# lvjiahui/DRT

Measured on AMD Instinct MI355X. Metric: M camera-rays/s (forward+backward) on 50k-tri mesh, 72 views, higher is better.
Workload: dtype f32 traversal + f64 shading/gradients; 1 GPU; horse_vh.ply x4 (1 midpoint subdivision) = 50248 tris / 25126 verts, 72 turntable views, 1024x1024 rays/view, LBVH rebuilt every step, forward+ray_loss+backward+all-reduce+SGD; targets=horse_scan.ply, mode=dropin, hip_graph=False, outputs_recycled=True, ray_binding=True, views_per_gpu=72, views_per_call=72

## Files before the change

drt_amd/_lib.py:

```python
from __future__ import annotations

import ctypes
import os

_HERE = os.path.dirname(os.path.abspath(__file__))
LIB_PATH = os.environ.get("DRT_HIP_LIB") or os.path.join(_HERE, "libdrt_hip.so")

_c = ctypes
_P = _c.c_void_p
_I64 = _c.c_int64
_D = _c.c_double

SIGNATURES = {
    "drt_last_error": (_c.c_char_p, []),
    "drt_version": (_c.c_int, []),
    "drt_deterministic": (_c.c_int, [_c.c_int]),
    "drt_fx_finalize": (_c.c_int, [_P, _I64, _P, _c.c_int, _P]),
    "drt_fx_add": (_c.c_int, [_P, _P, _I64, _P]),
    "drt_fx_to_limbs": (_c.c_int, [_P, _I64, _P, _P]),
    "drt_fx_from_limbs": (_c.c_int, [_P, _I64, _P, _P]),
    "drt_create": (_c.c_int, [_c.c_int, _c.POINTER(_P)]),
    "drt_destroy": (None, [_P]),
    "drt_update_mesh": (_c.c_int, [_P, _P, _I64, _P, _I64, _P]),
    "drt_update_vert": (_c.c_int, [_P, _P, _I64, _P]),
    "drt_update_vert_f64": (_c.c_int, [_P, _P, _I64, _P]),
    "drt_intersect": (_c.c_int, [_P, _P, _I64, _P, _P, _P]),
    "drt_intersect_any": (_c.c_int, [_P, _P, _I64, _P, _P]),
    "drt_intersect_bruteforce": (_c.c_int, [_P, _P, _I64, _P, _P, _P]),
    "drt_bvh_check": (_c.c_int, [_P, _P, _c.POINTER(_I64), _c.POINTER(_c.c_int32), _c.POINTER(_c.c_int32)]),
    "drt_bvh_sorted_faces": (_c.c_int, [_P, _P, _P]),
    "drt_build_params": (_c.c_int, [_P, _c.POINTER(_c.c_float), _P]),
    "drt_bvh_export": (_c.c_int, [_P, _c.c_int, _P, _I64, _P]),
    "drt_tree_mode": (_c.c_int, [_P, _c.c_int, _c.c_int]),
    "drt_render_forward": (_c.c_int, [_P, _P, _P, _P, _I64, _D, _D, _P, _P, _P, _P, _P, _P, _P, _c.c_int, _c.c_int, _c.c_int, _P, _P]),
    "drt_render_backward": (_c.c_int, [_P, _P, _P, _P, _I64, _D, _D, _P, _P, _P, _P, _P, _P, _P, _P]),
    "drt_render_paths_forward": (_c.c_int, [_P, _P, _P, _P, _I64, _D, _D, _c.c_int, _c.c_int, _P, _P, _P, _P, _P, _P, _P, _P]),
    "drt_render_paths_backward": (_c.c_int, [_P, _P, _P, _P, _I64, _D, _D, _c.c_int, _c.c_int, _P, _P, _P, _P, _P, _P, _P, _P]),
    "drt_render_paths_ray_loss_fused": (_c.c_int, [_P, _P, _P, _P, _P, _P, _I64, _D, _D, _c.c_int, _c.c_int, _P, _P, _P, _P]),
    "drt_render_paths_law_forward": (_c.c_int, [_P, _P, _P, _P, _I64, _D, _D, _c.c_int, _c.c_int, _P, _P, _P, _P, _P, _P, _P, _P]),
    "drt_render_paths_law_backward": (_c.c_int, [_P, _P, _P, _P, _I64, _D, _D, _c.c_int, _c.c_int, _P, _P, _P, _P, _P, _P, _P, _P]),
    "drt_render_paths_law_ray_loss_fused": (_c.c_int, [_P, _P, _P, _P, _P, _P, _I64, _D, _D, _c.c_int, _c.c_int, _P, _P, _P, _P]),
    "drt_render_paths_law_ray_loss_ior_fused": (_c.c_int, [_P, _P, _P, _P, _P, _P, _I64, _D, _D, _c.c_int, _c.c_int, _P, _P, _P, _P, _P]),
    "drt_ray_loss": (_c.c_int, [_P, _P, _P, _P, _P, _I64, _P, _P, _P, _P, _P]),
    "drt_ray_loss_listed": (_c.c_int, [_P, _P, _P, _P, _P, _P, _I64, _P, _P, _P, _P]),
    "drt_prefill_zero": (_c.c_int, [_P, _P, _I64, _P]),
    "drt_prefill_wait": (_c.c_int, [_P, _P]),
    "drt_outputs_clean": (_c.c_int, [_P, _P, _P, _P, _I64, _P, _P, _P]),
    "drt_outputs_cancel": (_c.c_int, [_P]),
    "drt_render_seed": (_c.c_int, [_P, _P, _I64]),
    "drt_render_loss_arm": (_c.c_int, [_P, _P, _P, _P, _P, _I64]),
    "drt_render_loss_taken": (_c.c_int, [_P]),
    "drt_ray_loss_listed_grad": (_c.c_int, [_P, _P, _P, _P, _I64, _D, _D, _P, _P, _P, _P, _P, _P, _P, _P, _P]),
    "drt_ray_loss_listed_grad_split": (_c.c_int, [_P, _P, _P, _P, _I64, _D, _D, _P, _P, _P, _P, _P, _P, _P, _P, _P]),
    "drt_scale_rows3": (_c.c_int, [_P, _P, _P, _P, _P]),
    "drt_render_backward_ray_loss": (_c.c_int, [_P, _P, _P, _P, _I64, _D, _D, _P, _P, _P, _P, _P, _P, _P, _P]),
    "drt_render_backward_inputs": (_c.c_int, [_P, _P, _P, _P, _I64, _D, _D, _P, _P, _P, _P, _P, _P, _P, _P, _P, _P, _P]),
    "drt_render_backward_ray_loss_inputs": (_c.c_int, [_P, _P, _P, _P, _I64, _D, _D, _P, _P, _P, _P, _P, _P, _P, _P, _P, _P, _P]),
    "drt_render_ray_loss_fused": (_c.c_int, [_P, _P, _P, _P, _P, _P, _I64, _D, _D, _P, _P, _P, _c.c_int, _c.c_int, _c.c_int, _P, _P]),
    "drt_dihedral_forward": (_c.c_int, [_P, _P, _I64, _P, _P]),
    "drt_dihedral_backward": (_c.c_int, [_P, _P, _I64, _P, _P, _P]),
    "drt_sm_loss_fused": (_c.c_int, [_P, _P, _I64, _P, _P, _P]),
    "drt_silhouette_flags": (_c.c_int, [_P, _P, _I64, _P, _P, _P]),
    "drt_edge_sample_forward": (_c.c_int, [_P, _P, _P, _I64, _P, _P, _P, _P, _P, _c.c_int, _c.c_int, _P, _P]),
    "drt_edge_sample_backward": (_c.c_int, [_P, _P, _I64, _P, _P, _P, _c.c_int, _P, _P]),
    "drt_edge_sample_backward_rows": (_c.c_int, [_P, _P, _I64, _P, _P, _P, _I64, _P, _c.c_int, _P, _P]),
    "drt_vh_term": (_c.c_int, [_P, _P, _I64, _P, _c.c_int, _c.c_int, _P, _P, _P]),
    "drt_edge_sample_backward_term": (_c.c_int, [_P, _P, _I64, _P, _P, _P, _P, _c.c_int, _P, _P]),
    "drt_edge_tables_workspace": (_I64, [_I64]),
    "drt_edge_tables": (_c.c_int, [_P, _I64, _P, _I64, _P, _P, _P, _P, _P, _P, _P]),
    "drt_subdivide_midpoint": (_c.c_int, [_P, _I64, _P, _I64, _P, _I64, _P, _c.c_int, _P, _P, _P]),
    "drt_hull_field": (_c.c_int, [_P, _c.c_int, _c.c_int, _c.c_int, _P, _D, _D, _D, _D, _c.c_int, _c.c_int, _c.c_int, _c.c_int, _P, _P]),
    "drt_hull_mark": (_c.c_int, [_P, _c.c_int, _c.c_int, _c.c_int, _D, _P, _P, _P, _P]),
    "drt_hull_emit": (_c.c_int, [_P, _c.c_int, _c.c_int, _c.c_int, _D, _D, _D, _D, _D, _P, _P, _P, _I64, _I64, _P, _P, _P]),
    "drt_decode_patterns": (_c.c_int, [_P, _P, _I64, _c.c_int, _c.c_int, _c.c_int, _c.c_int, _c.c_int, _c.c_int, _c.c_int, _P, _c.c_int, _P, _P, _P, _P, _P, _P]),
    "drt_render_image": (_c.c_int, [_P, _P, _P, _c.c_int, _c.c_int, _c.c_int, _c.c_int, _c.c_int, _D, _D, _c.c_int, _c.c_int, _c.c_int, _P, _P, _c.c_int, _c.c_int,
                                    _c.c_int, _P, _P, _P, _P, _P, _P]),
    "drt_render_image_loss": (_c.c_int, [_P, _P, _P, _c.c_int, _c.c_int, _c.c_int, _c.c_int, _c.c_int, _D, _D, _c.c_int, _c.c_int, _c.c_int, _P, _P, _c.c_int,
                                         _c.c_int, _c.c_int, _P, _P, _P, _P, _P, _P, _P, _P, _P, _P]),
    "drt_render_image_loss_screen": (_c.c_int, [_P, _P, _P, _c.c_int, _c.c_int, _c.c_int, _c.c_int, _c.c_int, _D, _D, _c.c_int, _c.c_int, _c.c_int, _P, _P, _c.c_int,
                                                _c.c_int, _c.c_int, _P, _P, _P, _P, _P, _P, _P, _P, _P, _P, _P, _P]),
    "drt_render_image_loss_camera": (_c.c_int, [_P, _P, _P, _c.c_int, _c.c_int, _c.c_int, _c.c_int, _c.c_int, _D, _D, _c.c_int, _c.c_int, _c.c_int, _P, _P, _c.c_int,
                                                _c.c_int, _c.c_int, _P, _P, _P, _P, _P, _P, _P, _P, _P, _P, _P, _P, _P]),
    "drt_render_image_absorb": (_c.c_int, [_P, _P, _P, _c.c_int, _c.c_int, _c.c_int, _c.c_int, _c.c_int, _D, _D, _c.c_int, _c.c_int, _c.c_int, _P, _P, _c.c_int,
                                           _c.c_int, _c.c_int, _P, _P, _P, _P, _P, _P, _P, _P]),
    "drt_render_image_loss_absorb": (_c.c_int, [_P, _P, _P, _c.c_int, _c.c_int, _c.c_int, _c.c_int, _c.c_int, _D, _D, _c.c_int, _c.c_int, _c.c_int, _P, _P, _c.c_int,
                                                _c.c_int, _c.c_int, _P, _P, _P, _P, _P, _P, _P, _P, _P, _P, _P, _P]),
    "drt_render_image_env": (_c.c_int, [_P, _P, _P, _c.c_int, _c.c_int, _c.c_int, _c.c_int, _c.c_int, _D, _D, _c.c_int, _c.c_int, _c.c_int, _P, _P, _c.c_int,
                                        _c.c_int, _c.c_int, _P, _P, _P, _P, _P, _P, _c.c_int, _c.c_int, _P, _c.c_int, _P, _P]),
    "drt_render_image_loss_env": (_c.c_int, [_P, _P, _P, _c.c_int, _c.c_int, _c.c_int, _c.c_int, _c.c_int, _D, _D, _c.c_int, _c.c_int, _c.c_int, _P, _P, _c.c_int,
                                             _c.c_int, _c.c_int, _P, _P, _P, _P, _P, _P, _P, _P, _P, _P, _c.c_int, _c.c_int, _P, _c.c_int, _P]),
    "drt_render_image_loss_env_param": (_c.c_int, [_P, _P, _P, _c.c_int, _c.c_int, _c.c_int, _c.c_int, _c.c_int, _D, _D, _c.c_int, _c.c_int, _c.c_int, _P, _P,
                                                   _c.c_int, _c.c_int, _c.c_int, _P, _P, _P, _P, _P, _P, _P, _P, _P, _P, _c.c_int, _c.c_int, _P, _c.c_int, _P, _P, _P]),
    "drt_image_views_check": (_c.c_int, [_c.c_int, _P, _P, _c.c_int, _c.c_int]),
    "drt_image_views_create": (_c.c_int, [_P, _c.c_int, _P, _P, _c.c_int, _c.c_int, _c.POINTER(_P)]),
    "drt_image_views_destroy": (None, [_P]),
    "drt_render_image_loss_views": (_c.c_int, [_P, _P, _P, _P, _c.c_int, _c.c_int, _c.c_int, _c.c_int, _D, _D, _c.c_int, _c.c_int, _c.c_int, _P, _c.c_int,
                                               _c.c_int, _c.c_int, _P, _P, _P, _P, _P, _P, _P, _P, _P]),
    "drt_render_image_loss_views_env": (_c.c_int, [_P, _P, _P, _P, _c.c_int, _c.c_int, _c.c_int, _c.c_int, _D, _D, _c.c_int, _c.c_int, _c.c_int, _P, _c.c_int,
                                                   _c.c_int, _c.c_int, _P, _P, _P, _P, _P, _P, _P, _P, _P, _c.c_int, _c.c_int, _P, _c.c_int, _P]),
    "drt_limit_sgd_step": (_c.c_int, [_P, _P, _P, _I64, _D, _D, _c.c_int, _c.c_int, _D, _P]),
    "drt_limit_sgd_step3": (_c.c_int, [_P, _P, _P, _I64, _D, _D, _c.c_int, _c.c_int, _D, _P, _P, _P, _P, _P]),
    "drt_weight_terms3": (_c.c_int, [_P, _P, _I64, _P, _P]),
    "drt_limit_sgd_step_total": (_c.c_int, [_P, _P, _P, _I64, _D, _D, _c.c_int, _c.c_int, _D, _P, _P, _P, _P]),
    "drt_fx_limbs_limit_sgd_step3": (_c.c_int, [_P, _I64, _P, _P, _P, _D, _D, _c.c_int, _c.c_int, _D, _P, _P, _P, _P]),
    "drt_internal_stream": (_c.c_int, [_P, _c.c_int, _c.POINTER(_P)]),
    "drt_closest_point": (_c.c_int, [_P, _P, _I64, _P, _P, _P, _P]),
    "drt_vh_loss_fused": (_c.c_int, [_P, _P, _P, _P, _I64, _c.c_int, _P, _P, _P, _c.c_int, _c.c_int, _c.c_int, _P, _P, _P]),
    "drt_remesh_isotropic": (_c.c_int, [_P, _I64, _P, _I64, _D, _c.c_int, _D, _c.c_uint, _c.POINTER(_P)]),
    "drt_rm_split_mark": (_c.c_int, [_P, _I64, _P, _D, _P, _P]),
    "drt_rm_split_plan": (_c.c_int, [_P, _I64, _P, _P, _P, _P, _I64, _P, _P, _P]),
    "drt_rm_split_faces": (_c.c_int, [_P, _I64, _P, _P, _P, _P, _P]),
    "drt_rm_vertex_normals": (_c.c_int, [_P, _P, _P, _P, _I64, _P, _P]),
    "drt_rm_vertex_faces": (_c.c_int, [_P, _I64, _I64, _P, _P, _P, _P, _P, _P, _P]),
    "drt_rm_collapse_eval_all": (_c.c_int, [_P, _I64, _P, _P, _P, _P, _D, _D, _c.c_int, _P, _P, _P, _P, _P, _P, _P, _P, _I64, _P, _P]),
    "drt_rm_surface_filter_list": (_c.c_int, [_P, _P, _P, _P, _P, _I64, _D, _P, _P]),
    "drt_rm_surface_filter": (_c.c_int, [_P, _P, _P, _P, _I64, _c.c_int, _D, _P, _P]),
    "drt_rm_closest_near": (_c.c_int, [_P, _P, _I64, _D, _P, _P]),
    "drt_rm_kill_faces": (_c.c_int, [_P, _P, _I64, _P, _P]),
    "drt_rm_collapse_apply": (_c.c_int, [_P, _I64, _P, _P, _P, _P, _P, _P, _I64, _D, _c.c_uint32, _c.c_int, _P, _P, _P, _P, _P, _c.c_int, _P, _P, _P]),
    "drt_rm_round_end": (_c.c_int, [_P, _c.c_int, _P]),
    "drt_rm_flip_eval": (_c.c_int, [_P, _I64, _P, _P, _P, _P, _D, _P, _P, _P, _P, _P]),
    "drt_rm_flip_apply": (_c.c_int, [_I64, _P, _P, _P, _I64, _c.c_int, _P, _P, _c.c_int, _P, _P, _P]),
    "drt_rm_smooth_target": (_c.c_int, [_P, _P, _P, _P, _I64, _P, _P]),
    "drt_rm_face_agreement": (_c.c_int, [_P, _P, _P, _I64, _P, _P]),
    "drt_rm_move_check": (_c.c_int, [_P, _P, _P, _P, _P, _I64, _I64, _P, _P, _P]),
    "drt_mesh_buf_size": (_c.c_int, [_P, _c.POINTER(_I64), _c.POINTER(_I64), _P]),
    "drt_mesh_buf_copy": (_c.c_int, [_P, _P, _P]),
    "drt_mesh_buf_free": (None, [_P]),
    "drt_profile_enable": (_c.c_int, [_P, _c.c_int]),
    "drt_profile_select": (_c.c_int, [_P, _c.c_uint32]),
    "drt_profile_read": (_c.c_int, [_P, _P, _P, _P]),
    "drt_profile_trace_stats": (_c.c_int, [_P, _P]),
    "drt_route_counts": (_c.c_int, [_P, _P]),
    "drt_raster_deal_counts": (_c.c_int, [_P, _P]),
    "drt_check_violations": (_c.c_int, [_P]),
}

_lib = None


class DrtError(RuntimeError):
    pass


def lib():
    global _lib
    if _lib is None:
        if not os.path.exists(LIB_PATH):
            raise DrtError(f"{LIB_PATH} not found: the HIP extension is not built "
                           "(run `python __graft_entry__.py`); there is no CPU fallback")
        h = ctypes.CDLL(LIB_PATH)
        for name, (res, args) in SIGNATURES.items():
            if os.environ.get("DRT_HIP_LIB") and not hasattr(h, name):
                continue
            fn = getattr(h, name)
            fn.restype = res
            fn.argtypes = args
        _lib = h
    return _lib


def check(rc):
    if rc != 0:
        raise DrtError(f"libdrt_hip error {rc}: {lib().drt_last_error().decode(errors='replace')}")


def ptr(t):
    return None if t is None else t.data_ptr()
```

drt_amd/csrc/drt_api.hip:

```cpp
#include "drt_scene.h"

static thread_local char g_err[512] = "";
int fail(int code, const char* fmt, ...) {
    va_list ap;
    va_start(ap, fmt);
    vsnprintf(g_err, sizeof(g_err), fmt, ap);
    va_end(ap);
    return code;
}

int ensure_slow_stack(drt_scene* s, hipStream_t st) {
    if (s->slow_stack) return DRT_OK;
    hipStreamCaptureStatus cap = hipStreamCaptureStatusNone;
    if (hipStreamIsCapturing(st, &cap) == hipSuccess && cap != hipStreamCaptureStatusNone)
        return fail(DRT_E_INVALID, "the first silhouette / closest-point / intersect query of a scene allocates its overflow area and cannot run inside a "
                                   "stream capture: issue one such call eagerly before capturing");
    int blocks = s->grid_trace;
    if (blocks < 4 * s->n_cu) blocks = 4 * s->n_cu;
    if (blocks < kRedoGrid) blocks = kRedoGrid;
    HIP_TRY(hipMalloc(&s->slow_stack, sizeof(int32_t) * (size_t)blocks * kTraceBlock * kStackSlowDev));
    return DRT_OK;
}

static int g_det = -1;
bool det_mode() {
    if (g_det < 0) { const char* ev = getenv("DRT_DETERMINISTIC"); g_det = ev && atoi(ev) != 0 ? 1 : 0; }
    return g_det != 0;
}
__global__ void __launch_bounds__(256) k_fx_finalize(const FxCell* __restrict__ cells, int64_t n, double* __restrict__ out, int accumulate) {
    for (int64_t i = blockIdx.x * 256ll + threadIdx.x; i < n; i += (int64_t)gridDim.x * 256) {
        const FxCell c = cells[i];
        const double v = fx_to_double(Fx128{c.hi, c.lo}, (uint32_t)c.flags);
        out[i] = accumulate ? out[i] + v : v;
    }
}

__global__ void __launch_bounds__(256) k_fx_add(FxCell* __restrict__ dst, const FxCell* __restrict__ src, int64_t n) {
    for (int64_t i = blockIdx.x * 256ll + threadIdx.x; i < n; i += (int64_t)gridDim.x * 256) {
        const FxCell a = dst[i], b = src[i];
        const Fx128 r = fx_add(Fx128{a.hi, a.lo}, Fx128{b.hi, b.lo});
        dst[i] = FxCell{r.hi, r.lo, a.flags | b.flags};
    }
}
constexpr int kLimbBits = kFxLimbBits;
__global__ void __launch_bounds__(256) k_fx_to_limbs(const FxCell* __restrict__ cells, int64_t n, int64_t* __restrict__ limbs) {
    constexpr uint64_t kMask = (1ull << kLimbBits) - 1ull;
    for (int64_t i = blockIdx.x * 256ll + threadIdx.x; i < n; i += (int64_t)gridDim.x * 256) {
        const FxCell c = cells[i];
        const uint64_t hi = (uint64_t)c.hi;
        limbs[4 * i + 0] = (int64_t)(c.lo & kMask);
        limbs[4 * i + 1] = (int64_t)(((c.lo >> kLimbBits) | (hi << (64 - kLimbBits))) & kMask);
        limbs[4 * i + 2] = c.hi >> (2 * kLimbBits - 64);
        limbs[4 * i + 3] = (int64_t)(((c.flags & kFxNaN) ? 1ull : 0ull) | ((c.flags & kFxPosInf) ? 1ull << 20 : 0ull) | ((c.flags & kFxNegInf) ? 1ull << 40 : 0ull));
    }
}
__global__ void __launch_bounds__(256) k_fx_from_limbs(const int64_t* __restrict__ limbs, int64_t n, FxCell* __restrict__ cells) {
    for (int64_t i = blockIdx.x * 256ll + threadIdx.x; i < n; i += (int64_t)gridDim.x * 256) {
        uint32_t flags;
        const Fx128 r = fx_from_limbs(limbs + 4 * i, flags);
        cells[i] = FxCell{r.hi, r.lo, (uint64_t)flags};
    }
}

extern "C" {

const char* drt_last_error(void) { return g_err; }
int drt_version(void) { return 13; }

int drt_deterministic(int on) {
    const int was = det_mode() ? 1 : 0;
    if (on >= 0) g_det = on != 0;
    return was;
}
int drt_fx_add(void* d_dst_cells, const void* d_src_cells, int64_t n, void* stream) {
    if (n < 0) return fail(DRT_E_INVALID, "negative size");
    if (n == 0) return DRT_OK;
    if (!d_dst_cells || !d_src_cells) return fail(DRT_E_INVALID, "null pointer argument");
    k_fx_add<<<grid_for(n, 256, 1024), 256, 0, (hipStream_t)stream>>>(static_cast<FxCell*>(d_dst_cells), static_cast<const FxCell*>(d_src_cells), n);
    HIP_TRY(hipGetLastError());
    return DRT_OK;
}
int drt_fx_to_limbs(const void* d_cells, int64_t n, int64_t* d_limbs, void* stream) {
    if (n < 0) return fail(DRT_E_INVALID, "negative size");
    if (n == 0) return DRT_OK;
    if (!d_cells || !d_limbs) return fail(DRT_E_INVALID, "null pointer argument");
    k_fx_to_limbs<<<grid_for(n, 256, 1024), 256, 0, (hipStream_t)stream>>>(static_cast<const FxCell*>(d_cells), n, d_limbs);
    HIP_TRY(hipGetLastError());
    return DRT_OK;
}
int drt_fx_from_limbs(const int64_t* d_limbs, int64_t n, void* d_cells, void* stream) {
    if (n < 0) return fail(DRT_E_INVALID, "negative size");
    if (n == 0) return DRT_OK;
    if (!d_cells || !d_limbs) return fail(DRT_E_INVALID, "null pointer argument");
    k_fx_from_limbs<<<grid_for(n, 256, 1024), 256, 0, (hipStream_t)stream>>>(d_limbs, n, static_cast<FxCell*>(d_cells));
    HIP_TRY(hipGetLastError());
    return DRT_OK;
}
int drt_fx_finalize(const void* d_cells, int64_t n, double* d_out, int accumulate, void* stream) {
    if (n < 0) return fail(DRT_E_INVALID, "negative size");
    if (n == 0) return DRT_OK;
    if (!d_cells || !d_out) return fail(DRT_E_INVALID, "null pointer argument");
    k_fx_finalize<<<grid_for(n, 256, 1024), 256, 0, (hipStream_t)stream>>>(static_cast<const FxCell*>(d_cells), n, d_out, accumulate);
    HIP_TRY(hipGetLastError());
    return DRT_OK;
}

int drt_create(int device, drt_scene_t** out) {
    if (!out) return fail(DRT_E_INVALID, "out is null");
    int count = 0;
    HIP_TRY(hipGetDeviceCount(&count));
    if (device < 0 || device >= count) return fail(DRT_E_INVALID, "device %d out of range (%d visible)", device, count);
    HIP_TRY(hipSetDevice(device));
    drt_scene* s = new (std::nothrow) drt_scene();
    if (!s) return fail(DRT_E_NOMEM, "host allocation failed");
    s->device = device;
    hipError_t e = hipMalloc(&s->params, sizeof(BuildParams));
    if (e == hipSuccess) e = hipMalloc(&s->scratch, sizeof(unsigned long long) * 8);
    if (e == hipSuccess) e = hipMalloc(&s->bounds_acc, sizeof(uint32_t) * 12);
    if (e == hipSuccess) {
        const uint32_t init[12] = {0xFF800000u, 0xFF800000u, 0xFF800000u, 0x007FFFFFu, 0x007FFFFFu, 0x007FFFFFu,
                                   0xFF800000u, 0xFF800000u, 0xFF800000u, 0x007FFFFFu, 0x007FFFFFu, 0x007FFFFFu};
        e = hipMemcpy(s->bounds_acc, init, sizeof(init), hipMemcpyHostToDevice);
    }
    if (e == hipSuccess) e = hipMalloc(&s->vcount, sizeof(unsigned) * 4);
    if (e == hipSuccess) e = hipMemset(s->vcount, 0, sizeof(unsigned) * 4);
    if (e == hipSuccess) e = hipMalloc(&s->seg_counts, sizeof(unsigned) * drt_scene::kMaxSeg);
    if (e == hipSuccess) e = hipEventCreateWithFlags(&s->fork_ev, hipEventDisableTiming);
    if (e == hipSuccess) e = hipStreamCreateWithFlags(&s->build_stream, hipStreamNonBlocking);
    if (e == hipSuccess) e = hipEventCreateWithFlags(&s->prefill_fork, hipEventDisableTiming);
    if (e == hipSuccess) e = hipEventCreateWithFlags(&s->prefill_done, hipEventDisableTiming);
    if (e == hipSuccess) e = hipEventCreateWithFlags(&s->prefill_done_cap, hipEventDisableTiming);
    if (e == hipSuccess) e = hipEventCreateWithFlags(&s->build_fork, hipEventDisableTiming);
    if (e == hipSuccess) e = hipEventCreateWithFlags(&s->build_done, hipEventDisableTiming);
    if (const char* ev = getenv("DRT_ASYNC_BUILD")) s->async_build = atoi(ev) != 0;
    if (const char* ev = getenv("DRT_CULL_DIRECT")) s->cull_direct = atoi(ev) != 0;
    if (const char* ev = getenv("DRT_CULL_PARK")) s->cull_park = atoi(ev) != 0;
    if (const char* ev = getenv("DRT_CULL_DIRECT_MIN_LOG2")) { const int v = atoi(ev); if (v >= 0 && v <= 40) s->cull_direct_min_rays = (int64_t)1 << v; }
    if (const char* ev = getenv("DRT_TREE")) { const int v = atoi(ev); if (v >= 0 && v <= 2) s->tree_mode = v; }
    if (const char* ev = getenv("DRT_REBUILD_EVERY")) { const int v = atoi(ev); if (v >= 1) s->rebuild_every = v; }
    if (const char* ev = getenv("DRT_STREAMS")) { const int v = atoi(ev); if (v >= 1 && v <= drt_scene::kMaxSub) s->n_sub = v; }
    if (const char* ev = getenv("DRT_RASTER")) s->use_raster = atoi(ev) != 0;
    if (const char* ev = getenv("DRT_RASTER_DEAL")) s->raster_deal = atoi(ev) != 0;
    if (const char* ev = getenv("DRT_RASTER_DEAL_MIN_RUNS")) { const long long v = atoll(ev); if (v >= 0) s->raster_deal_min_runs = v; }
    if (const char* ev = getenv("DRT_RASTER_DEAL_FIXED")) { const int v = atoi(ev); if (v >= 1 && v <= 65536) s->raster_deal_fixed = (uint32_t)v; }
    if (const char* ev = getenv("DRT_HIT_SEED")) s->hit_seed = atoi(ev) != 0;
    if (const char* ev = getenv("DRT_ARM_FINISH_BESIDE")) s->arm_finish_beside = atoi(ev) != 0;
    if (const char* ev = getenv("DRT_SEED_TILED")) s->seed_tiled = atoi(ev) != 0;
    if (const char* ev = getenv("DRT_GRID_CANARY")) s->grid_canary = atoi(ev) != 0;
    if (const char* ev = getenv("DRT_FILL_OVERLAP")) s->fill_overlap = atoi(ev) != 0;
    if (const char* ev = getenv("DRT_FILL_AFTER_SHADE1")) s->fill_after_shade1 = atoi(ev) != 0;
    if (const char* ev = getenv("DRT_SUB_PER_STREAM")) { const int v = atoi(ev); if (v >= 1 && v <= 16) s->sub_per_stream = v; }
    if (const char* ev = getenv("DRT_MIN_SUB_LOG2")) { const int v = atoi(ev); if (v >= 12 && v <= 30) s->min_sub_rays = (int64_t)1 << v; }
    for (int k = 0; k < s->n_sub && e == hipSuccess; ++k) {
        drt_scene::Sub& w = s->sub[k];
        e = hipStreamCreateWithFlags(&w.stream, hipStreamNonBlocking);
        if (e == hipSuccess) e = hipEventCreateWithFlags(&w.done, hipEventDisableTiming);
        if (e == hipSuccess) e = hipEventCreateWithFlags(&w.tail, hipEventDisableTiming);
        if (e == hipSuccess) e = hipEventCreateWithFlags(&w.fill_fork, hipEventDisableTiming);
        if (e == hipSuccess) e = hipEventCreateWithFlags(&w.fill_join, hipEventDisableTiming);
        if (e == hipSuccess) e = hipMalloc(&w.qcount, sizeof(unsigned) * kQCount);
        if (e == hipSuccess) e = hipMalloc(&w.slow_stack, sizeof(int32_t) * (size_t)kRedoGrid * kTraceBlock * kStackSlowDev);
    }
    if (e == hipSuccess) {
        hipDeviceProp_t prop;
        if (hipGetDeviceProperties(&prop, device) == hipSuccess && prop.multiProcessorCount > 0) s->n_cu = prop.multiProcessorCount;
        int per_cu;
        per_cu = query_blocks_per_cu();
        s->grid_trace = s->n_cu * per_cu;
        if (s->grid_trace > kTraceGridMax) s->grid_trace = kTraceGridMax;
        per_cu = pipeline_blocks_per_cu();
        s->grid_path = s->n_cu * per_cu;
        if (s->grid_path * 2 > kTraceGridMax) s->grid_path = kTraceGridMax / 2;
        per_cu = mega_blocks_per_cu();
        s->grid_mega = s->n_cu * per_cu;
        if (const char* e = getenv("DRT_MEGA_BPC")) { const int v = atoi(e); if (v >= 1 && v <= 8) s->grid_mega = v * s->n_cu; }
        if (const char* e = getenv("DRT_MEGA_MAX_LOG2")) { const int v = atoi(e); s->mega_max_rays = v <= 0 ? 0 : (v <= 31 ? (int64_t)1 << v : (int64_t)1 << 31); }
        if (const char* e = getenv("DRT_SHADE_MIN")) { const int v = atoi(e); if (v >= 1 && v <= 64) s->shade_min = v; }
        if (const char* e = getenv("DRT_MEGA_REFILL_MIN")) { const int v = atoi(e); if (v >= 1 && v <= 64) s->mega_refill_min = v; }
        if (const char* e = getenv("DRT_TRACE_BPC")) { const int v = atoi(e); if (v >= 1 && v * s->n_cu * 2 <= kTraceGridMax) s->grid_path = v * s->n_cu; }
        if (const char* e = getenv("DRT_INNER_MIN")) { const int v = atoi(e); if (v >= 1 && v <= 64) s->inner_min = v; }
        if (const char* e = getenv("DRT_REFILL_MIN")) { const int v = atoi(e); if (v >= 1 && v <= 64) s->refill_min = v; }
        if (const char* e = getenv("DRT_CHUNK_LOG2")) { const int v = atoi(e); if (v >= 16 && v <= 30) s->chunk_rays = (int64_t)1 << v; }
    }
    if (e != hipSuccess) {
        drt_destroy(s);
        return fail(DRT_E_HIP, "hipMalloc: %s", hipGetErrorString(e));
    }
    *out = s;
    return DRT_OK;
}

void drt_destroy(drt_scene_t* s) {
    if (!s) return;
    (void)hipSetDevice(s->device);
    if (s->build_stream) (void)hipStreamSynchronize(s->build_stream);
    scene_free_mesh(s);
    if (s->build_fork) (void)hipEventDestroy(s->build_fork);
    if (s->build_done) (void)hipEventDestroy(s->build_done);
    if (s->build_stream) (void)hipStreamDestroy(s->build_stream);
    (void)hipFree(s->params);
    (void)hipFree(s->slow_stack);
    (void)hipFree(s->scratch); (void)hipFree(s->bounds_acc); (void)hipFree(s->seg_counts);
    (void)hipFree(s->b1_list); (void)hipFree(s->b1_redo); (void)hipFree(s->b1_count);
    for (int j = 0; j < drt_scene::kMaxSub; ++j) {
        drt_scene::Sub& w = s->sub[j];
        for (int k = 0; k < 3; ++k) { (void)hipFree(w.q_idx[k]); (void)hipFree(w.q_ray[k]); (void)hipFree(w.q_face[k]); }
        (void)hipFree(w.tmp_face1); (void)hipFree(w.tmp_face2); (void)hipFree(w.qcount); (void)hipFree(w.slow_stack); (void)hipFree(w.redo);
        (void)hipFree(w.zbuf); (void)hipFree(w.zmask); (void)hipFree(w.vmodel); (void)hipFree(w.big); (void)hipFree(w.big_count); (void)hipFree(w.gen_list); (void)hipFree(w.ray64);
        (void)hipFree(w.deal.table);
        if (w.done) (void)hipEventDestroy(w.done);
        if (w.fill_fork) (void)hipEventDestroy(w.fill_fork);
        if (w.fill_join) (void)hipEventDestroy(w.fill_join);
        if (w.tail) (void)hipEventDestroy(w.tail);
        if (w.stream) (void)hipStreamDestroy(w.stream);
    }
    image_views_free(s);
    image_loss_free(s);
    paths_free(s);
    (void)hipFree(s->vcount);
    (void)hipFree(s->vh_list);
    if (s->fork_ev) (void)hipEventDestroy(s->fork_ev);
    if (s->prefill_fork) (void)hipEventDestroy(s->prefill_fork);
    if (s->prefill_done) (void)hipEventDestroy(s->prefill_done);
    if (s->prefill_done_cap) (void)hipEventDestroy(s->prefill_done_cap);
    for (auto& e : s->prof_ev) (void)hipEventDestroy(e);
    (void)hipFree(s->prof_counts);
    delete s;
}

int drt_profile_enable(drt_scene_t* s, int on) {
    CHECK_SCENE(s);
    if (on && s->prof_ev.empty()) {
        s->prof_ev.resize(8192);
        s->prof_stage.resize(4096);
        for (auto& e : s->prof_ev) HIP_TRY(hipEventCreate(&e));
        HIP_TRY(hipMalloc(&s->prof_counts, sizeof(unsigned long long) * (kProfStages + 12)));
        HIP_TRY(hipMemset(s->prof_counts, 0, sizeof(unsigned long long) * (kProfStages + 12)));
    }
    s->prof_on = on != 0;
    s->prof_stats = on == 2;
    s->prof_serial = on == 3;
    return DRT_OK;
}

int drt_profile_select(drt_scene_t* s, uint32_t stage_mask) {
    CHECK_SCENE(s);
    s->prof_mask = stage_mask;
    return DRT_OK;
}

int drt_profile_read(drt_scene_t* s, double* ms_out, int64_t* launches_out, int64_t* items_out) {
    CHECK_SCENE(s);
    if (!ms_out || !launches_out || !items_out) return fail(DRT_E_INVALID, "null pointer argument");
    for (int k = 0; k < kProfStages; ++k) { ms_out[k] = 0.0; launches_out[k] = 0; items_out[k] = 0; }
    if (s->prof_ev.empty()) return DRT_OK;
    HIP_TRY(hipStreamSynchronize(s->prof_stream));
    if (s->build_stream) HIP_TRY(hipStreamSynchronize(s->build_stream));
    if (s->prof_dropped) {
        const size_t lost = s->prof_dropped;
        s->prof_dropped = 0; s->prof_used = 0;
        return fail(DRT_E_INVALID, "%zu stage timings were not recorded (event pool exhausted): read the profile more often", lost);
    }
    for (size_t k = 0; k + 1 < s->prof_used; k += 2) {
        float ms = 0.f;
        HIP_TRY(hipEventElapsedTime(&ms, s->prof_ev[k], s->prof_ev[k + 1]));
        const int stg = s->prof_stage[k / 2];
        ms_out[stg] += ms;
        launches_out[stg] += 1;
    }
    unsigned long long h[kProfStages + 12];
    HIP_TRY(hipMemcpy(h, s->prof_counts, sizeof(h), hipMemcpyDeviceToHost));
    for (int k = 0; k < kProfStages; ++k) items_out[k] = (int64_t)h[k];
    for (int k = 0; k < 12; ++k) s->trace_stats[k] = (int64_t)h[kProfStages + k];
    HIP_TRY(hipMemset(s->prof_counts, 0, sizeof(h)));
    s->prof_used = 0;
    return DRT_OK;
}

int drt_route_counts(drt_scene_t* s, int64_t* out8) {
    CHECK_SCENE(s);
    if (!out8) return fail(DRT_E_INVALID, "null pointer argument");
    for (int k = 0; k < 8; ++k) out8[k] = s->route_counts[k];
    return DRT_OK;
}

int drt_raster_deal_counts(drt_scene_t* s, int64_t* out2) {
    CHECK_SCENE(s);
    if (!out2) return fail(DRT_E_INVALID, "null pointer argument");
    out2[0] = s->raster_deal_counts[0]; out2[1] = s->raster_deal_counts[1];
    return DRT_OK;
}

int drt_internal_stream(drt_scene_t* s, int which, void** out) {
    if (!s || !out) return fail(DRT_E_INVALID, "null pointer argument");
    if (which == 0) { *out = (void*)s->build_stream; return DRT_OK; }
    if (which >= 1 && which <= s->n_sub) { *out = (void*)s->sub[which - 1].stream; return DRT_OK; }
    return fail(DRT_E_INVALID, "no internal stream %d (0 = build, 1..%d = pipelines)", which, s->n_sub);
}

int drt_check_violations(int64_t* out4) {
    if (!out4) return fail(DRT_E_INVALID, "null pointer argument");
#if defined(DRT_CHECK)
    HIP_TRY(hipDeviceSynchronize());
    unsigned long long tot[4] = {0, 0, 0, 0};
    if (check_counters_pipeline(tot) || check_counters_trace(tot)) return fail(DRT_E_HIP, "could not read the check counters");
    for (int k = 0; k < 4; ++k) out4[k] = (int64_t)tot[k];
#else
    for (int k = 0; k < 4; ++k) out4[k] = -1;
#endif
    return DRT_OK;
}

int drt_profile_trace_stats(drt_scene_t* s, int64_t* out12) {
    CHECK_SCENE(s);
    if (!out12) return fail(DRT_E_INVALID, "null pointer argument");
    for (int k = 0; k < 12; ++k) out12[k] = s->trace_stats[k];
    return DRT_OK;
}


}
```

drt_amd/csrc/drt_pipeline.hip:

```cpp
#include "drt_device.h"
#include "drt_trace_kernel.h"
#include "drt_pathsink.h"


struct Ray64 {
    double* o;
    double* d;
};
struct Pipe {
    RayList r0, r1, r2;
    unsigned* count;
    unsigned* valid;
    int32_t* redo;
};




__device__ __forceinline__ void write_dead(int64_t i, double* out_ori, double* out_dir, uint8_t* mask, int32_t* face2) {
    const d3 z{0.0, 0.0, 0.0};
    store_d3(out_ori, i, z);
    store_d3(out_dir, i, z);
    mask[3 * i] = 0; mask[3 * i + 1] = 0; mask[3 * i + 2] = 0;
    face2[i] = -1;
// ... 103 lines not shown
            } else if (!FUSED || valid[i]) {
                const d3 o64 = load_d3(origin, i), d64 = load_d3(dir, i);
                o = to_f32(o64); d = to_f32(d64);
                bool verified = false;
                if (raster) {
                    ViewModel& vm = rz.views[view];
                    verified = vm.ok && view_verify(vm, o64, d64, (double)x, (double)(y - view * (unsigned)rz.img_h));
                    if (!verified && vm.all) __hip_atomic_store(&vm.all, 0, __ATOMIC_RELAXED, __HIP_MEMORY_SCOPE_AGENT);
                }
                if (verified) {
                    cand = key != kRasterEmpty;
                    face = (int32_t)(uint32_t)key;
                } else {
                    cand = n_tris > 0 && (rz.no_tree || hits_top_boxes(nodes, o, d));
                    generic = cand;
                }
            } else if (raster && rz.mode == DRT_GRID_ESTABLISH) {
                ViewModel& vm = rz.views[view];
                if (vm.all && !(vm.ok && view_verify(vm, load_d3(origin, i), load_d3(dir, i), (double)x, (double)(y - view * (unsigned)rz.img_h))))
                    __hip_atomic_store(&vm.all, 0, __ATOMIC_RELAXED, __HIP_MEMORY_SCOPE_AGENT);
            }
        }
        const bool live = i < n;
        if (!dead_writes) {
        } else if (tile_w > 0 && __ballot(cand || !live) == 0ull) {
            write_dead_row<FUSED>(i - (tid & 63), tid & 63, out_ori, out_dir, mask, face1, face2);
        } else if (live && !cand) {
            face1[i] = -1;
            write_dead(i, out_ori, out_dir, mask, face2);
        }
        const int any_cand = __syncthreads_or(cand ? 1 : 0);
        if (clear_bit && (tid & 63) == 0) atomicAnd(&rz.zmask[i >> 11], ~clear_bit);
        if (!any_cand) return;
        int slot;
        if (tile_w > 0) {
            s_flag[vt] = cand ? 1 : 0;
            __syncthreads();
            s_slot[tid] = block_push(s_flag[tid] != 0, &p.count[0], s_tmp);
            __syncthreads();
            slot = s_slot[vt];
            __syncthreads();
        } else {
            slot = block_push(cand, &p.count[0], s_tmp);
        }
        if (slot >= 0) {
            p.r0.idx[slot] = (int32_t)i; store_ray32(p.r0.ray, slot, o, d);
            if (raster) p.r0.face[slot] = generic && rz.pending ? kFacePending : face;
        }
        if (raster && __syncthreads_or(generic ? 1 : 0)) {
            const int g = block_push(generic, &p.count[3], s_tmp);
            if (g >= 0) rz.gen_list[g] = slot;
        }
    }
}

template <bool FUSED>
__global__ void __launch_bounds__(kPathBlock, 8) k_cull(const Node4Q* __restrict__ nodes, int n_tris, const double* __restrict__ origin, const double* __restrict__ dir,
                                                      const uint8_t* __restrict__ valid, int64_t n, double* __restrict__ out_ori,
                                                      double* __restrict__ out_dir, uint8_t* __restrict__ mask,
                                                      int32_t* __restrict__ face1, int32_t* __restrict__ face2, Pipe p, int tile_w, RasterIn rz,
                                                      bool prefilled ) {
    __shared__ CullShared sh;
    cull_patch<FUSED>(blockIdx.x, prefilled, sh, nodes, n_tris, origin, dir, valid, n, out_ori, out_dir, mask, face1, face2, p, tile_w, rz);
}

constexpr int kCullRun = 4;
constexpr int kCullPer = kCullRun;
constexpr int kCullCap = kCullRun * kPathBlock;
constexpr int kCullCursor = 32;
constexpr int kCullFewPerCu = 2;
constexpr int kCullLongRuns = 16;
static_assert(kCullCursor < kQCount, "the cursor word lies inside the counter block");
struct CullBatch {
    int32_t idx[kCullCap];
    int32_t face[kCullCap];
    unsigned n, base, next[2];
    unsigned wtot[kCullPer][kPathWaves];
};
template <bool FUSED>
__global__ void __launch_bounds__(kPathBlock) k_cull_listed(const uint32_t* __restrict__ patches, const unsigned* __restrict__ n_patches,
                                                           const Node4Q* __restrict__ nodes, int n_tris, const double* __restrict__ origin, const double* __restrict__ dir,
                                                           const uint8_t* __restrict__ valid, int64_t n, double* __restrict__ out_ori,
                                                           double* __restrict__ out_dir, uint8_t* __restrict__ mask,
                                                           int32_t* __restrict__ face1, int32_t* __restrict__ face2, Pipe p, int tile_w, RasterIn rz,
                                                           PathCtx c, bool direct, bool prefilled, Ray64 park, unsigned few, unsigned long_list) {
    __shared__ CullShared sh;
    __shared__ CullBatch sb;
    const int tid = threadIdx.x, wave = tid >> 6, lane = tid & 63;
    const unsigned ppr = (unsigned)tile_w / 64u;
    const RayList dst = direct ? p.r1 : p.r0;
    unsigned* const dst_count = direct ? &p.count[1] : &p.count[0];
    unsigned* const cursor = &p.count[kCullCursor];
    unsigned n_hits = 0;
    const unsigned count = *n_patches;
    const unsigned active = count >= long_list ? gridDim.x : min(few, gridDim.x);
    if (blockIdx.x >= active) return;
    unsigned first = blockIdx.x * (unsigned)kCullRun;
    if (tid == 0) {
        sb.n = 0u;
        if (first < count) sb.next[0] = active * (unsigned)kCullRun + atomicAdd(cursor, (unsigned)kCullRun);
    }
    __syncthreads();

    auto close_batch = [&]() {
        const unsigned cnt = sb.n;
        if (cnt == 0u) { __syncthreads(); return; }
        int32_t ei[kCullPer], ef[kCullPer];
        f3 eo[kCullPer], ed[kCullPer];
        bool push[kCullPer];
        unsigned rank[kCullPer];
#pragma unroll
        for (int j = 0; j < kCullPer; ++j) {
            const unsigned k = (unsigned)(j * kPathBlock + tid);
            push[j] = false;
            ei[j] = 0; ef[j] = -1;
            eo[j] = f3{0.f, 0.f, 0.f}; ed[j] = f3{0.f, 0.f, 1.f};
            if (k < cnt) {
                const int64_t i = sb.idx[k];
                const int32_t f1 = sb.face[k];
                ei[j] = (int32_t)i; ef[j] = f1;
                if (direct) {
                    face1[i] = f1;
                    d3 v0, v1, v2;
                    int32_t vid[3];
                    Bounce b;
                    load_tri64(c, f1, v0, v1, v2, vid);
                    bounce_forward(load_d3(origin, i), load_d3(dir, i), v0, v1, v2, c.ior_ext, c.ior_int, b);
                    push[j] = !b.tir;
                    eo[j] = to_f32(b.new_o); ed[j] = to_f32(b.wt);
                    if (push[j] && park.o) { store_d3(park.o, i, b.new_o); store_d3(park.d, i, b.wt); }
                    if (!push[j] && !FUSED) { if (prefilled) face2[i] = -1; else write_dead(i, out_ori, out_dir, mask, face2); }
                    ++n_hits;
                } else {
                    eo[j] = to_f32(load_d3(origin, i)); ed[j] = to_f32(load_d3(dir, i));
                    push[j] = true;
                }
            }
            const unsigned long long bm = __ballot(push[j]);
            if (lane == 0) sb.wtot[j][wave] = (unsigned)__popcll(bm);
            rank[j] = (unsigned)__popcll(bm & ((1ull << lane) - 1ull));
        }
        __syncthreads();
        unsigned tot = 0;
#pragma unroll
        for (int j = 0; j < kCullPer; ++j) {
            unsigned before = tot;
#pragma unroll
            for (int w = 0; w < kPathWaves; ++w) { const unsigned cw = sb.wtot[j][w]; if (w < wave) before += cw; tot += cw; }
            rank[j] += before;
        }
        if (tid == 0) { sb.base = tot ? atomicAdd(dst_count, tot) : 0u; sb.n = 0u; }
        __syncthreads();
        const unsigned base = sb.base;
#pragma unroll
        for (int j = 0; j < kCullPer; ++j) {
            if (!push[j]) continue;
            const unsigned slot = base + rank[j];
            dst.idx[slot] = ei[j];
            float2* e = reinterpret_cast<float2*>(dst.ray + 6 * (int64_t)slot);
            e[0] = float2{eo[j].x, eo[j].y}; e[1] = float2{eo[j].z, ed[j].x}; e[2] = float2{ed[j].y, ed[j].z};
            if (!direct) dst.face[slot] = ef[j];
        }
    };

    for (unsigned it = 0; first < count; ++it) {
        const unsigned cnt = min((unsigned)kCullRun, count - first);
        uint32_t pt[kCullRun];
        bool ok[kCullRun];
        unsigned word[kCullRun];
        unsigned long long key[kCullRun];
        int64_t zs[kCullRun], ri[kCullRun];
#pragma unroll
        for (int j = 0; j < kCullRun; ++j) pt[j] = (unsigned)j < cnt ? patches[first + j] : 0u;
#pragma unroll
        for (int j = 0; j < kCullRun; ++j) {
            const unsigned prow = pt[j] / ppr;
            const unsigned x = 64u * (pt[j] - prow * ppr) + 16u * (unsigned)wave + 4u * ((unsigned)lane >> 4) + ((unsigned)lane & 3u);
            const unsigned y = 4u * prow + (((unsigned)lane >> 2) & 3u);
            const unsigned view = (4u * prow) / (unsigned)rz.img_h;
            ri[j] = (int64_t)y * tile_w + x;
            zs[j] = raster_slot(x, y, (unsigned)tile_w);
            ok[j] = false; word[j] = 0u; key[j] = kRasterEmpty;
            if ((unsigned)j < cnt) {
                ok[j] = rz.views[view].ok && rz.views[view].all;
                word[j] = rz.zmask[ri[j] >> 11];
                key[j] = rz.zbuf[zs[j]];
            }
        }
#pragma unroll
        for (int j = 0; j < kCullRun; ++j) {
            if ((unsigned)j >= cnt) continue;
            if (!ok[j]) {
                cull_patch<FUSED>(pt[j], true, sh, nodes, n_tris, origin, dir, valid, n, out_ori, out_dir, mask, face1, face2, p, tile_w, rz);
                __syncthreads();
                continue;
            }
            const int64_t i = ri[j];
            const bool has = ((word[j] >> ((i >> 6) & 31)) & 1u) != 0u && key[j] != kRasterEmpty;
            if (has) rz.zbuf[zs[j]] = kRasterEmpty;
            const bool take = has && (!FUSED || valid[i]);
            const unsigned long long bm = __ballot(take);
            if (bm != 0ull) {
                unsigned at = 0u;
                if (lane == 0) at = atomicAdd(&sb.n, (unsigned)__popcll(bm));
                at = (unsigned)__shfl((int)at, 0);
                if (take) {
                    const unsigned k = at + (unsigned)__popcll(bm & ((1ull << lane) - 1ull));
                    sb.idx[k] = (int32_t)i;
                    sb.face[k] = (int32_t)(uint32_t)key[j];
                }
            }
        }
        __syncthreads();
        if (tid < 4 * (int)cnt) {
            const unsigned q = patches[first + ((unsigned)tid >> 2)], prow = q / ppr;
            const int64_t i0 = (int64_t)(4u * prow + ((unsigned)tid & 3u)) * tile_w + 64u * (q - prow * ppr);
            const unsigned bit = 1u << ((i0 >> 6) & 31);
            if (rz.zmask[i0 >> 11] & bit) atomicAnd(&rz.zmask[i0 >> 11], ~bit);
        }
        const unsigned nxt = sb.next[it & 1u];
        if (tid == 0 && nxt < count) sb.next[(it + 1u) & 1u] = active * (unsigned)kCullRun + atomicAdd(cursor, (unsigned)kCullRun);
        close_batch();
        first = nxt;
    }
    if (direct) {
        unsigned h = n_hits;
        for (int off = 32; off >= 1; off >>= 1) h += __shfl_xor(h, off);
        if (lane == 0 && h) atomicAdd(&p.count[17], h);
    }
}
constexpr int kCullSgprBlocks = 6;
int cull_blocks_per_cu() {
    int per_cu = 0;
    if (hipOccupancyMaxActiveBlocksPerMultiprocessor(&per_cu, k_cull_listed<false>, kPathBlock, 0) != hipSuccess || per_cu < 1) per_cu = 4;
    int f = 0;
    if (hipOccupancyMaxActiveBlocksPerMultiprocessor(&f, k_cull_listed<true>, kPathBlock, 0) == hipSuccess && f >= 1 && f < per_cu) per_cu = f;
    if (per_cu > 8) per_cu = 8;
    if (per_cu > kCullSgprBlocks) per_cu = kCullSgprBlocks;
    return per_cu;
}

__global__ void __launch_bounds__(kPathBlock) k_patch_list(unsigned n_patches, int tile_w, RasterIn rz, uint32_t* __restrict__ list, unsigned* count) {
    __shared__ unsigned s_tmp[kPathWaves + 1];
    const unsigned patch = blockIdx.x * kPathBlock + threadIdx.x;
    bool take = false;
    if (patch < n_patches) {
        const unsigned ppr = (unsigned)tile_w / 64u, prow = patch / ppr;
        const unsigned view = (4u * prow) / (unsigned)rz.img_h;
        take = true;
        if (rz.views[view].ok && rz.views[view].all) {
            const int64_t row0 = (int64_t)(4u * prow) * tile_w + 64u * (patch - prow * ppr);
            unsigned any = 0;
            for (int r = 0; r < 4; ++r) {
                const int64_t g = (row0 + (int64_t)r * tile_w) >> 6;
                any |= rz.zmask[g >> 5] >> (g & 31);
            }
            take = (any & 1u) != 0;
        }
    }
    const int slot = block_push(take, count, s_tmp);
    if (slot >= 0) list[slot] = patch;
}

template <bool FUSED>
__global__ void __launch_bounds__(kPathBlock) k_shade1(PathCtx c, const double* __restrict__ origin, const double* __restrict__ dir,
                                                        double* __restrict__ out_ori, double* __restrict__ out_dir, uint8_t* __restrict__ mask,
                                                        int32_t* __restrict__ face1, int32_t* __restrict__ face2, Pipe p,
                                                        bool prefilled , Ray64 r64) {
    __shared__ StageMem stage;
    stage_init(stage);
    const unsigned n0 = p.count[0];
    const unsigned per_block = ((n0 + gridDim.x - 1) / gridDim.x + kPathBlock - 1) / kPathBlock * kPathBlock;
    const unsigned first = blockIdx.x * per_block, last = min(n0, first + per_block);
    for (unsigned base = first; base < last; base += kPathBlock) {
        const unsigned k = base + threadIdx.x;
        bool ok = false;
        int64_t i = 0;
        f3 o2{0.f, 0.f, 0.f}, d2{0.f, 0.f, 1.f};
        if (k < n0) {
            i = p.r0.idx[k];
            const int32_t f1 = p.r0.face[k];
            if (f1 != kFacePending) face1[i] = f1;
            if (f1 >= 0) {
                d3 v0, v1, v2;
                int32_t vid[3];
                Bounce b;
                load_tri64(c, f1, v0, v1, v2, vid);
                bounce_forward(load_d3(origin, i), load_d3(dir, i), v0, v1, v2, c.ior_ext, c.ior_int, b);
                ok = !b.tir;
                o2 = to_f32(b.new_o); d2 = to_f32(b.wt);
                if (ok && r64.o) { store_d3(r64.o, i, b.new_o); store_d3(r64.d, i, b.wt); }
            }
            if (!ok && !FUSED && f1 != kFacePending) { if (prefilled) face2[i] = -1; else write_dead(i, out_ori, out_dir, mask, face2); }
        }
        stage_push(stage, ok, (int32_t)i, o2, d2, p.r1, &p.count[1]);
    }
    stage_flush(stage, p.r1, &p.count[1]);
}

template <bool FUSED>
__global__ void __launch_bounds__(kTraceBlock) k_gen_late(PathCtx c, const double* __restrict__ origin, const double* __restrict__ dir,
                                                          double* __restrict__ out_ori, double* __restrict__ out_dir, uint8_t* __restrict__ mask,
                                                          int32_t* __restrict__ face1, int32_t* __restrict__ face2, Pipe p,
                                                          const int32_t* __restrict__ gen_list, bool prefilled, Ray64 r64) {
    __shared__ int32_t lds[kStackFast][kTraceBlock];
    const unsigned n = p.count[3];
    if (n == 0) return;
    Stack st = make_stack(lds, c.tc);
    for (unsigned k = blockIdx.x * kTraceBlock + threadIdx.x; k < n; k += gridDim.x * kTraceBlock) {
        const int32_t slot = gen_list[k];
        if (p.r0.face[slot] != kFacePending) continue;
        const int64_t i = p.r0.idx[slot];
        const float* e = p.r0.ray + 6 * (int64_t)slot;
        const Hit h = traverse<false>(c.tc.nodes, c.tc.tris, c.tc.n_tris, f3{e[0], e[1], e[2]}, f3{e[3], e[4], e[5]}, st);
        p.r0.face[slot] = h.face;
        face1[i] = h.face;
        bool ok = false;
        if (h.face >= 0) {
            d3 v0, v1, v2;
            int32_t vid[3];
            Bounce b;
            load_tri64(c, h.face, v0, v1, v2, vid);
            bounce_forward(load_d3(origin, i), load_d3(dir, i), v0, v1, v2, c.ior_ext, c.ior_int, b);
            ok = !b.tir;
            if (ok) {
                const unsigned s1 = atomicAdd(&p.count[1], 1u);
                p.r1.idx[s1] = (int32_t)i;
                store_ray32(p.r1.ray, (int)s1, to_f32(b.new_o), to_f32(b.wt));
                if (r64.o) { store_d3(r64.o, i, b.new_o); store_d3(r64.d, i, b.wt); }
            }
        }
        if (!ok && !FUSED) { if (prefilled) face2[i] = -1; else write_dead(i, out_ori, out_dir, mask, face2); }
    }
}

template <bool FUSED>
__global__ void __launch_bounds__(kPathBlock) k_shade2(PathCtx c, const double* __restrict__ origin, const double* __restrict__ dir,
                                                        double* __restrict__ out_ori, double* __restrict__ out_dir, uint8_t* __restrict__ mask,
                                                        const int32_t* __restrict__ face1, int32_t* __restrict__ face2, Pipe p,
                                                        bool parked ) {
    __shared__ StageMem stage;
    stage_init(stage);
    const unsigned n1 = p.count[1];
    const unsigned per_block = ((n1 + gridDim.x - 1) / gridDim.x + kPathBlock - 1) / kPathBlock * kPathBlock;
    const unsigned first = blockIdx.x * per_block, last = min(n1, first + per_block);
    for (unsigned base = first; base < last; base += kPathBlock) {
        const unsigned k = base + threadIdx.x;
        bool ok = false;
        int64_t i = 0;
        f3 o3{0.f, 0.f, 0.f}, d3f{0.f, 0.f, 1.f};
        if (k < n1) {
            i = p.r1.idx[k];
            const int32_t f2 = p.r1.face[k];
            if (f2 >= 0) {
                d3 v0, v1, v2;
                int32_t vid[3];
                Bounce b;
                d3 o2, d2;
                if (parked) {
                    o2 = load_d3(out_ori, i); d2 = load_d3(out_dir, i);
                } else {
                    load_tri64(c, face1[i], v0, v1, v2, vid);
                    bounce_forward(load_d3(origin, i), load_d3(dir, i), v0, v1, v2, c.ior_ext, c.ior_int, b);
                    o2 = b.new_o; d2 = b.wt;
                }
                load_tri64(c, f2, v0, v1, v2, vid);
                bounce_forward(o2, d2, v0, v1, v2, c.ior_ext, c.ior_int, b);
                ok = !b.tir;
                if (ok) {
                    o3 = to_f32(b.new_o); d3f = to_f32(b.wt);
                    face2[i] = f2;
                    if (!FUSED) {
                        store_d3(out_ori, i, b.new_o);
                        store_d3(out_dir, i, b.wt);
                        mask[3 * i] = 1; mask[3 * i + 1] = 1; mask[3 * i + 2] = 1;
                    }
                }
            }
            if (!ok) { if (FUSED) face2[i] = -1; else write_dead(i, out_ori, out_dir, mask, face2); }
        }
        stage_push(stage, ok, (int32_t)i, o3, d3f, p.r2, &p.count[2]);
    }
    stage_flush(stage, p.r2, &p.count[2]);
}

__global__ void __launch_bounds__(kPathBlock) k_finish(double* __restrict__ out_ori, double* __restrict__ out_dir, uint8_t* __restrict__ mask,
                                                        int32_t* __restrict__ face2, Pipe p, int64_t chunk_base, int32_t* __restrict__ valid_idx) {
    __shared__ StageMem stage;
    stage_init(stage);
    const RayList out{valid_idx, nullptr, nullptr};
    const unsigned n2 = p.count[2];
    const unsigned per_block = ((n2 + gridDim.x - 1) / gridDim.x + kPathBlock - 1) / kPathBlock * kPathBlock;
    const unsigned first = blockIdx.x * per_block, last = min(n2, first + per_block);
    for (unsigned base = first; base < last; base += kPathBlock) {
        const unsigned k = base + threadIdx.x;
        bool keep = false;
        int64_t i = 0;
        if (k < n2) {
            i = p.r2.idx[k];
            keep = p.r2.face[k] < 0;
            if (!keep) write_dead(i, out_ori, out_dir, mask, face2);
        }
        if (valid_idx) stage_push(stage, keep, (int32_t)(chunk_base + i), f3{0.f, 0.f, 0.f}, f3{0.f, 0.f, 0.f}, out, p.valid);
    }
    if (valid_idx) stage_flush(stage, out, p.valid);
}

enum : int { kLaneIdle = 0, kLaneT1 = 2, kLaneT1D = 3, kLaneT2 = 4, kLaneT2D = 5 };
constexpr int kVBuf = 128;

template <class STACK>
__device__ __forceinline__ bool path_leaf(const TriRec* __restrict__ tris, TravState& s, STACK& st, bool any) {
    if (s.cur == kEmptyChild) return trav_pop(s, st);
    const int32_t ref = ~s.cur;
    const int first = ref >> kLeafBits, count = (ref & (kLeafMax - 1)) + 1;
    for (int j = 0; j < count; ++j) {
        const F4* tp = reinterpret_cast<const F4*>(tris + first + j);
        const F4 p0 = tp[0], p1 = tp[1], p2 = tp[2];
        float t;
        if (tri_hit(s.o, s.d, f3{p0.x, p0.y, p0.z}, f3{p1.x, p1.y, p1.z}, f3{p2.x, p2.y, p2.z}, p1.w, t)) {
            int32_t face;
            memcpy(&face, &p0.w, 4);
            if (any) { s.best_t = t; s.best_face = face; return true; }
            if (t < s.best_t || (t == s.best_t && face < s.best_face)) { s.best_t = t; s.best_face = face; }
        }
    }
    return trav_pop(s, st);
}

template <bool FUSED>
__global__ void __launch_bounds__(kPathBlock, 4) k_path(PathCtx c, Ray64 r64, double* __restrict__ out_ori, double* __restrict__ out_dir, uint8_t* __restrict__ mask,
                                                        int32_t* __restrict__ face2, Pipe p, unsigned* cursor , int64_t chunk_base,
                                                        int32_t* __restrict__ valid_idx, int refill_min, int inner_min, int shade_min,
                                                        unsigned long long* stats, bool count_items) {
    __shared__ int32_t lds[kStackFast + 1 + kGuardRows][kPathBlock];
    __shared__ int32_t s_vbuf[kPathWaves][kVBuf];
    FastStack st;
    st.base = (drt::FastPtr)&lds[0][threadIdx.x]; st.stride = kPathBlock; st.depth = kStackFast - 3; st.reset(); st.overflow = false;
#if defined(DRT_CHECK)
    for (int g = 0; g < kGuardRows; ++g) lds[kStackFast + 1 + g][threadIdx.x] = kGuardPoison;
#endif
    const unsigned n = p.count[1];
    const int lane = threadIdx.x & 63, wv = threadIdx.x >> 6;
    const unsigned long long lower = (1ull << lane) - 1ull;
    constexpr unsigned kXcd = 8;
    const bool split = gridDim.x % kXcd == 0 && n >= 4096u * kXcd;
    const unsigned xcd = split ? blockIdx.x % kXcd : 0u, parts = split ? kXcd : 1u;
    const unsigned wave = (split ? blockIdx.x / kXcd : blockIdx.x) * kPathWaves + (threadIdx.x >> 6);
    const unsigned n_waves = (split ? gridDim.x / kXcd : gridDim.x) * kPathWaves;
    const unsigned part_lo = (unsigned)((unsigned long long)n * xcd / parts), part_hi = (unsigned)((unsigned long long)n * (xcd + 1) / parts);
    const unsigned part_n = part_hi - part_lo;
    unsigned first = (part_n + n_waves - 1) / n_waves;
    first = first > 64u ? 64u : (first < 8u ? 8u : first);
    unsigned my_next = part_lo + wave * first;
    unsigned my_end = my_next + first;
    if (my_end > part_hi) my_end = part_hi;
    if (my_next > part_hi) my_next = part_hi;
    const unsigned dyn_lo = part_lo + n_waves * first;
    bool dry = dyn_lo >= part_hi;
    int32_t* const v_out = FUSED ? p.r2.idx : valid_idx;
    unsigned* const v_count = FUSED ? &p.count[2] : p.valid;
    unsigned vn = 0;
    auto v_flush = [&]() {
        if (vn == 0) return;
        unsigned base = 0;
        if (lane == 0) base = atomicAdd(v_count, vn);
        base = (unsigned)__builtin_amdgcn_readfirstlane((int)base);
        for (unsigned k = lane; k < vn; k += 64u) {
            v_out[base + k] = s_vbuf[wv][k];
            if (FUSED) p.r2.face[base + k] = -1;
        }
        vn = 0;
    };
    int stage = kLaneIdle;
    int32_t rk = 0, ri = 0;
    TravState s;
    s.cur = 0; s.best_face = -1; s.best_t = 0.f;
    unsigned long long wave_steps = 0, lane_steps = 0, leaf_steps = 0;
    unsigned n_t2 = 0;
    for (;;) {
        const unsigned long long idle = __ballot(stage == kLaneIdle);
        if (idle != 0 && (my_next < my_end || !dry) && ((int)__popcll(idle) >= refill_min || idle == ~0ull)) {
            const unsigned want = (unsigned)__popcll(idle);
            unsigned base, got;
            if (my_next < my_end) {
                base = my_next;
                got = my_end - my_next < want ? my_end - my_next : want;
                my_next += got;
            } else {
                unsigned b0 = 0;
                if (lane == 0) b0 = atomicAdd(&cursor[xcd], want);
                b0 = (unsigned)__builtin_amdgcn_readfirstlane((int)b0);
                base = dyn_lo + b0;
                got = base >= part_hi ? 0u : (part_hi - base < want ? part_hi - base : want);
                if (got < want) dry = true;
            }
            const unsigned r = (unsigned)__popcll(idle & lower);
            if (stage == kLaneIdle && r < got) {
                const unsigned k = base + r;
                rk = (int32_t)k;
                ri = p.r1.idx[k];
                const float* e = p.r1.ray + 6 * (int64_t)k;
                trav_init(s, st, f3{e[0], e[1], e[2]}, f3{e[3], e[4], e[5]});
                st.overflow = false;
                stage = kLaneT1;
            }
        }
        if (__ballot(stage != kLaneIdle) == 0) {
            if (my_next < my_end || !dry) continue;
            break;
        }
        {
            const unsigned long long waiting = __ballot(stage & 1), walking = __ballot(stage != kLaneIdle && !(stage & 1));
            if (waiting != 0 && ((int)__popcll(waiting) >= shade_min || walking == 0)) {
                const bool fin = stage == kLaneT2D;
                const bool keep = fin && s.best_face < 0;
                if (fin && !keep) { if (FUSED) face2[ri] = -1; else write_dead(ri, out_ori, out_dir, mask, face2); }
                if (v_out) {
                    const unsigned long long km = __ballot(keep);
                    if (km != 0) {
                        if (keep) s_vbuf[wv][vn + (unsigned)__popcll(km & lower)] = FUSED ? ri : (int32_t)(chunk_base + ri);
                        vn += (unsigned)__popcll(km);
                        __builtin_amdgcn_wave_barrier();
                        if (vn > kVBuf - 64) v_flush();
                    }
                }
                if (fin) stage = kLaneIdle;
                if (stage == kLaneT1D) {
                    const int32_t f2 = s.best_face;
                    bool ok = false;
                    if (f2 >= 0) {
                        d3 v0, v1, v2;
                        int32_t vid[3];
                        Bounce b;
                        const d3 o2 = load_d3(r64.o, ri), d2 = load_d3(r64.d, ri);
                        load_tri64(c, f2, v0, v1, v2, vid);
                        bounce_forward(o2, d2, v0, v1, v2, c.ior_ext, c.ior_int, b);
                        ok = !b.tir;
                        if (ok) {
                            face2[ri] = f2;
                            if (!FUSED) {
                                store_d3(out_ori, ri, b.new_o);
                                store_d3(out_dir, ri, b.wt);
                                mask[3 * (int64_t)ri] = 1; mask[3 * (int64_t)ri + 1] = 1; mask[3 * (int64_t)ri + 2] = 1;
                            }
                            trav_init(s, st, to_f32(b.new_o), to_f32(b.wt));
                            st.overflow = false;
                            stage = kLaneT2;
                            ++n_t2;
                        }
                    }
                    if (!ok) {
                        if (FUSED) face2[ri] = -1; else write_dead(ri, out_ori, out_dir, mask, face2);
                        stage = kLaneIdle;
                    }
                }
            }
        }
        for (;;) {
            const bool walking = stage != kLaneIdle && !(stage & 1);
            const bool at_inner = walking && s.cur >= 0;
            const unsigned long long mi = __ballot(at_inner);
            if (mi == 0) break;
            if ((int)__popcll(mi) < inner_min && __ballot(walking && s.cur < 0) != 0) break;
            ++wave_steps;
            lane_steps += (unsigned long long)__popcll(mi);
            if (at_inner) {
                const bool done = trav_inner<false>(c.tc.nodes, s, st);
                if (st.overflow) {
                    p.redo[atomicAdd(&p.count[5], 1u)] = rk;
                    stage = kLaneIdle;
                } else if (done) {
                    stage |= 1;
                }
            }
        }
        {
            const bool at_leaf = stage != kLaneIdle && !(stage & 1) && s.cur < 0;
            const unsigned long long ml = __ballot(at_leaf);
            if (ml != 0) {
                ++wave_steps; ++leaf_steps;
                lane_steps += (unsigned long long)__popcll(ml);
                if (at_leaf && path_leaf(c.tc.tris, s, st, stage == kLaneT2)) stage |= 1;
            }
        }
    }
    v_flush();
#if defined(DRT_CHECK)
    for (int g = 0; g < kGuardRows; ++g) DRT_DEV_ASSERT(lds[kStackFast + 1 + g][threadIdx.x] == kGuardPoison, drt::kCheckGuardRow);
#endif
    if (count_items) {
        const unsigned t2 = (unsigned)wave_sum((double)n_t2);
        if (lane == 0 && t2) atomicAdd(&p.count[6], t2);
    }
    if (stats && lane == 0 && wave_steps) {
        atomicAdd(stats + 0, wave_steps);
        atomicAdd(stats + 1, lane_steps);
        atomicAdd(stats + 2, leaf_steps);
        atomicMax(stats + 3, wave_steps);
    }
}

template <bool FUSED>
__global__ void __launch_bounds__(kTraceBlock) k_path_redo(PathCtx c, const double* __restrict__ origin, const double* __restrict__ dir, const int32_t* __restrict__ face1,
                                                           double* __restrict__ out_ori, double* __restrict__ out_dir, uint8_t* __restrict__ mask,
                                                           int32_t* __restrict__ face2, Pipe p, int64_t chunk_base, int32_t* __restrict__ valid_idx) {
    __shared__ int32_t lds[kStackFast][kTraceBlock];
    const unsigned n = p.count[5];
    if (n == 0) return;
    Stack st = make_stack(lds, c.tc);
    for (unsigned q = blockIdx.x * kTraceBlock + threadIdx.x; q < n; q += gridDim.x * kTraceBlock) {
        const int32_t rk = p.redo[q];
        const int64_t i = p.r1.idx[rk];
        const float* e = p.r1.ray + 6 * (int64_t)rk;
        const int32_t f2 = traverse<false>(c.tc.nodes, c.tc.tris, c.tc.n_tris, f3{e[0], e[1], e[2]}, f3{e[3], e[4], e[5]}, st).face;
        bool alive = false;
        if (f2 >= 0) {
            d3 v0, v1, v2;
            int32_t vid[3];
            Bounce b;
            load_tri64(c, face1[i], v0, v1, v2, vid);
            bounce_forward(load_d3(origin, i), load_d3(dir, i), v0, v1, v2, c.ior_ext, c.ior_int, b);
            const d3 o2 = b.new_o, d2 = b.wt;
            load_tri64(c, f2, v0, v1, v2, vid);
            bounce_forward(o2, d2, v0, v1, v2, c.ior_ext, c.ior_int, b);
// ... 125 lines not shown
        for (unsigned k = threadIdx.x; k < cnt; k += kPathBlock) list[base + k] = s_buf[k];
        __syncthreads();
        if (threadIdx.x == 0) s_tmp[kPathWaves] = 0u;
        __syncthreads();
    };
    LossAcc<DET> acc;
    const int64_t span = (int64_t)kLossRays * kPathBlock;
    for (int64_t base = blockIdx.x * span; base < n; base += (int64_t)gridDim.x * span) {
        const int64_t i0 = base + kLossRays * (int64_t)threadIdx.x;
        bool on[kLossRays] = {false, false, false, false};
        d3 g[kLossRays] = {d3{0.0, 0.0, 0.0}, d3{0.0, 0.0, 0.0}, d3{0.0, 0.0, 0.0}, d3{0.0, 0.0, 0.0}};
        const bool full = i0 + kLossRays - 1 < n;
        if (full) {
            const uint32_t v4 = *reinterpret_cast<const uint32_t*>(valid + i0);
            const uint32_t* mp = reinterpret_cast<const uint32_t*>(mask + 3 * i0);
            const uint32_t m0 = mp[0], m1 = mp[1], m2 = mp[2];
            on[0] = (v4 & 0xFFu) && (m0 & 0xFFu);
            on[1] = (v4 & 0xFF00u) && (m0 & 0xFF000000u);
            on[2] = (v4 & 0xFF0000u) && (m1 & 0xFF0000u);
            on[3] = (v4 & 0xFF000000u) && (m2 & 0xFF00u);
        } else {
            for (int k = 0; k < kLossRays; ++k) on[k] = i0 + k < n && valid[i0 + k] && mask[3 * (i0 + k)];
        }
        for (int k = 0; k < kLossRays; ++k)
            if (on[k]) acc.add(ray_loss_term(load_d3(out_ori, i0 + k), load_d3(out_dir, i0 + k), load_d3(screen_pixel, i0 + k), g[k]));
        if (g_out_dir) {
            const int64_t w0 = i0 - kLossRays * (int64_t)lane;
            if (w0 + kLossRays * 64 <= n) {
                Dbl2* q = reinterpret_cast<Dbl2*>(g_out_dir + 3 * w0);
                for (int j = 0; j < 6; ++j) q[j * 64 + lane] = Dbl2{0.0, 0.0};
                if (__ballot(on[0] | on[1] | on[2] | on[3]) != 0) {
                    asm volatile("s_waitcnt vmcnt(0)" ::: "memory");
                    for (int k = 0; k < kLossRays; ++k) if (on[k]) store_d3(g_out_dir, i0 + k, g[k]);
                }
            } else {
                for (int k = 0; k < kLossRays; ++k) if (i0 + k < n) store_d3(g_out_dir, i0 + k, g[k]);
            }
        }
        if (list) {
            unsigned long long m[kLossRays];
            unsigned before[kLossRays], tot = 0;
            for (int k = 0; k < kLossRays; ++k) { m[k] = __ballot(on[k]); before[k] = tot; tot += (unsigned)__popcll(m[k]); }
            if (lane == 0) s_tmp[wave] = tot;
            __syncthreads();
            unsigned wbase = s_tmp[kPathWaves], add = 0;
            for (int w = 0; w < kPathWaves; ++w) { const unsigned c = s_tmp[w]; if (w < wave) wbase += c; add += c; }
            if (add) {
                for (int k = 0; k < kLossRays; ++k)
                    if (on[k]) s_buf[wbase + before[k] + (unsigned)__popcll(m[k] & lower)] = (int32_t)(i0 + k);
                __syncthreads();
                if (threadIdx.x == 0) s_tmp[kPathWaves] += add;
                __syncthreads();
                if (s_tmp[kPathWaves] > kLossBuf - kLossRays * kPathBlock) flush();
            } else {
                __syncthreads();
            }
        }
    }
    if (list) flush();
    acc.flush(loss);
}

template <bool DET>
__global__ void __launch_bounds__(256) k_ray_loss_listed(const double* __restrict__ out_ori, const double* __restrict__ out_dir,
                                                         const double* __restrict__ screen_pixel, const uint8_t* __restrict__ valid,
                                                         const int32_t* __restrict__ paths, const int64_t* __restrict__ n_paths, double* loss,
                                                         int32_t* __restrict__ rows, unsigned* n_rows) {
    __shared__ unsigned s_tmp[kPathWaves + 1];
    const int64_t n = *n_paths;
    LossAcc<DET> acc;
    for (int64_t base = blockIdx.x * 256ll; base < n; base += (int64_t)gridDim.x * 256) {
        const int64_t k = base + threadIdx.x;
        bool on = false;
        int32_t i = 0;
        if (k < n) {
            i = paths[k];
            on = valid[i] != 0;
            if (on) { d3 g; acc.add(ray_loss_term(load_d3(out_ori, i), load_d3(out_dir, i), load_d3(screen_pixel, i), g)); }
        }
        if (rows) {
            const int slot = block_push(on, n_rows, s_tmp);
            if (slot >= 0) rows[slot] = i;
        }
    }
    acc.flush(loss);
}

__global__ void __launch_bounds__(256) k_scale_rows3(double* __restrict__ x, const int32_t* __restrict__ list, const unsigned* __restrict__ n_ptr,
                                                     const double* __restrict__ scale) {
    const unsigned n = *n_ptr;
    const double sc = *scale;
    for (unsigned k = blockIdx.x * blockDim.x + threadIdx.x; k < n; k += gridDim.x * blockDim.x) {
        const int64_t i = list[k];
        x[3 * i] *= sc; x[3 * i + 1] *= sc; x[3 * i + 2] *= sc;
    }
}

template <bool DET>
__global__ void __launch_bounds__(256) k_loss_bwd_fused(PathCtx c, const double* __restrict__ origin, const double* __restrict__ dir,
                                                        const double* __restrict__ screen_pixel, const int32_t* __restrict__ face1,
                                                        const int32_t* __restrict__ face2, Pipe p, double* loss, double* grad_verts,
                                                        unsigned long long* n_valid) {
    const unsigned n2 = p.count[2];
    LossAcc<DET> acc;
    unsigned cnt = 0;
    sink_pass<DET, kBwdBatch>(n2, grad_verts, [&](unsigned k, const PathSink<DET>& add) {
        if (p.r2.face[k] >= 0) return;
        const int64_t i = p.r2.idx[k];
        int32_t vid1[3], vid2[3];
        Bounce b1, b2;
        path_recompute(c, load_d3(origin, i), load_d3(dir, i), face1[i], face2[i], b1, b2, vid1, vid2);
        d3 g_dir;
        acc.add(ray_loss_term(b2.new_o, b2.wt, load_d3(screen_pixel, i), g_dir));
        ++cnt;
        path_backward(b1, b2, vid1, vid2, d3{0.0, 0.0, 0.0}, g_dir, add);
    });
    acc.flush(loss);
    if (n_valid && cnt) atomicAdd(n_valid, (unsigned long long)cnt);
}


template <bool DET, bool INPUTS = false>
__global__ void __launch_bounds__(256) k_render_bwd_rows(PathCtx c, const double* __restrict__ origin, const double* __restrict__ dir,
                                                         const double* __restrict__ screen_pixel, const int32_t* __restrict__ face1,
                                                         const int32_t* __restrict__ face2, const int32_t* __restrict__ rows,
                                                         const unsigned* __restrict__ n_rows, const double* __restrict__ scale, double* grad_verts,
                                                         InputGrads in) {
    const unsigned n = *n_rows;
    const double sc = *scale;
    InputAcc<DET> inp;
    sink_pass<DET, kBwdBatch>(n, grad_verts, [&](unsigned k, const PathSink<DET>& add) {
        const int64_t i = rows[k];
        int32_t vid1[3], vid2[3];
        Bounce b1, b2;
        path_recompute(c, load_d3(origin, i), load_d3(dir, i), face1[i], face2[i], b1, b2, vid1, vid2);
        d3 g_dir;
        (void)ray_loss_term(b2.new_o, b2.wt, load_d3(screen_pixel, i), g_dir);
        g_dir = sc * g_dir;
        const d3 z{0.0, 0.0, 0.0};
        if constexpr (INPUTS) {
            d3 g_o0, g_d0;
            double gi, ge;
            path_backward_inputs(c, b1, b2, vid1, vid2, z, g_dir, add, g_o0, g_d0, gi, ge);
            inp.add(in, i, g_o0, g_d0, gi, ge);
        } else {
            path_backward(b1, b2, vid1, vid2, z, g_dir, add);
        }
    });
    if constexpr (INPUTS) inp.flush(in);
}

template <bool DET>
__global__ void __launch_bounds__(256) k_loss_bwd_listed(PathCtx c, const double* __restrict__ origin, const double* __restrict__ dir,
                                                         const double* __restrict__ screen_pixel, const uint8_t* __restrict__ valid,
                                                         const int32_t* __restrict__ face1, const int32_t* __restrict__ face2,
                                                         const int32_t* __restrict__ paths, const int64_t* __restrict__ n_paths,
                                                         const unsigned* __restrict__ first_ptr, const unsigned* __restrict__ n32_ptr,
                                                         double* loss, double* grad_verts) {
    const int64_t first = first_ptr ? (int64_t)*first_ptr : 0;
    paths += first;
    const int64_t n = (n32_ptr ? (int64_t)*n32_ptr : *n_paths) - first;
    LossAcc<DET> acc;
    sink_pass<DET, kBwdBatch>(n, grad_verts, [&](int64_t k, const PathSink<DET>& add) {
        const int64_t i = paths[k];
        if (!valid[i]) return;
        int32_t vid1[3], vid2[3];
        Bounce b1, b2;
        path_recompute(c, load_d3(origin, i), load_d3(dir, i), face1[i], face2[i], b1, b2, vid1, vid2);
        d3 g_dir;
        acc.add(ray_loss_term(b2.new_o, b2.wt, load_d3(screen_pixel, i), g_dir));
        path_backward(b1, b2, vid1, vid2, d3{0.0, 0.0, 0.0}, g_dir, add);
    });
    acc.flush(loss);
}

template <bool DET>
__global__ void __launch_bounds__(256) k_loss_bwd_armed(PathCtx c, const double* __restrict__ origin, const double* __restrict__ dir,
                                                        const double* __restrict__ screen_pixel, const uint8_t* __restrict__ valid,
                                                        const int32_t* __restrict__ face1, const int32_t* __restrict__ face2, Pipe p,
                                                        double* loss, double* grad_verts) {
    const unsigned n2 = p.count[2];
    LossAcc<DET> acc;
    sink_pass<DET, kBwdBatch>(n2, grad_verts, [&](unsigned k, const PathSink<DET>& add) {
        if (p.r2.face[k] >= 0) return;
        const int64_t i = p.r2.idx[k];
        if (!valid[i]) return;
        int32_t vid1[3], vid2[3];
        Bounce b1, b2;
        path_recompute(c, load_d3(origin, i), load_d3(dir, i), face1[i], face2[i], b1, b2, vid1, vid2);
        d3 g_dir;
        acc.add(ray_loss_term(b2.new_o, b2.wt, load_d3(screen_pixel, i), g_dir));
        path_backward(b1, b2, vid1, vid2, d3{0.0, 0.0, 0.0}, g_dir, add);
    });
    acc.flush(loss);
}

__global__ void k_prof_counts(const unsigned* __restrict__ qcount, unsigned long long n_rays, unsigned long long* __restrict__ tot, int fused, int raster, bool mega) {
    if (threadIdx.x != 0 || blockIdx.x != 0) return;
    atomicAdd(&tot[kStageCull], n_rays);
    if (raster) atomicAdd(&tot[kStageRaster], n_rays);
    if (raster && !fused) atomicAdd(&tot[kStageFill], n_rays);
    if (mega) {
        atomicAdd(&tot[kStageTrace1], (unsigned long long)qcount[raster ? 3 : 0]); atomicAdd(&tot[kStageShade1], (unsigned long long)qcount[0] + qcount[17]);
        atomicAdd(&tot[kStagePath], (unsigned long long)qcount[1]);
        atomicAdd(&tot[kStageTrace2], (unsigned long long)qcount[1]); atomicAdd(&tot[kStageShade2], (unsigned long long)qcount[1]);
        atomicAdd(&tot[kStageTrace3], (unsigned long long)qcount[6]);
        atomicAdd(&tot[fused ? kStageLossBwdFused : kStageFinish], (unsigned long long)qcount[6]);
        return;
    }
    atomicAdd(&tot[kStageTrace1], (unsigned long long)qcount[raster ? 3 : 0]); atomicAdd(&tot[kStageShade1], (unsigned long long)qcount[0] + qcount[17]);
    atomicAdd(&tot[kStageTrace2], (unsigned long long)qcount[1]); atomicAdd(&tot[kStageShade2], (unsigned long long)qcount[1]);
    atomicAdd(&tot[kStageTrace3], (unsigned long long)qcount[2]);
    atomicAdd(&tot[fused ? kStageLossBwdFused : kStageFinish], (unsigned long long)qcount[2]);
}
__global__ void k_prof_counts_bwd(const unsigned* __restrict__ vcount, unsigned long long n_rays, unsigned long long* __restrict__ tot) {
    if (threadIdx.x != 0 || blockIdx.x != 0) return;
    tot[kStageCollect] += n_rays;
    tot[kStageBackward] += vcount[0];
}

static int ensure_queues(drt_scene::Sub& w, int64_t n, bool fused, bool mega = false) {
    if (fused && mega && n > w.ray64_cap) {
        (void)hipFree(w.ray64); w.ray64 = nullptr; w.ray64_cap = 0;
        HIP_TRY(hipMalloc(&w.ray64, sizeof(double) * 6 * n));
        w.ray64_cap = n;
    }
    if (n > w.q_cap) {
        for (int k = 0; k < 3; ++k) {
            (void)hipFree(w.q_idx[k]); (void)hipFree(w.q_ray[k]); (void)hipFree(w.q_face[k]);
            w.q_idx[k] = nullptr; w.q_ray[k] = nullptr; w.q_face[k] = nullptr;
        }
        w.q_cap = 0;
        for (int k = 0; k < 3; ++k) {
            HIP_TRY(hipMalloc(&w.q_idx[k], sizeof(int32_t) * n));
            HIP_TRY(hipMalloc(&w.q_ray[k], sizeof(float) * 6 * n));
            HIP_TRY(hipMalloc(&w.q_face[k], sizeof(int32_t) * n));
        }
        (void)hipFree(w.redo); w.redo = nullptr;
        HIP_TRY(hipMalloc(&w.redo, sizeof(int32_t) * n));
        (void)hipFree(w.gen_list); w.gen_list = nullptr;
        HIP_TRY(hipMalloc(&w.gen_list, sizeof(int32_t) * n));
        w.q_cap = n;
    }
    if (fused && n > w.fused_cap) {
        (void)hipFree(w.tmp_face1); (void)hipFree(w.tmp_face2);
        w.tmp_face1 = w.tmp_face2 = nullptr; w.fused_cap = 0;
        HIP_TRY(hipMalloc(&w.tmp_face1, sizeof(int32_t) * n));
        HIP_TRY(hipMalloc(&w.tmp_face2, sizeof(int32_t) * n));
        w.fused_cap = n;
    }
    return DRT_OK;
}

static Pipe pipe_of(const drt_scene* s, const drt_scene::Sub& w) {
    return Pipe{RayList{w.q_idx[0], w.q_ray[0], w.q_face[0]}, RayList{w.q_idx[1], w.q_ray[1], w.q_face[1]},
                RayList{w.q_idx[2], w.q_ray[2], w.q_face[2]}, w.qcount, s->vcount, w.redo};
}

struct Plan { int64_t size; int count; int streams; };
static Plan plan_call(const drt_scene* s, int64_t n_rays, int tile_w, int tile_h) {
    int64_t unit = 256;
    if (tile_w >= 64 && tile_w % 64 == 0) unit = 4 * (int64_t)tile_w;
    if (unit > 256 && tile_h >= 4 && tile_h % 4 == 0 && n_rays % ((int64_t)tile_w * tile_h) == 0) unit = (int64_t)tile_w * tile_h;
    int64_t count = (n_rays + s->chunk_rays - 1) / s->chunk_rays;
    const int64_t by_min = n_rays / s->min_sub_rays;
    const int64_t most = (int64_t)s->n_sub * s->sub_per_stream;
    const int64_t want = by_min < most ? by_min : most;
    if (want > count) count = want;
    if (count < 1) count = 1;
    int64_t size = (n_rays + count - 1) / count;
    size = (size + unit - 1) / unit * unit;
    count = (n_rays + size - 1) / size;
    Plan pl;
    pl.size = size; pl.count = (int)count; pl.streams = count < s->n_sub ? (int)count : s->n_sub;
    if (s->prof_serial) pl.streams = 1;
    return pl;
}

__global__ void k_store_models(const ViewModel* __restrict__ work, ViewModel* __restrict__ cache, int n) {
    const int v = blockIdx.x * blockDim.x + threadIdx.x;
    if (v >= n) return;
    ViewModel m = work[v];
    m.all = (m.ok && m.all) ? 1 : 0;
    m.ok = m.all;
    cache[v] = m;
}

static bool raster_on(const drt_scene* s, int64_t n, int tile_w, int tile_h) {
    if (!s->use_raster || s->n_faces <= 0 || tile_w < 64 || tile_w % 64 != 0 || tile_h < 4 || tile_h % 4 != 0) return false;
    const int64_t image = (int64_t)tile_w * tile_h;
    return n > 0 && n % image == 0 && n / image <= 65535;
}

constexpr int kIntPreOri = 1 << 16, kIntPreDir = 1 << 17, kIntPreMask = 1 << 18, kIntMask = kIntPreOri | kIntPreDir | kIntPreMask;
extern "C++" {
template <bool FUSED>
static int launch_chunk(drt_scene* s, drt_scene::Sub& w, hipStream_t st, const PathCtx& pc, const Pipe& p, const double* o, const double* d, const uint8_t* valid,
                        int64_t n, double* out_ori, double* out_dir, uint8_t* mask, int32_t* face1, int32_t* face2, int tile_w, int tile_h,
                        int grid_mode, ViewModel* grid_cache ,
                        hipStream_t aux , int64_t chunk_base, int32_t* valid_idx,
                        bool* n_finished ,
                        int32_t* seed2 = nullptr ) {
    if (n_finished) *n_finished = false;
    const bool sparse_faces = (grid_mode & DRT_GRID_SPARSE_FACES) != 0;
    const bool pre_ori = (grid_mode & kIntPreOri) != 0, pre_dir = (grid_mode & kIntPreDir) != 0, pre_mask = (grid_mode & kIntPreMask) != 0;
    const bool all_verified = (grid_mode & DRT_GRID_ALL_VERIFIED) != 0 && (grid_mode & 3) == DRT_GRID_TRUST && grid_cache;
    grid_mode &= 3;
    const int gs = 8 * s->n_cu;
    if (tile_w < 64 || tile_w % 64 != 0 || n % (4 * (int64_t)tile_w) != 0) tile_w = 0;
    RasterIn rz{nullptr, 0, nullptr, nullptr, nullptr, 0, 0, 0, 0};
    const bool mega = s->mega_max_rays > 0 && n <= s->mega_max_rays && n_finished != nullptr;
    const Ray64 r64 = !mega ? Ray64{nullptr, nullptr} : (FUSED ? Ray64{w.ray64, w.ray64 + 3 * n} : Ray64{out_ori, out_dir});
    bool late_fill = false;
    hipStream_t fs = s->prof_serial ? st : s->build_stream;
    {
        hipStreamCaptureStatus cs = hipStreamCaptureStatusNone;
        if (fs != st && hipStreamIsCapturing(st, &cs) == hipSuccess && cs != hipStreamCaptureStatusNone) fs = aux ? aux : st;
    }
    const int64_t image = (int64_t)tile_w * tile_h;
    if (raster_on(s, n, tile_w, tile_h)) {
        const int n_views = (int)(n / image);
        int rc = ensure_raster(s, w, n, n_views, st);
        if (rc) return rc;
        if (!grid_cache) grid_mode = DRT_GRID_NONE;
        if (!FUSED && grid_mode == DRT_GRID_TRUST) {
            late_fill = s->fill_overlap;
            if (!late_fill) {
                StageTimer t(s, st, kStageFill);
                if (!pre_ori) (void)hipMemsetAsync(out_ori, 0, sizeof(double) * 3 * n, st);
                if (!pre_dir) (void)hipMemsetAsync(out_dir, 0, sizeof(double) * 3 * n, st);
                if (!pre_mask) (void)hipMemsetAsync(mask, 0, 3 * n, st);
            }
            if (!sparse_faces) { (void)hipMemsetAsync(face1, 0xFF, sizeof(int32_t) * n, st); (void)hipMemsetAsync(face2, 0xFF, sizeof(int32_t) * n, st); }
        }
        if (late_fill && mega) {
            if (fs != st && aux) fs = aux;
            if (fs != st) { HIP_TRY(hipEventRecord(w.fill_fork, st)); HIP_TRY(hipStreamWaitEvent(fs, w.fill_fork, 0)); }
            { StageTimer tf(s, fs, kStageFill);
              if (!pre_ori) (void)hipMemsetAsync(out_ori, 0, sizeof(double) * 3 * n, fs);
              if (!pre_dir) (void)hipMemsetAsync(out_dir, 0, sizeof(double) * 3 * n, fs);
              if (!pre_mask) (void)hipMemsetAsync(mask, 0, 3 * n, fs); }
            if (fs != st) HIP_TRY(hipEventRecord(w.fill_join, fs));
        }
        StageTimer t(s, st, kStageRaster);
        rc = launch_raster(s, w, st, o, d, n_views, tile_w, tile_h, grid_mode == DRT_GRID_TRUST ? grid_cache : nullptr);
        if (rc) return rc;
        rz = RasterIn{w.vmodel, grid_mode, w.zbuf, w.zmask, w.gen_list, tile_w, tile_h, all_verified ? 1 : 0, all_verified ? 1 : 0};
    }
    const bool pre_any = pre_ori || pre_dir || pre_mask;
    if (pre_any && !late_fill) HIP_TRY(hipStreamWaitEvent(st, s->prefill_done, 0));
    const bool tree_late = all_verified && rz.views != nullptr;
    if (!tree_late) { int rc = wait_build(s, st); if (rc) return rc; }
    const bool direct = s->cull_direct && rz.views && grid_mode == DRT_GRID_TRUST && !mega && n >= s->cull_direct_min_rays;
    const bool park = !FUSED && !mega && rz.views && grid_mode == DRT_GRID_TRUST && pre_ori && pre_dir && pre_mask && s->cull_park;
    const Ray64 r64p = park ? Ray64{out_ori, out_dir} : r64;
    if (park) HIP_TRY(hipStreamWaitEvent(st, s->prefill_done, 0));
    {
        int64_t* rc = s->route_counts;
        rc[kRouteTotal] += 1;
        rc[kRouteRaster] += rz.views != nullptr;
        rc[kRouteTrust] += rz.views && grid_mode == DRT_GRID_TRUST;
        rc[kRouteDirect] += direct;
        rc[kRoutePark] += park;
        rc[kRouteLateFill] += late_fill;
        rc[kRouteTreeLate] += tree_late;
        rc[kRouteMega] += mega;
    }
    { StageTimer t(s, st, kStageCull);
      const unsigned n_patches = (unsigned)((n + kPathBlock - 1) / kPathBlock);
      if (rz.views && grid_mode == DRT_GRID_TRUST) {
          uint32_t* list = reinterpret_cast<uint32_t*>(p.redo);
          k_patch_list<<<(n_patches + kPathBlock - 1) / kPathBlock, kPathBlock, 0, st>>>(n_patches, tile_w, rz, list, p.count + 7);
          static const int cull_per_cu = cull_blocks_per_cu();
          const unsigned few = (unsigned)(kCullFewPerCu * s->n_cu), long_list = few * (unsigned)(kCullRun * kCullLongRuns);
          k_cull_listed<FUSED><<<cull_per_cu * s->n_cu, kPathBlock, 0, st>>>(list, p.count + 7, pc.tc.nodes, pc.tc.n_tris, o, d, valid, n, out_ori, out_dir, mask, face1, face2, p, tile_w, rz,
                                                          pc, direct, late_fill, park ? Ray64{out_ori, out_dir} : Ray64{nullptr, nullptr}, few, long_list);
      } else {
          k_cull<FUSED><<<n_patches, kPathBlock, 0, st>>>(pc.tc.nodes, pc.tc.n_tris, o, d, valid, n, out_ori, out_dir, mask, face1, face2, p, tile_w, rz,
                                                          pre_ori && pre_dir && pre_mask && sparse_faces);
      } }
    auto issue_late_fills = [&]() -> int {
        if (fs != st) { HIP_TRY(hipEventRecord(w.fill_fork, st)); HIP_TRY(hipStreamWaitEvent(fs, w.fill_fork, 0)); }
        { StageTimer tf(s, fs, kStageFill);
          if (!pre_ori) (void)hipMemsetAsync(out_ori, 0, sizeof(double) * 3 * n, fs);
          if (!pre_dir) (void)hipMemsetAsync(out_dir, 0, sizeof(double) * 3 * n, fs);
          if (!pre_mask) (void)hipMemsetAsync(mask, 0, 3 * n, fs); }
        if (fs != st) HIP_TRY(hipEventRecord(w.fill_join, fs));
        return DRT_OK;
    };
    const bool fills_after_shade1 = s->fill_after_shade1 && fs != st;
    if (late_fill && !mega && !fills_after_shade1) { int rc = issue_late_fills(); if (rc) return rc; }
    if (rz.views && grid_mode == DRT_GRID_ESTABLISH)
        k_store_models<<<(int)(n / ((int64_t)tile_w * tile_h) + 63) / 64, 64, 0, st>>>(w.vmodel, grid_cache, (int)(n / ((int64_t)tile_w * tile_h)));
    { StageTimer t(s, st, kStageTrace1);
      if (rz.views && all_verified) {
      } else if (rz.views) {
          const TraceOut out{p.r0.face, nullptr, nullptr, w.gen_list};
          launch_trace_list(kTraceClosestListed, s->grid_path, st, pc.tc, p.r0.ray, p.count + 3, out, p.redo, p.count + 4, p.count + 16, s->refill_min, s->inner_min, s->prof_stats ? s->prof_counts + kProfStages + 4 * 0 : nullptr);
      } else {
          launch_trace_list(kTraceClosest, s->grid_path, st, pc.tc, p.r0.ray, p.count + 0, TraceOut{p.r0.face, nullptr, nullptr, nullptr}, p.redo, p.count + 4, p.count + 16, s->refill_min, s->inner_min, s->prof_stats ? s->prof_counts + kProfStages + 4 * 0 : nullptr);
      } }
    if (mega) {
        if (late_fill && fs != st) HIP_TRY(hipStreamWaitEvent(st, w.fill_join, 0));
        if (pre_any) HIP_TRY(hipStreamWaitEvent(st, s->prefill_done, 0));
    }
    {
      StageTimer t(s, st, kStageShade1);
      k_shade1<FUSED><<<gs, kPathBlock, 0, st>>>(pc, o, d, out_ori, out_dir, mask, face1, face2, p, late_fill, r64p); }
    if (late_fill && !mega && fills_after_shade1) { int rc = issue_late_fills(); if (rc) return rc; }
    if (tree_late) {
        int rc = wait_build(s, st); if (rc) return rc;
        StageTimer t(s, st, kStageTrace1);
        k_gen_late<FUSED><<<kRedoGrid, kTraceBlock, 0, st>>>(pc, o, d, out_ori, out_dir, mask, face1, face2, p, w.gen_list, late_fill, r64p);
    }
    if (mega) {
        StageTimer t(s, st, kStagePath);
        k_path<FUSED><<<s->grid_mega, kPathBlock, 0, st>>>(pc, r64, out_ori, out_dir, mask, face2, p, p.count + 8, chunk_base, valid_idx,
                                                           s->mega_refill_min, s->inner_min, s->shade_min, s->prof_stats ? s->prof_counts + kProfStages + 4 * 1 : nullptr, s->prof_on);
        k_path_redo<FUSED><<<kRedoGrid, kTraceBlock, 0, st>>>(pc, o, d, face1, out_ori, out_dir, mask, face2, p, chunk_base, valid_idx);
        *n_finished = true;
        return DRT_OK;
    }
    { StageTimer t(s, st, kStageTrace2);
      unsigned long long* stats = s->prof_stats ? s->prof_counts + kProfStages + 4 * 1 : nullptr;
      if (seed2 && s->hit_seed)
          launch_trace_list(kTraceClosestSeeded, s->grid_path, st, pc.tc, p.r1.ray, p.count + 1, TraceOut{p.r1.face, nullptr, nullptr, nullptr}, p.redo, p.count + 5, p.count + 16, s->refill_min, s->inner_min, stats,
                                                                        TraceSeed{p.r1.idx, seed2, s->slot_of_face, tile_w > 0 && s->seed_tiled ? (unsigned)tile_w : 0u});
      else
          launch_trace_list(kTraceClosest, s->grid_path, st, pc.tc, p.r1.ray, p.count + 1, TraceOut{p.r1.face, nullptr, nullptr, nullptr}, p.redo, p.count + 5, p.count + 16, s->refill_min, s->inner_min, stats); }
    if (late_fill && fs != st) HIP_TRY(hipStreamWaitEvent(st, w.fill_join, 0));
    if (late_fill && pre_any) HIP_TRY(hipStreamWaitEvent(st, s->prefill_done, 0));
    { StageTimer t(s, st, kStageShade2);
      k_shade2<FUSED><<<gs, kPathBlock, 0, st>>>(pc, o, d, out_ori, out_dir, mask, face1, face2, p, park); }
    { StageTimer t(s, st, kStageTrace3);
      launch_trace_list(kTraceAny, s->grid_path, st, pc.tc, p.r2.ray, p.count + 2, TraceOut{p.r2.face, nullptr, nullptr, nullptr}, p.redo, p.count + 6, p.count + 16, s->refill_min, s->inner_min, s->prof_stats ? s->prof_counts + kProfStages + 4 * 2 : nullptr); }
    return DRT_OK;
}
}

static int fork_streams(drt_scene* s, hipStream_t st, int streams) {
    HIP_TRY(hipEventRecord(s->fork_ev, st));
    for (int k = 0; k < streams; ++k) HIP_TRY(hipStreamWaitEvent(s->sub[k].stream, s->fork_ev, 0));
    return DRT_OK;
}
static int join_streams(drt_scene* s, hipStream_t st, int streams) {
    for (int k = 0; k < streams; ++k) {
        HIP_TRY(hipEventRecord(s->sub[k].done, s->sub[k].stream));
        HIP_TRY(hipStreamWaitEvent(st, s->sub[k].done, 0));
    }
    return DRT_OK;
}

static ViewModel* sub_cache(void* d_grid_cache, int64_t b, int tile_w, int tile_h) {
    if (!d_grid_cache || tile_w <= 0 || tile_h <= 0) return nullptr;
    return static_cast<ViewModel*>(d_grid_cache) + b / ((int64_t)tile_w * tile_h);
}
static PathCtx sub_ctx(const drt_scene* s, const drt_scene::Sub& w, const double* d_verts, double ior_int, double ior_ext) {
    PathCtx pc = path_ctx(s, d_verts, ior_int, ior_ext);
    pc.tc.slow_stack = w.slow_stack;
    return pc;
}
#if defined(DRT_CHECK)
int check_counters_pipeline(unsigned long long* out4) { return read_check_counters(out4); }
#endif
int mega_blocks_per_cu() {
    int per_cu = 0;
    if (hipOccupancyMaxActiveBlocksPerMultiprocessor(&per_cu, k_path<false>, kPathBlock, 0) != hipSuccess || per_cu < 1) per_cu = 2;
    int f = 0;
    if (hipOccupancyMaxActiveBlocksPerMultiprocessor(&f, k_path<true>, kPathBlock, 0) == hipSuccess && f >= 1 && f < per_cu) per_cu = f;
    return per_cu;
}

static int32_t* take_seed(drt_scene* s, int64_t n_rays) {
    int32_t* p = s->seed.face2 && s->seed.n == n_rays ? s->seed.face2 : nullptr;
    s->seed = drt_scene::Seed{};
    return p;
}
static drt_scene::LossArm take_loss_arm(drt_scene* s, int64_t n_rays) {
    const drt_scene::LossArm a = s->loss_arm.loss && s->loss_arm.n == n_rays ? s->loss_arm : drt_scene::LossArm{};
    s->loss_arm = drt_scene::LossArm{};
    s->loss_taken = false;
    return a;
}

extern "C" {

int drt_render_seed(drt_scene_t* s, int32_t* d_seed_face2, int64_t n_rays) {
    CHECK_SCENE(s);
    if (n_rays < 0 || (d_seed_face2 == nullptr && n_rays != 0)) return fail(DRT_E_INVALID, "bad seed buffer");
    s->seed = drt_scene::Seed{d_seed_face2, n_rays};
    return DRT_OK;
}

int drt_render_loss_arm(drt_scene_t* s, const double* d_screen_pixel, const uint8_t* d_valid, double* d_loss, double* d_grad_verts, int64_t n_rays) {
    CHECK_SCENE(s);
    if (n_rays <= 0 || !d_screen_pixel || !d_valid || !d_loss || !d_grad_verts) return fail(DRT_E_INVALID, "drt_render_loss_arm: bad arguments");
    s->loss_arm = drt_scene::LossArm{d_screen_pixel, d_valid, d_loss, d_grad_verts, n_rays};
    return DRT_OK;
}

int drt_render_loss_taken(drt_scene_t* s) {
    return s && s->loss_taken ? 1 : 0;
}

static int flush_clean(drt_scene* s, hipStream_t st);
static int render_forward_impl(drt_scene_t* s, const double* d_verts, const double* d_origin, const double* d_dir, int64_t n_rays,
                               double ior_int, double ior_ext, double* d_out_ori, double* d_out_dir, uint8_t* d_mask,
                               int32_t* d_face1, int32_t* d_face2, int32_t* d_valid_idx, int64_t* d_n_valid, int tile_w, int tile_h,
                               int grid_mode, void* d_grid_cache, void* stream);
int drt_render_forward(drt_scene_t* s, const double* d_verts, const double* d_origin, const double* d_dir, int64_t n_rays,
                       double ior_int, double ior_ext, double* d_out_ori, double* d_out_dir, uint8_t* d_mask,
                       int32_t* d_face1, int32_t* d_face2, int32_t* d_valid_idx, int64_t* d_n_valid, int tile_w, int tile_h,
                       int grid_mode, void* d_grid_cache, void* stream) {
    hipStreamCaptureStatus cap0 = hipStreamCaptureStatusNone;
    const bool swap_ev = s && s->clean.rows && s->clean.captured && hipStreamIsCapturing((hipStream_t)stream, &cap0) == hipSuccess && cap0 != hipStreamCaptureStatusNone;
    if (swap_ev) std::swap(s->prefill_done, s->prefill_done_cap);
    const int rc = render_forward_impl(s, d_verts, d_origin, d_dir, n_rays, ior_int, ior_ext, d_out_ori, d_out_dir, d_mask, d_face1, d_face2, d_valid_idx,
                                       d_n_valid, tile_w, tile_h, grid_mode, d_grid_cache, stream);
    if (swap_ev) std::swap(s->prefill_done, s->prefill_done_cap);
    if (rc != DRT_OK && s) {
        s->clean = drt_scene::Clean{};
        s->n_prefill = 0;
        s->seed = drt_scene::Seed{};
        s->segs = drt_scene::Segs{};
        s->loss_arm = drt_scene::LossArm{};
        s->loss_taken = false;
    }
    return rc;
}
static int render_forward_impl(drt_scene_t* s, const double* d_verts, const double* d_origin, const double* d_dir, int64_t n_rays,
                               double ior_int, double ior_ext, double* d_out_ori, double* d_out_dir, uint8_t* d_mask,
                               int32_t* d_face1, int32_t* d_face2, int32_t* d_valid_idx, int64_t* d_n_valid, int tile_w, int tile_h,
                               int grid_mode, void* d_grid_cache, void* stream) {
    CHECK_BUILT(s);
    drt_scene::LossArm arm = take_loss_arm(s, n_rays);
    if (n_rays < 0 || n_rays > INT32_MAX) return fail(DRT_E_INVALID, "ray count out of range");
    hipStream_t st = (hipStream_t)stream;
    if (n_rays == 0) {
        if (d_n_valid) HIP_TRY(hipMemsetAsync(d_n_valid, 0, sizeof(int64_t), st));
        return DRT_OK;
    }
    if (!d_verts || !d_origin || !d_dir || !d_out_ori || !d_out_dir || !d_mask || !d_face1 || !d_face2) return fail(DRT_E_INVALID, "null pointer argument");
    if ((d_valid_idx == nullptr) != (d_n_valid == nullptr)) return fail(DRT_E_INVALID, "d_valid_idx and d_n_valid go together");
    int32_t* const seed2 = take_seed(s, n_rays);
    const Plan pl = plan_call(s, n_rays, tile_w, tile_h);
    for (int k = 0; k < pl.streams; ++k) { int rc = ensure_queues(s->sub[k], pl.size, false); if (rc) return rc; }
    HIP_TRY(hipMemsetAsync(s->vcount, 0, sizeof(unsigned), st));
    const bool segmented = d_valid_idx != nullptr && pl.count >= 2 && pl.count <= drt_scene::kMaxSeg;
    if (segmented) HIP_TRY(hipMemsetAsync(s->seg_counts, 0, sizeof(unsigned) * pl.count, st));
    s->segs = drt_scene::Segs{};
    grid_mode &= ~kIntMask;
    hipStreamCaptureStatus cap = hipStreamCaptureStatusNone;
    (void)hipStreamIsCapturing(st, &cap);
    if (arm.loss && (cap != hipStreamCaptureStatusNone || (s->mega_max_rays > 0 && n_rays - (pl.count - 1) * pl.size <= s->mega_max_rays)))
        arm = drt_scene::LossArm{};
    if (s->n_prefill && (cap == hipStreamCaptureStatusNone || (s->clean.rows && s->clean.captured))) {
        int matched = 0;
        for (int k = 0; k < s->n_prefill; ++k) {
            const drt_scene::Prefill& f = s->prefill[k];
            const int before = grid_mode;
            if (f.ptr == d_out_ori && f.bytes == (int64_t)sizeof(double) * 3 * n_rays) grid_mode |= kIntPreOri;
            if (f.ptr == d_out_dir && f.bytes == (int64_t)sizeof(double) * 3 * n_rays) grid_mode |= kIntPreDir;
            if (f.ptr == d_mask && f.bytes == 3 * n_rays) grid_mode |= kIntPreMask;
            matched += grid_mode != before;
        }
        if (matched != s->n_prefill && cap == hipStreamCaptureStatusNone) HIP_TRY(hipStreamWaitEvent(st, s->prefill_done, 0));
        s->n_prefill = 0;
    }
    bool clean_late = s->clean.rows != nullptr && (grid_mode & 3) == DRT_GRID_TRUST && d_grid_cache != nullptr;
    for (int j = 0; j < pl.count && clean_late; ++j) {
        const int64_t b = j * pl.size, n = n_rays - b < pl.size ? n_rays - b : pl.size;
        clean_late = raster_on(s, n, tile_w, tile_h);
    }
    int rc = DRT_OK;
    if (s->clean.rows && !clean_late) { rc = flush_clean(s, st); if (rc) return rc; }
    rc = fork_streams(s, st, pl.streams);
    if (rc) return rc;
    if (s->clean.rows) { rc = flush_clean(s, st); if (rc) return rc; }
    bool finish_moved = false;
    for (int j = 0; j < pl.count; ++j) {
        drt_scene::Sub& w = s->sub[j % pl.streams];
        const int64_t b = j * pl.size;
        const int64_t n = n_rays - b < pl.size ? n_rays - b : pl.size;
        const PathCtx pc = sub_ctx(s, w, d_verts, ior_int, ior_ext);
        Pipe p = pipe_of(s, w);
        int32_t* vlist = d_valid_idx;
        if (segmented) { p.valid = s->seg_counts + j; vlist = d_valid_idx + b; }
        HIP_TRY(hipMemsetAsync(w.qcount, 0, kQCount * sizeof(unsigned), w.stream));
        bool finished = false;
        rc = launch_chunk<false>(s, w, w.stream, pc, p, d_origin + 3 * b, d_dir + 3 * b, nullptr, n, d_out_ori + 3 * b, d_out_dir + 3 * b,
                                 d_mask + 3 * b, d_face1 + b, d_face2 + b, tile_w, tile_h, grid_mode, sub_cache(d_grid_cache, b, tile_w, tile_h),
                                 st, b, vlist, &finished, seed2 ? seed2 + b : nullptr);
        if (rc) return rc;
        if (!finished) {
            hipStream_t fin = w.stream;
            if (arm.loss && s->arm_finish_beside && !s->prof_serial && j + pl.streams >= pl.count) {
                HIP_TRY(hipEventRecord(w.tail, w.stream));
                HIP_TRY(hipStreamWaitEvent(st, w.tail, 0));
                fin = st;
                finish_moved = true;
            }
            StageTimer t(s, fin, kStageFinish);
            k_finish<<<8 * s->n_cu, kPathBlock, 0, fin>>>(d_out_ori + 3 * b, d_out_dir + 3 * b, d_mask + 3 * b, d_face2 + b, p, b, vlist);
        }
        if (arm.loss) {
            if (finished) return fail(DRT_E_INVALID, "armed loss: a sub-batch took the one-kernel path");
            StageTimer t(s, w.stream, kStageBackward);
            DET_LAUNCH(k_loss_bwd_armed, DRT_BWD_BPC * s->n_cu, 256, w.stream, pc, d_origin + 3 * b, d_dir + 3 * b, arm.screen_pixel + 3 * b, arm.valid + b,
                                                                 d_face1 + b, d_face2 + b, p, arm.loss, arm.grad_verts);
        }
        if (s->prof_on) k_prof_counts<<<1, 64, 0, w.stream>>>(w.qcount, (unsigned long long)n, s->prof_counts, 0, raster_on(s, n, tile_w, tile_h), finished);
    }
    rc = join_streams(s, st, pl.streams);
    if (rc) return rc;
    if (segmented) {
        for (int j = 1; j < pl.count; ++j)
            k_join_lists<<<2 * s->n_cu, 256, 0, st>>>(d_valid_idx, s->seg_counts, j, (int64_t)j * pl.size, j + 1 == pl.count, s->vcount, d_n_valid);
        if (cap == hipStreamCaptureStatusNone && !finish_moved) s->segs = drt_scene::Segs{d_valid_idx, pl.count, 0};
    } else if (d_n_valid) {
        k_store_count<<<1, 64, 0, st>>>(s->vcount, d_n_valid);
    }
    if (s->prof_on) s->prof_stream = st;
    HIP_TRY(hipGetLastError());
    s->loss_taken = arm.loss != nullptr;
    return DRT_OK;
}

int drt_prefill_zero(drt_scene_t* s, void* d_buf, int64_t bytes, void* stream) {
    CHECK_SCENE(s);
    if (!d_buf || bytes <= 0) return fail(DRT_E_INVALID, "bad buffer");
    hipStream_t st = (hipStream_t)stream;
    hipStreamCaptureStatus cs = hipStreamCaptureStatusNone;
    if (hipStreamIsCapturing(st, &cs) == hipSuccess && cs != hipStreamCaptureStatusNone) return fail(DRT_E_INVALID, "drt_prefill_zero: not while a graph is being captured");
    if (s->n_prefill >= 3) s->n_prefill = 0;
    hipStream_t bs = s->build_stream;
    HIP_TRY(hipEventRecord(s->prefill_fork, st));
    HIP_TRY(hipStreamWaitEvent(bs, s->prefill_fork, 0));
    { StageTimer t(s, bs, kStageFill);
      HIP_TRY(hipMemsetAsync(d_buf, 0, (size_t)bytes, bs)); }
    HIP_TRY(hipEventRecord(s->prefill_done, bs));
    s->prefill[s->n_prefill].ptr = d_buf; s->prefill[s->n_prefill].bytes = bytes; ++s->n_prefill;
    return DRT_OK;
}

static int flush_clean(drt_scene* s, hipStream_t st) {
    const drt_scene::Clean c = s->clean;
    s->clean = drt_scene::Clean{};
    if (!c.rows) return DRT_OK;
    { StageTimer t(s, st, kStageFill);
      k_unwrite_rows<<<4 * s->n_cu, 256, 0, st>>>(c.ori, c.dir, c.mask, c.rows, c.n_rows, c.n); }
    HIP_TRY(hipGetLastError());
    HIP_TRY(hipEventRecord(s->prefill_done, st));
    return DRT_OK;
}

int drt_outputs_clean(drt_scene_t* s, double* d_out_ori, double* d_out_dir, uint8_t* d_mask, int64_t n_rays,
                      const int32_t* d_valid_idx, const int64_t* d_n_valid, void* stream) {
    CHECK_SCENE(s);
    if (n_rays <= 0 || !d_out_ori || !d_out_dir || !d_mask || !d_valid_idx || !d_n_valid) return fail(DRT_E_INVALID, "bad arguments");
    hipStream_t st = (hipStream_t)stream;
    hipStreamCaptureStatus cs = hipStreamCaptureStatusNone;
    const bool capturing = hipStreamIsCapturing(st, &cs) == hipSuccess && cs != hipStreamCaptureStatusNone;
    if (capturing && (s->n_prefill || s->clean.rows)) return fail(DRT_E_INVALID, "drt_outputs_clean: zeroings requested outside the capture are still pending");
    if (s->n_prefill) {
        HIP_TRY(hipStreamWaitEvent(st, s->prefill_done, 0));
        s->n_prefill = 0;
    }
    if (s->clean.rows) { int rc = flush_clean(s, st); if (rc) return rc; }
    s->clean = drt_scene::Clean{d_out_ori, d_out_dir, d_mask, n_rays, d_valid_idx, d_n_valid, capturing};
    s->prefill[0].ptr = d_out_ori; s->prefill[0].bytes = (int64_t)sizeof(double) * 3 * n_rays;
    s->prefill[1].ptr = d_out_dir; s->prefill[1].bytes = (int64_t)sizeof(double) * 3 * n_rays;
    s->prefill[2].ptr = d_mask;    s->prefill[2].bytes = 3 * n_rays;
    s->n_prefill = 3;
    return DRT_OK;
}

int drt_outputs_cancel(drt_scene_t* s) {
    CHECK_SCENE(s);
    if (s->clean.rows) { s->clean = drt_scene::Clean{}; s->n_prefill = 0; }
    return DRT_OK;
}

int drt_prefill_wait(drt_scene_t* s, void* stream) {
    CHECK_SCENE(s);
    HIP_TRY(hipStreamWaitEvent((hipStream_t)stream, s->prefill_done, 0));
    s->n_prefill = 0;
    return DRT_OK;
}

}

#define DET_LAUNCH_IN(kern, grid, block, st, ...)                                               \
    do {                                                                                        \
        if (det_mode()) kern<true, INPUTS><<<grid, block, 0, st>>>(__VA_ARGS__);                \
        else kern<false, INPUTS><<<grid, block, 0, st>>>(__VA_ARGS__);                          \
    } while (0)
template <bool INPUTS>
static int render_backward(drt_scene_t* s, const double* d_verts, const double* d_origin, const double* d_dir, int64_t n_rays,
                           double ior_int, double ior_ext, const int32_t* d_face1, const int32_t* d_face2,
                           const int32_t* d_valid_idx, const int64_t* d_n_valid,
                           const double* d_grad_out_ori, const double* d_grad_out_dir, double* d_grad_verts, InputGrads in, void* stream) {
    CHECK_BUILT(s);
    if (n_rays < 0 || n_rays > INT32_MAX) return fail(DRT_E_INVALID, "ray count out of range");
    if (n_rays == 0 || (!d_grad_out_ori && !d_grad_out_dir)) return DRT_OK;
    if (!d_verts || !d_origin || !d_dir || !d_face1 || !d_face2 || !d_grad_verts) return fail(DRT_E_INVALID, "null pointer argument");
    if ((d_valid_idx == nullptr) != (d_n_valid == nullptr)) return fail(DRT_E_INVALID, "d_valid_idx and d_n_valid go together");
    hipStream_t st = (hipStream_t)stream;
    const PathCtx pc = path_ctx(s, d_verts, ior_int, ior_ext);
    if (d_valid_idx) {
        StageTimer t(s, st, kStageBackward);
        DET_LAUNCH_IN(k_render_bwd, DRT_BWD_BPC * s->n_cu, 256, st, pc, d_origin, d_dir, d_face1, d_face2, d_grad_out_ori, d_grad_out_dir, d_grad_verts,
                                                   d_valid_idx, nullptr, d_n_valid, in);
    } else {
        drt_scene::Sub& w = s->sub[0];
        const int64_t chunk = n_rays < s->chunk_rays ? n_rays : s->chunk_rays;
        int rc = ensure_queues(w, chunk, false);
        if (rc) return rc;
        for (int64_t b = 0; b < n_rays; b += chunk) {
            const int64_t n = n_rays - b < chunk ? n_rays - b : chunk;
            HIP_TRY(hipMemsetAsync(s->vcount, 0, sizeof(unsigned), st));
            { StageTimer t(s, st, kStageCollect);
              k_collect_valid<<<grid_for(n, kPathBlock, 8 * s->n_cu), kPathBlock, 0, st>>>(d_face2 + b, n, b, w.q_idx[0], s->vcount); }
            { StageTimer t(s, st, kStageBackward);
              DET_LAUNCH_IN(k_render_bwd, DRT_BWD_BPC * s->n_cu, 256, st, pc, d_origin, d_dir, d_face1, d_face2, d_grad_out_ori, d_grad_out_dir, d_grad_verts,
                                                         w.q_idx[0], s->vcount, nullptr, in); }
            if (s->prof_on) k_prof_counts_bwd<<<1, 64, 0, st>>>(s->vcount, (unsigned long long)n, s->prof_counts);
        }
    }
    if (s->prof_on) s->prof_stream = st;
    HIP_TRY(hipGetLastError());
    return DRT_OK;
}

template <bool INPUTS>
static int render_backward_ray_loss(drt_scene_t* s, const double* d_verts, const double* d_origin, const double* d_dir, int64_t n_rays,
                                    double ior_int, double ior_ext, const int32_t* d_face1, const int32_t* d_face2,
                                    const int32_t* d_rows, const uint32_t* d_n_rows, const double* d_screen_pixel, const double* d_scale,
                                    double* d_grad_verts, InputGrads in, void* stream) {
    CHECK_BUILT(s);
    if (n_rays < 0 || n_rays > INT32_MAX) return fail(DRT_E_INVALID, "ray count out of range");
    if (n_rays == 0) return DRT_OK;
    if (!d_verts || !d_origin || !d_dir || !d_face1 || !d_face2 || !d_rows || !d_n_rows || !d_screen_pixel || !d_scale || !d_grad_verts)
        return fail(DRT_E_INVALID, "null pointer argument");
// ... 173 lines not shown
```

drt_amd/csrc/drt_raster.hip:

```cpp
#include "drt_device.h"

__global__ void __launch_bounds__(64) k_fit_views(const double* __restrict__ origin, const double* __restrict__ dir, int w, int h,
                                                  ViewModel* __restrict__ views) {
    __shared__ ViewModel vm;
    const int64_t base = (int64_t)blockIdx.x * w * h;
    if (threadIdx.x == 0) {
        const int64_t i00 = base, iW0 = base + (w - 1), i0H = base + (int64_t)(h - 1) * w, iWH = i0H + (w - 1);
        if (fit_view_model(load_d3(origin, i00), load_d3(dir, i00), load_d3(dir, iW0), load_d3(dir, i0H), load_d3(dir, iWH),
                           (double)(w - 1), (double)(h - 1), vm))
            vm.ok = 1;
    }
    __syncthreads();
    bool good = vm.ok != 0;
    if (good) {
        const int sx = (int)(threadIdx.x & 7), sy = (int)(threadIdx.x >> 3);
        const int x = (int)(((int64_t)(w - 1) * sx) / 7), y = (int)(((int64_t)(h - 1) * sy) / 7);
        const int64_t i = base + (int64_t)y * w + x;
        good = view_verify(vm, load_d3(origin, i), load_d3(dir, i), (double)x, (double)y);
    }
    const bool all_good = __ballot(good) == ~0ull;
    if (threadIdx.x == 0) {
        vm.ok = all_good ? 1 : 0;
        vm.all = vm.ok;
        views[blockIdx.x] = vm;
    }
}

__device__ __forceinline__ uint32_t canary_hash(uint32_t a, uint32_t b, uint32_t c) {
    uint32_t h = a * 0x9E3779B1u ^ (b + 0x7F4A7C15u) * 0x85EBCA6Bu ^ (c + 0x165667B1u) * 0xC2B2AE35u;
    h ^= h >> 15; h *= 0x2C1B3C6Du; h ^= h >> 12; h *= 0x297A2D39u; h ^= h >> 15;
    return h;
}
__global__ void __launch_bounds__(64) k_check_views(const double* __restrict__ origin, const double* __restrict__ dir, int w, int h,
                                                    ViewModel* __restrict__ cache, ViewModel* __restrict__ views, unsigned salt, unsigned* __restrict__ salt_ctr) {
    __shared__ ViewModel vm;
    __shared__ unsigned s_ctr;
    const int64_t base = (int64_t)blockIdx.x * w * h;
    if (threadIdx.x == 0) {
        vm = cache[blockIdx.x];
        s_ctr = salt_ctr ? __hip_atomic_load(salt_ctr, __ATOMIC_RELAXED, __HIP_MEMORY_SCOPE_AGENT) : 0u;
        if (salt_ctr && blockIdx.x == 0) atomicAdd(salt_ctr, 1u);
    }
    __syncthreads();
    if (salt) salt = (salt ^ (s_ctr * 0x9E3779B1u)) | 1u;
    const bool trusted = vm.ok && vm.all;
    const int sx = (int)(threadIdx.x & 7), sy = (int)(threadIdx.x >> 3);
    const int x = (int)(((int64_t)(w - 1) * sx) / 7), y = (int)(((int64_t)(h - 1) * sy) / 7);
    const int64_t i = base + (int64_t)y * w + x;
    bool good = trusted && view_verify(vm, load_d3(origin, i), load_d3(dir, i), (double)x, (double)y);
    if (good && salt) {
        const uint32_t hx = canary_hash(salt, blockIdx.x, threadIdx.x), hy = canary_hash(salt ^ 0xA5A5A5A5u, threadIdx.x, blockIdx.x);
        const int cx = (int)(((uint64_t)hx * (uint64_t)w) >> 32), cy = (int)(((uint64_t)hy * (uint64_t)h) >> 32);
        const int64_t ci = base + (int64_t)cy * w + cx;
        good = view_verify(vm, load_d3(origin, ci), load_d3(dir, ci), (double)cx, (double)cy);
    }
    if (__ballot(good) == ~0ull) {
        if (threadIdx.x == 0) views[blockIdx.x] = vm;
        return;
    }
    __syncthreads();
    if (threadIdx.x == 0) {
        const int64_t i00 = base, iW0 = base + (w - 1), i0H = base + (int64_t)(h - 1) * w, iWH = i0H + (w - 1);
        if (fit_view_model(load_d3(origin, i00), load_d3(dir, i00), load_d3(dir, iW0), load_d3(dir, i0H), load_d3(dir, iWH),
                           (double)(w - 1), (double)(h - 1), vm))
            vm.ok = 1;
    }
    __syncthreads();
    good = vm.ok != 0 && view_verify(vm, load_d3(origin, i), load_d3(dir, i), (double)x, (double)y);
    const bool all_good = __ballot(good) == ~0ull;
    if (threadIdx.x == 0) {
        vm.ok = all_good ? 1 : 0;
        vm.all = 0;
        views[blockIdx.x] = vm;
        if (trusted) { cache[blockIdx.x].ok = 0; cache[blockIdx.x].all = 0; }
    }
}

__device__ __forceinline__ void raster_test(const TriRec& t, f3 o32, const double* __restrict__ dir, int64_t i, int64_t slot,
                                            unsigned long long* __restrict__ zbuf, uint32_t* __restrict__ zmask) {
    const f3 d32 = to_f32(load_d3(dir, i));
    float tt;
    if (!tri_hit_mt(o32, d32, f3{t.v0x, t.v0y, t.v0z}, f3{t.e1x, t.e1y, t.e1z}, f3{t.e2x, t.e2y, t.e2z}, tt)) return;
    const unsigned long long key = raster_key(tt, t.face);
    if (key >= zbuf[slot]) return;
    if (!hit_point_in_box(o32, d32, tt, f3{t.v0x, t.v0y, t.v0z}, f3{t.e1x, t.e1y, t.e1z}, f3{t.e2x, t.e2y, t.e2z}, t.margin)) return;
    atomicMin(&zbuf[slot], key);
    const uint32_t bit = 1u << ((i >> 6) & 31);
    if (!(zmask[i >> 11] & bit)) atomicOr(&zmask[i >> 11], bit);
}

struct BigItem { int32_t view, tri, x0, y0, nx, ny; };

struct RasterLane {
    TriRec tri;
    int32_t x0, y0, nx, end;
};

__device__ __forceinline__ float wave_uniform(float v) { return __int_as_float(__builtin_amdgcn_readfirstlane(__float_as_int(v))); }

constexpr int kRasterCostAt = 32;
template <bool DEAL, bool RECORD, int pass>
__global__ void __launch_bounds__(256, 8) k_raster(const TriRec* __restrict__ tris, int n_tris, ViewModel* views, int n_views,
                                                   const double* __restrict__ dir, int w, int h,
                                                   unsigned long long* __restrict__ zbuf, uint32_t* __restrict__ zmask,
                                                   BigItem* __restrict__ big, unsigned* big_count,
                                                   const DealPos* __restrict__ table ) {
    constexpr unsigned big_cap = drt_scene::kBigCap;
    __shared__ RasterLane s_lane[256];
    const int lane = threadIdx.x & 63;
    RasterLane* const wl = s_lane + (threadIdx.x & ~63);
    const unsigned n_waves = gridDim.x * 4u, wave = __builtin_amdgcn_readfirstlane(blockIdx.x * 4u + (threadIdx.x >> 6));
    const unsigned runs_per_view = ((unsigned)n_tris + 63u) / 64u, n_runs = runs_per_view * (unsigned)n_views;
    int cur_view = -1;
    float minv32[9] = {};
    f3 o32{0.0f, 0.0f, 0.0f};
    DealRange g{wave, n_runs, 0u, 0xFFFFFFFFu};
    if (DEAL) {
        const DealPos b0 = wave == 0 ? DealPos{0, 0} : raster_deal_clamp(table[wave], n_runs);
        const DealPos b1 = wave + 1 >= n_waves ? DealPos{n_runs, 0} : raster_deal_clamp(table[wave + 1], n_runs);
        g = raster_deal_range(b0, b1);
        g.end = min(g.end, n_runs);
    }
    for (; g.run < g.end; DEAL ? raster_deal_next(g) : (void)(g.run += n_waves)) {
        const unsigned run = g.run;
        const int view = (int)(run / runs_per_view);
        const int k = (int)(run - (unsigned)view * runs_per_view) * 64 + lane;
        const DealSlice sl = DEAL ? raster_deal_slice(g) : DealSlice{0u, 0xFFFFFFFFu, true};
        const bool ok = __hip_atomic_load(&views[view].ok, __ATOMIC_RELAXED, __HIP_MEMORY_SCOPE_AGENT) != 0;
        if (!RECORD && !ok) continue;
        if (ok && view != cur_view) {
            cur_view = view;
            for (int q = 0; q < 9; ++q) minv32[q] = wave_uniform((float)views[view].minv[q]);
            o32 = f3{wave_uniform((float)views[view].o[0]), wave_uniform((float)views[view].o[1]), wave_uniform((float)views[view].o[2])};
        }
        int count = 0;
        __builtin_amdgcn_wave_barrier();
        if ((!RECORD || ok) && k < n_tris) {
            const TriRec tri = tris[k];
            if ((pass == 1) == tri_faces_away(o32, tri)) {
                ViewModel vm;
                for (int q = 0; q < 9; ++q) vm.minv[q] = (double)minv32[q];
                const PixelBox box = project_tri_box(vm, o32, tri, w, h);
                if (box.unsafe) {
                    if (sl.owner) __hip_atomic_store(&views[view].ok, 0, __ATOMIC_RELAXED, __HIP_MEMORY_SCOPE_AGENT);
                } else if (box.x0 <= box.x1 && box.y0 <= box.y1) {
                    const int nx = box.x1 - box.x0 + 1, ny = box.y1 - box.y0 + 1;
                    const int64_t cnt = (int64_t)nx * ny;
                    if (cnt > kRasterMaxPerLane) {
                        const int rows_per = max(1, kRasterBandPixels / nx), n_bands = (ny + rows_per - 1) / rows_per;
                        const unsigned slot = sl.owner ? atomicAdd(big_count, (unsigned)n_bands) : 0u;
                        if (!sl.owner) {
                        } else if (slot <= big_cap && (unsigned)n_bands <= big_cap - slot) {
                            for (int b = 0; b < n_bands; ++b)
                                big[slot + b] = BigItem{view, k, box.x0, box.y0 + b * rows_per, nx, min(rows_per, ny - b * rows_per)};
                        } else {
                            __hip_atomic_store(&views[view].ok, 0, __ATOMIC_RELAXED, __HIP_MEMORY_SCOPE_AGENT);
                            for (unsigned q = slot; q < big_cap; ++q) big[q] = BigItem{view, k, 0, 0, 0, 0};
                        }
                    } else {
                        count = (int)cnt;
                        wl[lane].tri = tri;
                        wl[lane].x0 = box.x0; wl[lane].y0 = box.y0; wl[lane].nx = nx;
                    }
                }
            }
        }
        int end = count;
        for (int off = 1; off < 64; off <<= 1) {
            const int v = __shfl_up(end, off);
            if (lane >= off) end += v;
        }
        const int total = __builtin_amdgcn_readlane(end, 63);
        if (RECORD && sl.owner && lane == 0) big_count[kRasterCostAt + 2 * run + pass] = (unsigned)total;
        const int stop = (int)min((unsigned)total, sl.hi);
        if (sl.lo >= (unsigned)stop) continue;
        wl[lane].end = end;
        __builtin_amdgcn_wave_barrier();
        const int64_t base = (int64_t)view * w * h;
        for (int item0 = (int)sl.lo; item0 < stop; item0 += 64) {
            const int item = item0 + lane;
            if (item >= stop) break;
            int lo = 0, hi = 63;
            while (lo < hi) {
                const int mid = (lo + hi) >> 1;
                if (wl[mid].end > item) hi = mid; else lo = mid + 1;
            }
            const RasterLane& ow = wl[lo];
            const int local = item - (lo == 0 ? 0 : wl[lo - 1].end);
            const int row = (int)(((float)local + 0.5f) / (float)ow.nx);
            const int x = ow.x0 + (local - row * ow.nx), y = ow.y0 + row;
            raster_test(ow.tri, o32, dir, base + (int64_t)y * w + x, raster_slot((unsigned)x, (unsigned)(view * h + y), (unsigned)w), zbuf, zmask);
        }
    }
}

constexpr int kDealBlock = 1024;
__device__ __forceinline__ uint64_t shfl_up_u64(uint64_t v, int off) {
    return ((uint64_t)(uint32_t)__shfl_up((int)(v >> 32), off) << 32) | (uint32_t)__shfl_up((int)(uint32_t)v, off);
}
__global__ void __launch_bounds__(kDealBlock) k_raster_deal(const unsigned* __restrict__ counts , DealPos* __restrict__ table,
                                                            unsigned n_runs, unsigned n_waves, uint32_t c_fixed) {
    __shared__ uint64_t s_all[kDealBlock / 64], s_before[kDealBlock / 64], s_own[kDealBlock / 64];
    const unsigned pass = blockIdx.y, tid = threadIdx.x, lane = tid & 63, wid = tid >> 6;
    DealPos* const tab = table + pass * (n_waves + 1);
    const unsigned* const cost = counts + kRasterCostAt + pass;
    const unsigned first = blockIdx.x * kDealBlock, run = first + tid;
    constexpr unsigned kMost = 64u * (unsigned)kRasterMaxPerLane;
    uint64_t all = 0, before = 0, own = 0;
    for (unsigned base = 0; base < n_runs; base += kDealBlock) {
        const unsigned r = base + tid;
        const uint64_t wgt = r < n_runs ? raster_deal_weight(min(cost[2 * r], kMost), c_fixed) : 0;
        all += wgt;
        if (base < first) before += wgt;
        if (base == first) own = wgt;
    }
    uint64_t incl = own;
    for (int off = 1; off < 64; off <<= 1) {
        const uint64_t v = shfl_up_u64(incl, off), va = shfl_up_u64(all, off), vb = shfl_up_u64(before, off);
        if ((int)lane >= off) { incl += v; all += va; before += vb; }
    }
    if (lane == 63) { s_all[wid] = all; s_before[wid] = before; s_own[wid] = incl; }
    __syncthreads();
    uint64_t total = 0, start = 0;
    for (unsigned q = 0; q < kDealBlock / 64; ++q) {
        total += s_all[q];
        start += s_before[q];
        if (q < wid) start += s_own[q];
    }
    const uint64_t with = start + incl;
    if (run < n_runs) raster_deal_place(tab, run, with - own, with, total, n_waves, c_fixed);
    if (run == 0) tab[n_waves] = DealPos{n_runs, 0};
}

__global__ void __launch_bounds__(256) k_raster_big(const TriRec* __restrict__ tris, const ViewModel* __restrict__ views,
                                                    const double* __restrict__ dir, int w, int h,
                                                    unsigned long long* __restrict__ zbuf, uint32_t* __restrict__ zmask,
                                                    const BigItem* __restrict__ big, const unsigned* __restrict__ big_count, unsigned big_cap) {
    const unsigned n = min(*big_count, big_cap);
    const unsigned n_waves = gridDim.x * 4u;
    const int lane = threadIdx.x & 63;
    for (unsigned e = __builtin_amdgcn_readfirstlane(blockIdx.x * 4u + (threadIdx.x >> 6)); e < n; e += n_waves) {
        const BigItem it = big[e];
        const ViewModel& vm = views[it.view];
        const TriRec t = tris[it.tri];
        const f3 o32 = to_f32(d3{vm.o[0], vm.o[1], vm.o[2]});
        const int64_t base = (int64_t)it.view * w * h;
        const int cnt = it.nx * it.ny;
        for (int p = lane; p < cnt; p += 64) {
            const int row = (int)(((float)p + 0.5f) / (float)it.nx);
            int y = it.y0 + row, x = it.x0 + (p - row * it.nx);
            if (x >= it.x0 + it.nx) { x -= it.nx; ++y; } else if (x < it.x0) { x += it.nx; --y; }
            raster_test(t, o32, dir, base + (int64_t)y * w + x, raster_slot((unsigned)x, (unsigned)(it.view * h + y), (unsigned)w), zbuf, zmask);
        }
    }
}

__global__ void k_fill_u64(unsigned long long* __restrict__ p, int64_t n, unsigned long long v) {
    for (int64_t i = blockIdx.x * (int64_t)blockDim.x + threadIdx.x; i < n; i += (int64_t)gridDim.x * blockDim.x) p[i] = v;
}

constexpr int64_t kRasterDealMaxRuns = (int64_t)1 << 18;
static int64_t raster_runs(int64_t n_tris, int n_views) { return (n_tris + 63) / 64 * n_views; }

int ensure_raster(drt_scene* s, drt_scene::Sub& w, int64_t n_rays, int n_views, hipStream_t st) {
    if (n_rays > w.z_cap) {
        (void)hipFree(w.zbuf); (void)hipFree(w.zmask);
        w.zbuf = nullptr; w.zmask = nullptr; w.z_cap = 0;
        const int64_t words = (n_rays + 2047) / 2048 + 1;
        HIP_TRY(hipMalloc(&w.zbuf, sizeof(unsigned long long) * n_rays));
        HIP_TRY(hipMalloc(&w.zmask, sizeof(uint32_t) * words));
        k_fill_u64<<<4 * s->n_cu, 256, 0, st>>>(w.zbuf, n_rays, kRasterEmpty);
        HIP_TRY(hipMemsetAsync(w.zmask, 0, sizeof(uint32_t) * words, st));
        w.z_cap = n_rays;
    }
    if (n_views > w.vm_cap) {
        (void)hipFree(w.vmodel); w.vmodel = nullptr; w.vm_cap = 0;
        HIP_TRY(hipMalloc(&w.vmodel, sizeof(ViewModel) * n_views));
        w.vm_cap = n_views;
    }
    if (!w.big) HIP_TRY(hipMalloc(&w.big, sizeof(BigItem) * drt_scene::kBigCap));
    drt_scene::Sub::Deal& dl = w.deal;
    if (!w.big_count) {
        const int n_waves = 8 * s->n_cu * 4;
        HIP_TRY(hipMalloc(&w.big_count, sizeof(unsigned) * (kRasterCostAt + (s->raster_deal ? 2 * kRasterDealMaxRuns : 0))));
        if (s->raster_deal) {
            HIP_TRY(hipMalloc(&dl.table, sizeof(DealPos) * 2 * (n_waves + 1)));
            dl.cap_runs = kRasterDealMaxRuns; dl.cap_waves = n_waves;
        }
    }
    return DRT_OK;
}

int launch_raster(drt_scene* s, drt_scene::Sub& w, hipStream_t st, const double* d_origin, const double* d_dir, int n_views, int iw, int ih,
                  ViewModel* trusted) {
    const int n = (int)s->n_faces;
    HIP_TRY(hipMemsetAsync(w.big_count, 0, sizeof(unsigned), st));
    if (trusted) k_check_views<<<n_views, 64, 0, st>>>(d_origin, d_dir, iw, ih, trusted, w.vmodel,
                                                        s->grid_canary ? (++s->canary_salt ? s->canary_salt : ++s->canary_salt) : 0u,
                                                        s->vcount + 3);
    else k_fit_views<<<n_views, 64, 0, st>>>(d_origin, d_dir, iw, ih, w.vmodel);
    if (n > 0) {
        drt_scene::Sub::Deal& dl = w.deal;
        const int grid = 8 * s->n_cu;
        const int64_t n_runs = raster_runs(n, n_views);
        const bool record = s->raster_deal && dl.table && n_runs > 0 && n_runs >= s->raster_deal_min_runs && n_runs <= dl.cap_runs && grid * 4 == dl.cap_waves;
        const bool dealt = record && dl.complete && dl.dir == d_dir && dl.n_views == n_views && dl.iw == iw && dl.ih == ih && dl.n_tris == n && dl.grid == grid;
        s->raster_deal_counts[dealt ? 0 : 1] += 2;
        for (int pass = 0; pass < 2; ++pass) {
            auto* const kern = pass == 0 ? (dealt ? k_raster<true, true, 0> : record ? k_raster<false, true, 0> : k_raster<false, false, 0>)
                                         : (dealt ? k_raster<true, true, 1> : record ? k_raster<false, true, 1> : k_raster<false, false, 1>);
            kern<<<grid, 256, 0, st>>>(s->tris_flat, n, w.vmodel, n_views, d_dir, iw, ih, w.zbuf, w.zmask, reinterpret_cast<BigItem*>(w.big), w.big_count,
                                       dealt ? dl.table + pass * (dl.cap_waves + 1) : nullptr);
            if (pass == 0) {
                k_raster_big<<<8 * s->n_cu, 256, 0, st>>>(s->tris_flat, w.vmodel, d_dir, iw, ih, w.zbuf, w.zmask,
                                                           reinterpret_cast<const BigItem*>(w.big), w.big_count, drt_scene::kBigCap);
                HIP_TRY(hipMemsetAsync(w.big_count, 0, sizeof(unsigned), st));
            }
        }
        k_raster_big<<<8 * s->n_cu, 256, 0, st>>>(s->tris_flat, w.vmodel, d_dir, iw, ih, w.zbuf, w.zmask,
                                                   reinterpret_cast<const BigItem*>(w.big), w.big_count, drt_scene::kBigCap);
        dl.complete = false;
        if (record) {
            k_raster_deal<<<dim3((unsigned)((n_runs + kDealBlock - 1) / kDealBlock), 2), kDealBlock, 0, st>>>(w.big_count, dl.table, (unsigned)n_runs, (unsigned)(grid * 4), s->raster_deal_fixed);
            dl.dir = d_dir; dl.n_views = n_views; dl.iw = iw; dl.ih = ih; dl.n_tris = n; dl.grid = grid;
            dl.complete = true;
        }
    }
    HIP_TRY(hipGetLastError());
    return DRT_OK;
}
```

drt_amd/csrc/drt_scene.h:

```cpp
#pragma once
#include <hip/hip_runtime.h>

#include <cstdarg>
#include <cstdio>
#include <cstdlib>
#include <cstring>
#include <new>
#include <vector>

#include "../../include/drt_hip.h"
#include "drt_common.h"
#include "drt_closest.h"
#include "drt_edge.h"
#include "drt_fixed.h"
#include "drt_lbvh.h"
#include "drt_path.h"
#include "drt_raster.h"
#include "drt_shade.h"
#include "drt_traverse.h"
#include "drt_tri.h"

using namespace drt;


int fail(int code, const char* fmt, ...);
#define HIP_TRY(expr)                                                                         \
    do {                                                                                      \
        hipError_t e_ = (expr);                                                               \
        if (e_ != hipSuccess) return fail(DRT_E_HIP, "%s: %s", #expr, hipGetErrorString(e_)); \
    } while (0)

constexpr int kTraceBlock = 128;
#ifndef DRT_STACK_FAST
#define DRT_STACK_FAST 19
#endif
constexpr int kStackFast = DRT_STACK_FAST;
static_assert(kStackFast >= 3, "FastStack keeps four spare entries (kStackFast + 1 rows) above its usable depth");
constexpr int kStackTotal = 192;
constexpr int kStackSlowDev = kStackTotal - kStackFast;
constexpr int kQCount = 64;
constexpr int kRedoGrid = 64;
constexpr int kTraceGridMax = 4096;
constexpr int64_t kChunkRays = 1 << 26;

constexpr int kSortBlock = 256, kSortItems = 8, kSortTile = kSortBlock * kSortItems, kRadix = 256;

enum { kRouteTotal = 0, kRouteRaster, kRouteTrust, kRouteDirect, kRoutePark, kRouteLateFill, kRouteTreeLate, kRouteMega };
enum { kStageBuild = 0, kStageCull, kStageTrace1, kStageShade1, kStageTrace2, kStageShade2, kStageTrace3, kStageFinish, kStageCollect, kStageBackward, kStageLossBwdFused, kStageRaster, kStageFill, kStagePath, kProfStages };
static_assert(kProfStages == DRT_PROFILE_STAGES, "include/drt_hip.h");

struct BuildParams {
    float lox, loy, loz;
    float ix, iy, iz;
    float pad;
    int32_t reserved;
    MortonPlan plan;
};

struct drt_scene {
    int device = 0;
    int64_t n_faces = 0, n_verts = 0;
    int64_t cap_faces = 0, cap_verts = 0;
    int32_t* faces = nullptr;
    float* verts = nullptr;
    Node* nodes = nullptr;
    Node4Q* wide = nullptr;
    int32_t *range_lo = nullptr, *range_hi = nullptr;
    TriRec* tris = nullptr;
    TriRec* tris_flat = nullptr;
    int32_t* slot_of_face = nullptr;
    struct Seed { int32_t* face2 = nullptr; int64_t n = 0; } seed;
    struct LossArm { const double* screen_pixel = nullptr; const uint8_t* valid = nullptr; double* loss = nullptr; double* grad_verts = nullptr; int64_t n = 0; } loss_arm;
    bool loss_taken = false;
    hipStream_t build_stream = nullptr;
    hipEvent_t build_fork = nullptr, build_done = nullptr;
    bool build_pending = false;
    bool order_valid = false;
    int sorted_buf = 0;
    bool cull_direct = true;
    bool cull_park = true;
    int64_t cull_direct_min_rays = (int64_t)1 << 25;
    int64_t route_counts[8] = {0};
    int tree_mode = 0, rebuild_every = 1, since_full = 0;
    bool topology_fixed = false;
    uint32_t* bounds_acc = nullptr;
    bool async_build = true;
    uint32_t *keys[2] = {nullptr, nullptr}, *idx[2] = {nullptr, nullptr};
    uint32_t* hist = nullptr;
    int32_t *parent_inner = nullptr, *parent_leaf = nullptr;
    uint32_t* flags = nullptr;
    BuildParams* params = nullptr;
    int32_t* slow_stack = nullptr;
    unsigned long long* scratch = nullptr;
    int32_t *b1_list = nullptr, *b1_redo = nullptr;
    unsigned* b1_count = nullptr;
    int64_t b1_cap = 0;
    struct Sub {
        hipStream_t stream = nullptr;
        hipEvent_t done = nullptr;
        hipEvent_t tail = nullptr;
        hipEvent_t fill_fork = nullptr, fill_join = nullptr;
        int32_t* q_idx[3] = {nullptr, nullptr, nullptr};
        float* q_ray[3] = {nullptr, nullptr, nullptr};
        int32_t* q_face[3] = {nullptr, nullptr, nullptr};
        int32_t *tmp_face1 = nullptr, *tmp_face2 = nullptr;
        unsigned* qcount = nullptr;
        double* ray64 = nullptr;
        int64_t ray64_cap = 0;
        int32_t* redo = nullptr;
        int32_t* slow_stack = nullptr;
        int64_t q_cap = 0, fused_cap = 0;
        unsigned long long* zbuf = nullptr;
        uint32_t* zmask = nullptr;
        int64_t z_cap = 0;
        ViewModel* vmodel = nullptr;
        int vm_cap = 0;
        void* big = nullptr;
        unsigned* big_count = nullptr;
        int32_t* gen_list = nullptr;
        struct Deal {
            DealPos* table = nullptr;
            int64_t cap_runs = 0;
            int cap_waves = 0;
            const double* dir = nullptr;
            int n_views = 0, iw = 0, ih = 0, n_tris = 0, grid = 0;
            bool complete = false;
        } deal;
    };
    static constexpr unsigned kBigCap = 1u << 20;
    static constexpr int kMaxSub = 4;
    Sub sub[kMaxSub];
    int n_sub = 2;
    int sub_per_stream = 1;
    int64_t min_sub_rays = 1 << 24;
    hipEvent_t fork_ev = nullptr;
    struct Clean { double* ori = nullptr; double* dir = nullptr; uint8_t* mask = nullptr; int64_t n = 0; const int32_t* rows = nullptr; const int64_t* n_rows = nullptr;
                   bool captured = false;  } clean;
    static constexpr int kMaxSeg = 32;
    unsigned* seg_counts = nullptr;
    struct Segs { const int32_t* list = nullptr; int n = 0; int stream0 = 0; } segs;
    struct Prefill { const void* ptr = nullptr; int64_t bytes = 0; };
    Prefill prefill[3];
    int n_prefill = 0;
    hipEvent_t prefill_fork = nullptr, prefill_done = nullptr, prefill_done_cap = nullptr;
    unsigned* vcount = nullptr;
    uint32_t* vh_list = nullptr;
    int64_t vh_cap = 0;
    bool prof_on = false;
    uint32_t prof_mask = ~0u;
    bool prof_stats = false;
    bool prof_serial = false;
    std::vector<hipEvent_t> prof_ev;
    std::vector<int> prof_stage;
    size_t prof_used = 0;
    size_t prof_dropped = 0;
    unsigned long long* prof_counts = nullptr;
    hipStream_t prof_stream = nullptr;
    int n_cu = 256;
    int grid_trace = 2048;
    int grid_path = 2048;
    int64_t trace_stats[12] = {0};
    int grid_mega = 1024;
    int64_t mega_max_rays = 0;
    int shade_min = 8;
    int mega_refill_min = 16;
    int refill_min = 32;
    int inner_min = 24;
    int64_t chunk_rays = kChunkRays;

    bool fill_after_shade1 = true;
    bool fill_overlap = true;
    bool grid_canary = true;
    unsigned canary_salt = 0;
    bool seed_tiled = true;
    bool arm_finish_beside = true;
    bool hit_seed = true;
    bool use_raster = true;
    bool raster_deal = true;
    int64_t raster_deal_min_runs = 16384;
    uint32_t raster_deal_fixed = kRasterDealFixed;
    int64_t raster_deal_counts[2] = {0, 0};
    bool built = false;
    void* paths_ws = nullptr;
    void* image_loss_ws = nullptr;
    void* image_views = nullptr;
};


int query_blocks_per_cu();
int pipeline_blocks_per_cu();
int mega_blocks_per_cu();

int ensure_raster(drt_scene* s, drt_scene::Sub& w, int64_t n_rays, int n_views, hipStream_t st);
int launch_raster(drt_scene* s, drt_scene::Sub& w, hipStream_t st, const double* d_origin, const double* d_dir, int n_views, int iw, int ih,
                  ViewModel* trusted);

void paths_free(drt_scene* s);
void image_loss_free(drt_scene* s);
void image_views_free(drt_scene* s);

int ensure_slow_stack(drt_scene* s, hipStream_t st);
bool det_mode();
#define DET_LAUNCH(kern, grid, block, st, ...)                                        \
    do {                                                                              \
        if (det_mode()) kern<true><<<grid, block, 0, st>>>(__VA_ARGS__);              \
        else kern<false><<<grid, block, 0, st>>>(__VA_ARGS__);                        \
    } while (0)
int check_counters_pipeline(unsigned long long* out4);
int check_counters_trace(unsigned long long* out4);

void scene_free_mesh(drt_scene* s);
int ensure_capacity(drt_scene* s, int64_t n_faces, int64_t n_verts);
int rebuild(drt_scene* s, hipStream_t st, const uint32_t* acc);
int wait_build(drt_scene* s, hipStream_t st);

inline int grid_for(int64_t n, int block, int cap) {
    int64_t g = (n + block - 1) / block;
    if (g < 1) g = 1;
    if (g > cap) g = cap;
    return (int)g;
}

inline TraceCtx trace_ctx(const drt_scene* s) { return TraceCtx{s->wide, s->tris, (int)s->n_faces, s->slow_stack}; }
inline PathCtx path_ctx(const drt_scene* s, const double* d_verts, double ior_int, double ior_ext) {
    return PathCtx{trace_ctx(s), s->faces, d_verts, ior_int, ior_ext};
}

#define CHECK_SCENE(s)                                                        \
    do {                                                                      \
        if (!(s)) return fail(DRT_E_INVALID, "null scene");                   \
        HIP_TRY(hipSetDevice((s)->device));                                   \
    } while (0)
#define CHECK_BUILT(s)                                                                          \
    do {                                                                                        \
        CHECK_SCENE(s);                                                                         \
        if (!(s)->built) return fail(DRT_E_INVALID, "no mesh: call drt_update_mesh first");     \
    } while (0)

struct StageTimer {
    drt_scene* s; hipStream_t st; bool on;
    StageTimer(drt_scene* s_, hipStream_t st_, int stage) : s(s_), st(st_), on(false) {
        if (!s->prof_on || !((s->prof_mask >> stage) & 1u)) return;
        if (s->prof_used + 2 > s->prof_ev.size() && !grow()) { ++s->prof_dropped; return; }
        on = true;
        s->prof_stage[s->prof_used / 2] = stage;
        if (!s->prof_stream) s->prof_stream = st;
        (void)hipEventRecord(s->prof_ev[s->prof_used], st);
    }
    bool grow() {
        constexpr size_t kMaxEvents = (size_t)1 << 22;
        const size_t want = s->prof_ev.size() ? 2 * s->prof_ev.size() : 8192;
        if (want > kMaxEvents) return false;
        const size_t old = s->prof_ev.size();
        s->prof_ev.resize(want, nullptr);
        s->prof_stage.resize(want / 2, 0);
        for (size_t k = old; k < want; ++k)
            if (hipEventCreate(&s->prof_ev[k]) != hipSuccess) {
                for (size_t j = old; j < k; ++j) (void)hipEventDestroy(s->prof_ev[j]);
                s->prof_ev.resize(old); s->prof_stage.resize(old / 2);
                return false;
            }
        return true;
    }
    ~StageTimer() {
        if (!on) return;
        (void)hipEventRecord(s->prof_ev[s->prof_used + 1], st);
        s->prof_used += 2;
    }
};
```

drt_amd/optix_mesh.py:

```python
from __future__ import annotations

import ctypes

import torch

from . import _lib


_raw_stream = getattr(torch._C, "_cuda_getCurrentRawStream", None)
_raw_device = getattr(torch._C, "_cuda_getDevice", None)


def _stream():
    if _raw_stream is not None and _raw_device is not None:
        return ctypes.c_void_p(_raw_stream(_raw_device()))
    return ctypes.c_void_p(torch.cuda.current_stream().cuda_stream)


class _NoContext:
    def __enter__(self):
        return None

    def __exit__(self, *exc):
        return False


_NO_CONTEXT = _NoContext()


def _on(device):
    idx = device if isinstance(device, int) else getattr(device, "index", None)
    if idx is not None and _raw_device is not None and _raw_device() == idx:
        return _NO_CONTEXT
    return torch.cuda.device(device)


def _require(t, dtype, cols, name):
    if not isinstance(t, torch.Tensor):
        raise TypeError(f"{name} must be a torch.Tensor")
    if t.dtype != dtype:
        raise RuntimeError(f"{name} must be {dtype}, got {t.dtype}")
    if t.dim() != 2 or t.size(1) != cols:
        raise RuntimeError(f"{name} must have shape [N,{cols}], got {tuple(t.shape)}")
    if not t.is_cuda:
        raise RuntimeError(f"{name} must be a GPU tensor (there is no CPU tracer in the product path)")
    return t.contiguous()


class optix_mesh:
    def __init__(self, cuda_device=0):
        if not torch.cuda.is_available():
            raise _lib.DrtError("no GPU visible: drt_amd needs an MI355X (gfx950) device")
        self.device = int(cuda_device)
        h = ctypes.c_void_p()
        with _on(self.device):
            _lib.check(_lib.lib().drt_create(self.device, ctypes.byref(h)))
        self._h = h
        self.builded = False
        self.n_faces = 0
        self.n_verts = 0

    def __del__(self):
        h = getattr(self, "_h", None)
        if h:
            try:
                _lib.lib().drt_destroy(h)
            except Exception:
                pass
            self._h = None

    def _check_device(self, t, name):
        if t.device.index != self.device:
            raise RuntimeError(f"{name} is on {t.device}, this tracer is bound to cuda:{self.device}")

    def update_mesh(self, F, V):
        F = _require(F, torch.int32, 3, "F")
        V = _require(V, torch.float32, 3, "V")
        self._check_device(F, "F")
        self._check_device(V, "V")
        with _on(self.device):
            _lib.check(_lib.lib().drt_update_mesh(self._h, F.data_ptr(), F.size(0), V.data_ptr(), V.size(0), _stream()))
        self.n_faces, self.n_verts = F.size(0), V.size(0)
        self.builded = True

    def update_vert(self, V):
        assert self.builded, "update_mesh must be called first"
        V = _require(V, torch.float32, 3, "V")
        self._check_device(V, "V")
        with _on(self.device):
            _lib.check(_lib.lib().drt_update_vert(self._h, V.data_ptr(), V.size(0), _stream()))

    def update_vert_f64(self, V):
        assert self.builded, "update_mesh must be called first"
        V = _require(V.detach(), torch.float64, 3, "V")
        self._check_device(V, "V")
        with _on(self.device):
            _lib.check(_lib.lib().drt_update_vert_f64(self._h, V.data_ptr(), V.size(0), _stream()))

    def intersect(self, Ray):
        assert self.builded, "update_mesh must be called first"
        Ray = _require(Ray, torch.float32, 6, "Ray")
        self._check_device(Ray, "Ray")
        n = Ray.size(0)
        T = torch.empty(n, dtype=torch.float32, device=Ray.device)
        ID = torch.empty(n, dtype=torch.int32, device=Ray.device)
        with _on(self.device):
            _lib.check(_lib.lib().drt_intersect(self._h, Ray.data_ptr(), n, T.data_ptr(), ID.data_ptr(), _stream()))
        return [T, ID]

    def intersect_any(self, Ray):
        assert self.builded, "update_mesh must be called first"
        Ray = _require(Ray, torch.float32, 6, "Ray")
        self._check_device(Ray, "Ray")
        n = Ray.size(0)
        hit = torch.empty(n, dtype=torch.uint8, device=Ray.device)
        with _on(self.device):
            _lib.check(_lib.lib().drt_intersect_any(self._h, Ray.data_ptr(), n, hit.data_ptr(), _stream()))
        return hit.view(torch.bool)

    def intersect_bruteforce(self, Ray):
        Ray = _require(Ray, torch.float32, 6, "Ray")
        n = Ray.size(0)
        T = torch.empty(n, dtype=torch.float32, device=Ray.device)
        ID = torch.empty(n, dtype=torch.int32, device=Ray.device)
        with _on(self.device):
            _lib.check(_lib.lib().drt_intersect_bruteforce(self._h, Ray.data_ptr(), n, T.data_ptr(), ID.data_ptr(), _stream()))
        return [T, ID]

    def closest_point(self, points, want_face=True, want_point=False):
        assert self.builded, "update_mesh must be called first"
        points = _require(points, torch.float64, 3, "points")
        self._check_device(points, "points")
        n = points.size(0)
        dist = torch.empty(n, dtype=torch.float64, device=points.device)
        face = torch.empty(n, dtype=torch.int32, device=points.device) if want_face else None
        closest = torch.empty(n, 3, dtype=torch.float64, device=points.device) if want_point else None
        with _on(self.device):
            _lib.check(_lib.lib().drt_closest_point(self._h, points.data_ptr(), n, dist.data_ptr(), face.data_ptr() if want_face else None,
                                                    closest.data_ptr() if want_point else None, _stream()))
        return dist, face, closest

    def check(self):
        v = ctypes.c_int64()
        hgt = ctypes.c_int32()
        wide = ctypes.c_int32()
        with _on(self.device):
            _lib.check(_lib.lib().drt_bvh_check(self._h, _stream(), ctypes.byref(v), ctypes.byref(hgt), ctypes.byref(wide)))
        self.wide_depth = wide.value
        return v.value, hgt.value

    def tree_mode(self, mode, rebuild_every=1):
        _lib.check(_lib.lib().drt_tree_mode(self._h, int(mode), int(rebuild_every)))

    def build_params(self):
        out = (ctypes.c_float * 7)()
        with _on(self.device):
            _lib.check(_lib.lib().drt_build_params(self._h, out, _stream()))
        return list(out)

    def sorted_faces(self):
        out = torch.empty(self.n_faces, dtype=torch.int32, device=f"cuda:{self.device}")
        with _on(self.device):
            _lib.check(_lib.lib().drt_bvh_sorted_faces(self._h, out.data_ptr(), _stream()))
        return out

    NODE_DTYPE = [(k, "<f4") for k in ("c0lox", "c0hix", "c0loy", "c0hiy", "c1lox", "c1hix", "c1loy", "c1hiy", "c0loz", "c0hiz", "c1loz", "c1hiz")] + \
                 [(k, "<i4") for k in ("child0", "child1", "pad0", "pad1")]
    NODE4Q_DTYPE = [(k, "<f4") for k in ("ox", "oy", "oz", "sx", "sy", "sz")] + \
                   [(k, "u1", (4,)) for k in ("qlox", "qloy", "qloz", "qhix", "qhiy", "qhiz")] + [("child", "<i4", (4,))]
    TRIREC_DTYPE = [("v0", "<f4", (3,)), ("face", "<i4"), ("e1", "<f4", (3,)), ("margin", "<f4"), ("e2", "<f4", (3,)), ("pad1", "<f4")]
    PARAMS_DTYPE = dict(names=["lo", "inv", "pad", "reserved", "axis", "pos", "bits", "plan_pad"], offsets=[0, 12, 24, 28, 32, 62, 92, 95], itemsize=100,
                        formats=[("<f4", (3,)), ("<f4", (3,)), "<f4", "<i4", ("u1", (30,)), ("u1", (30,)), ("u1", (3,)), ("u1", (3,))])
    TREE_ARRAYS = ("keys", "order", "nodes", "parent_inner", "parent_leaf", "range_lo", "range_hi", "wide", "tris", "tris_flat", "slot_of_face", "params")

    def tree_arrays(self, names=None):
        import numpy as np
        assert self.builded, "update_mesh must be called first"
        n = self.n_faces
        inner = max(n - 1, 1) if n else 0
        shape = {"keys": (np.uint32, n), "order": (np.uint32, n), "nodes": (np.dtype(self.NODE_DTYPE), inner), "parent_inner": (np.int32, inner),
                 "parent_leaf": (np.int32, n), "range_lo": (np.int32, inner), "range_hi": (np.int32, inner), "wide": (np.dtype(self.NODE4Q_DTYPE), inner),
                 "tris": (np.dtype(self.TRIREC_DTYPE), n), "tris_flat": (np.dtype(self.TRIREC_DTYPE), n), "slot_of_face": (np.int32, n),
                 "params": (np.dtype(self.PARAMS_DTYPE), 1)}
        out = {}
        with _on(self.device):
            for name in (self.TREE_ARRAYS if names is None else names):
                dtype, count = shape[name]
                nbytes = np.dtype(dtype).itemsize * count
                buf = torch.empty(nbytes, dtype=torch.uint8, device=f"cuda:{self.device}")
                _lib.check(_lib.lib().drt_bvh_export(self._h, self.TREE_ARRAYS.index(name), buf.data_ptr(), nbytes, _stream()))
                out[name] = buf.cpu().numpy().view(dtype)
        out_params = out.get("params")
        if out_params is not None:
            out["params"] = out_params[0]
        return out

    STAGES = ("build", "cull", "trace1", "shade1", "trace2", "shade2", "trace3", "finish", "collect", "backward", "loss_bwd_fused", "raster", "fill", "path")

    def profile_enable(self, on=1):
        with _on(self.device):
            _lib.check(_lib.lib().drt_profile_enable(self._h, int(on)))

    def profile_select(self, stages=None):
        mask = 0xFFFFFFFF if stages is None else sum(1 << self.STAGES.index(k) for k in stages)
        _lib.check(_lib.lib().drt_profile_select(self._h, mask))

    def profile_read(self):
        n = len(self.STAGES)
        ms = (ctypes.c_double * n)()
        launches = (ctypes.c_int64 * n)()
        items = (ctypes.c_int64 * n)()
        with _on(self.device):
            _lib.check(_lib.lib().drt_profile_read(self._h, ms, launches, items))
        return {k: (ms[i], launches[i], items[i]) for i, k in enumerate(self.STAGES)}

    ROUTES = ("total", "raster", "trust", "direct", "park", "late_fill", "tree_late", "mega")

    def route_counts(self):
        out = (ctypes.c_int64 * len(self.ROUTES))()
        _lib.check(_lib.lib().drt_route_counts(self._h, out))
        return dict(zip(self.ROUTES, out))

    def raster_deal_counts(self):
        out = (ctypes.c_int64 * 2)()
        _lib.check(_lib.lib().drt_raster_deal_counts(self._h, out))
        return tuple(out)

    def trace_stats(self):
        out = (ctypes.c_int64 * 12)()
        _lib.check(_lib.lib().drt_profile_trace_stats(self._h, out))
        return {f"trace{k + 1}": tuple(out[4 * k:4 * k + 4]) for k in range(3)}
```

include/drt_hip.h:

```cpp
#ifndef DRT_HIP_H
#define DRT_HIP_H

#include <stdint.h>

#ifdef __cplusplus
extern "C" {
#endif

#define DRT_OK            0
#define DRT_E_INVALID    -1
#define DRT_E_HIP        -2
#define DRT_E_NOMEM      -3

typedef struct drt_scene drt_scene_t;

const char* drt_last_error(void);
int drt_version(void);

#define DRT_FX_BYTES_PER_VALUE 24
int drt_deterministic(int on);
int drt_fx_finalize(const void* d_cells, int64_t n, double* d_out, int accumulate, void* stream);
int drt_fx_add(void* d_dst_cells, const void* d_src_cells, int64_t n, void* stream);
int drt_fx_to_limbs(const void* d_cells, int64_t n, int64_t* d_limbs, void* stream);
int drt_fx_from_limbs(const int64_t* d_limbs, int64_t n, void* d_cells, void* stream);
// ... 24 lines not shown

#define DRT_GRID_NONE 0
#define DRT_GRID_ESTABLISH 1
#define DRT_GRID_TRUST 2
#define DRT_GRID_CACHE_BYTES 104
#define DRT_GRID_SPARSE_FACES 16
#define DRT_GRID_ALL_VERIFIED 32
int drt_render_forward(drt_scene_t* s, const double* d_verts, const double* d_origin,
                       const double* d_dir, int64_t n_rays, double ior_int, double ior_ext,
                       double* d_out_ori, double* d_out_dir, uint8_t* d_mask,
                       int32_t* d_face1, int32_t* d_face2,
                       int32_t* d_valid_idx, int64_t* d_n_valid, int tile_w, int tile_h,
                       int grid_mode, void* d_grid_cache, void* stream);
int drt_render_backward(drt_scene_t* s, const double* d_verts, const double* d_origin,
                        const double* d_dir, int64_t n_rays, double ior_int, double ior_ext,
                        const int32_t* d_face1, const int32_t* d_face2,
                        const int32_t* d_valid_idx, const int64_t* d_n_valid,
                        const double* d_grad_out_ori, const double* d_grad_out_dir,
                        double* d_grad_verts, void* stream);
int drt_render_backward_inputs(drt_scene_t* s, const double* d_verts, const double* d_origin,
                               const double* d_dir, int64_t n_rays, double ior_int, double ior_ext,
                               const int32_t* d_face1, const int32_t* d_face2,
                               const int32_t* d_valid_idx, const int64_t* d_n_valid,
                               const double* d_grad_out_ori, const double* d_grad_out_dir,
                               double* d_grad_verts, double* d_grad_origin, double* d_grad_dir,
                               double* d_grad_ior, void* stream);

int drt_render_paths_forward(drt_scene_t* s, const double* d_verts, const double* d_origin,
                             const double* d_dir, int64_t n_rays, double ior_int, double ior_ext,
                             int max_bounces, int reflect,
                             double* d_out_ori, double* d_out_dir, uint8_t* d_mask,
                             int32_t* d_tape, uint8_t* d_hits,
                             int32_t* d_valid_idx, int64_t* d_n_valid, void* stream);
int drt_render_paths_backward(drt_scene_t* s, const double* d_verts, const double* d_origin,
                              const double* d_dir, int64_t n_rays, double ior_int, double ior_ext,
                              int max_bounces, int reflect,
                              const int32_t* d_tape, const uint8_t* d_hits,
                              const int32_t* d_valid_idx, const int64_t* d_n_valid,
                              const double* d_grad_out_ori, const double* d_grad_out_dir,
                              double* d_grad_verts, void* stream);

int drt_render_paths_ray_loss_fused(drt_scene_t* s, const double* d_verts, const double* d_origin, const double* d_dir,
                                    const double* d_screen_pixel, const uint8_t* d_valid, int64_t n_rays,
                                    double ior_int, double ior_ext, int max_bounces, int reflect,
                                    double* d_loss, double* d_grad_verts, int64_t* d_n_valid, void* stream);

#define DRT_LAW_REFLECT 1
#define DRT_LAW_SNELL 2
int drt_render_paths_law_forward(drt_scene_t* s, const double* d_verts, const double* d_origin,
                                 const double* d_dir, int64_t n_rays, double ior_int, double ior_ext,
                                 int max_bounces, int law_flags,
                                 double* d_out_ori, double* d_out_dir, uint8_t* d_mask,
                                 int32_t* d_tape, uint8_t* d_hits,
                                 int32_t* d_valid_idx, int64_t* d_n_valid, void* stream);
int drt_render_paths_law_backward(drt_scene_t* s, const double* d_verts, const double* d_origin,
                                  const double* d_dir, int64_t n_rays, double ior_int, double ior_ext,
                                  int max_bounces, int law_flags,
                                  const int32_t* d_tape, const uint8_t* d_hits,
                                  const int32_t* d_valid_idx, const int64_t* d_n_valid,
                                  const double* d_grad_out_ori, const double* d_grad_out_dir,
                                  double* d_grad_verts, void* stream);
int drt_render_paths_law_ray_loss_fused(drt_scene_t* s, const double* d_verts, const double* d_origin, const double* d_dir,
                                        const double* d_screen_pixel, const uint8_t* d_valid, int64_t n_rays,
                                        double ior_int, double ior_ext, int max_bounces, int law_flags,
                                        double* d_loss, double* d_grad_verts, int64_t* d_n_valid, void* stream);

int drt_render_paths_law_ray_loss_ior_fused(drt_scene_t* s, const double* d_verts, const double* d_origin, const double* d_dir,
                                            const double* d_screen_pixel, const uint8_t* d_valid, int64_t n_rays,
                                            double ior_int, double ior_ext, int max_bounces, int law_flags,
                                            double* d_loss, double* d_grad_verts, double* d_grad_ior, int64_t* d_n_valid, void* stream);

int drt_ray_loss(const double* d_out_ori, const double* d_out_dir, const uint8_t* d_mask,
                 const double* d_screen_pixel, const uint8_t* d_valid, int64_t n_rays,
                 double* d_loss, double* d_grad_out_dir,
                 int32_t* d_list, uint32_t* d_n_list, void* stream);
int drt_ray_loss_listed(const double* d_out_ori, const double* d_out_dir, const double* d_screen_pixel,
                        const uint8_t* d_valid, const int32_t* d_paths, const int64_t* d_n_paths, int64_t n_rays,
                        double* d_loss, int32_t* d_rows, uint32_t* d_n_rows, void* stream);
int drt_scale_rows3(double* d_x, const int32_t* d_list, const uint32_t* d_n_list,
                    const double* d_scale, void* stream);

int drt_prefill_zero(drt_scene_t* s, void* d_buf, int64_t bytes, void* stream);
int drt_prefill_wait(drt_scene_t* s, void* stream);
int drt_outputs_clean(drt_scene_t* s, double* d_out_ori, double* d_out_dir, uint8_t* d_mask, int64_t n_rays,
                      const int32_t* d_valid_idx, const int64_t* d_n_valid, void* stream);
int drt_outputs_cancel(drt_scene_t* s);
int drt_render_seed(drt_scene_t* s, int32_t* d_seed_face2, int64_t n_rays);
int drt_ray_loss_listed_grad(drt_scene_t* s, const double* d_verts, const double* d_origin, const double* d_dir, int64_t n_rays,
                             double ior_int, double ior_ext, const int32_t* d_face1, const int32_t* d_face2,
                             const double* d_screen_pixel, const uint8_t* d_valid, const int32_t* d_paths, const int64_t* d_n_paths,
                             double* d_loss, double* d_grad_verts, void* stream);
int drt_ray_loss_listed_grad_split(drt_scene_t* s, const double* d_verts, const double* d_origin, const double* d_dir, int64_t n_rays,
                                   double ior_int, double ior_ext, const int32_t* d_face1, const int32_t* d_face2,
                                   const double* d_screen_pixel, const uint8_t* d_valid, const int32_t* d_paths, const int64_t* d_n_paths,
                                   double* d_loss, double* d_grad_verts, void* stream);
int drt_render_loss_arm(drt_scene_t* s, const double* d_screen_pixel, const uint8_t* d_valid, double* d_loss, double* d_grad_verts,
                        int64_t n_rays);
int drt_render_loss_taken(drt_scene_t* s);
int drt_render_backward_ray_loss(drt_scene_t* s, const double* d_verts, const double* d_origin,
                                 const double* d_dir, int64_t n_rays, double ior_int, double ior_ext,
                                 const int32_t* d_face1, const int32_t* d_face2,
                                 const int32_t* d_rows, const uint32_t* d_n_rows,
                                 const double* d_screen_pixel, const double* d_scale,
                                 double* d_grad_verts, void* stream);
int drt_render_backward_ray_loss_inputs(drt_scene_t* s, const double* d_verts, const double* d_origin,
                                        const double* d_dir, int64_t n_rays, double ior_int, double ior_ext,
                                        const int32_t* d_face1, const int32_t* d_face2,
                                        const int32_t* d_rows, const uint32_t* d_n_rows,
                                        const double* d_screen_pixel, const double* d_scale,
                                        double* d_grad_verts, double* d_grad_origin, double* d_grad_dir,
                                        double* d_grad_ior, void* stream);

int drt_render_ray_loss_fused(drt_scene_t* s, const double* d_verts, const double* d_origin,
                              const double* d_dir, const double* d_screen_pixel,
                              const uint8_t* d_valid, int64_t n_rays, double ior_int,
                              double ior_ext, double* d_loss, double* d_grad_verts,
                              int64_t* d_n_valid, int tile_w, int tile_h,
                              int grid_mode, void* d_grid_cache, void* stream);

int drt_dihedral_forward(const double* d_verts, const int64_t* d_e2f, int64_t n_edges, double* d_cos, void* stream);
int drt_dihedral_backward(const double* d_verts, const int64_t* d_e2f, int64_t n_edges,
                          const double* d_grad_cos, double* d_grad_verts, void* stream);
int drt_sm_loss_fused(const double* d_verts, const int64_t* d_e2f, int64_t n_edges, double* d_loss,
                      double* d_grad_verts, void* stream);

int drt_silhouette_flags(const double* d_verts, const int64_t* d_e2f, int64_t n_edges,
                         const double* d_origin3, uint8_t* d_flags, void* stream);
int drt_edge_sample_forward(drt_scene_t* s, const double* d_verts, const int64_t* d_edges, int64_t n_edges,
                            const double* d_camera, const double* d_origin3, int64_t* d_index,
                            float* d_f, uint8_t* d_keep, int resx, int resy, const uint8_t* d_flags, void* stream);
int drt_edge_sample_backward(const double* d_verts, const int64_t* d_edges, int64_t n_edges,
                             const double* d_camera, const float* d_f, const double* d_coef,
                             int detach_depth, double* d_grad_verts, void* stream);
int drt_edge_sample_backward_rows(const double* d_verts, const int64_t* d_edges, int64_t n_edges,
                                  const double* d_camera, const float* d_f, const int64_t* d_rows, int64_t n_rows,
                                  const float* d_g, int detach_depth, double* d_grad_verts, void* stream);

int drt_vh_term(const int64_t* d_index, const uint8_t* d_keep, int64_t n_edges, const double* d_soft_mask, int resx, int resy,
                double* d_loss, double* d_dterm, void* stream);
int drt_edge_sample_backward_term(const double* d_verts, const int64_t* d_edges, int64_t n_edges, const double* d_camera, const float* d_f,
                                  const double* d_dterm, const double* d_g, int detach_depth, double* d_grad_verts, void* stream);

int drt_vh_loss_fused(drt_scene_t* s, const double* d_verts, const int64_t* d_edges, const int64_t* d_e2f,
                      int64_t n_edges, int n_views, const double* const* d_cameras,
                      const double* const* d_origins, const double* const* d_soft_masks, int resx, int resy,
                      int detach_depth, double* d_loss, double* d_grad_verts, void* stream);

int drt_closest_point(drt_scene_t* s, const double* d_points, int64_t n, double* d_dist, int32_t* d_face,
                      double* d_closest, void* stream);

int drt_rm_split_mark(const int64_t* d_faces, int64_t n_faces, const double* d_verts, double max_len, uint8_t* d_flag, void* stream);
int drt_rm_split_plan(const int64_t* d_faces, int64_t n_faces, const int64_t* d_vf_start, const int64_t* d_vf_face, const uint8_t* d_flag,
                      const int64_t* d_rank, int64_t n_verts, int64_t* d_mid_of_slot, int64_t* d_count, void* stream);
int drt_rm_split_faces(const int64_t* d_faces, int64_t n_faces, const int64_t* d_mid_of_slot, double* d_verts, const int64_t* d_offset,
                       int64_t* d_faces_out, void* stream);
int drt_rm_vertex_faces(const int64_t* d_faces, int64_t n_faces, int64_t n_verts, int32_t* d_count, int64_t* d_vf_start, int64_t* d_vf_face,
                        const double* d_verts, double* d_vn, const int32_t* d_live, void* stream);
int drt_rm_vertex_normals(const int64_t* d_faces, const double* d_verts, const int64_t* d_vf_start, const int64_t* d_vf_face, int64_t n_verts,
                          double* d_vn, void* stream);
int drt_rm_collapse_apply(const int64_t* d_cand, int64_t n_cand, const uint8_t* d_ok, const int64_t* d_edges, int64_t* d_faces, double* d_verts,
                          const int64_t* d_vf_start, const int64_t* d_vf_face, int64_t n_verts, double min_len, uint32_t seed, int round, const double* d_length,
                          uint64_t* d_lock, uint8_t* d_f_alive, uint8_t* d_v_alive, uint8_t* d_dirty, int sub_rounds, int32_t* d_n_done, const int32_t* d_live, void* stream);
int drt_rm_collapse_eval_all(const int64_t* d_faces, int64_t n_faces, const double* d_verts, const double* d_vn, const int64_t* d_vf_start,
                             const int64_t* d_vf_face, double min_len, double max_len, int max_q, int64_t* d_edge_snap, double* d_length,
                             uint8_t* d_ok, int32_t* d_n_query, double* d_query, int32_t* d_list_item, double* d_list_point, uint32_t* d_list_count,
                             int64_t list_cap, const int32_t* d_live, void* stream);
int drt_rm_surface_filter_list(drt_scene_t* s, uint8_t* d_ok, const int32_t* d_list_item, const double* d_list_point, const uint32_t* d_list_count,
                               int64_t list_cap, double max_dist, const int32_t* d_live, void* stream);
int drt_rm_surface_filter(drt_scene_t* s, uint8_t* d_ok, const int32_t* d_n_query, const double* d_query, int64_t n_items, int max_q,
                          double max_dist, const int32_t* d_live, void* stream);
int drt_rm_closest_near(drt_scene_t* s, const double* d_points, int64_t n, double hint_radius, double* d_closest, void* stream);
int drt_rm_kill_faces(int64_t* d_faces, uint8_t* d_f_alive, int64_t n_faces, const int32_t* d_live, void* stream);
int drt_rm_round_end(int32_t* d_ctl, int tail_cut, void* stream);
int drt_rm_flip_eval(const int64_t* d_faces, int64_t n_faces, const double* d_verts, const double* d_vn, const int64_t* d_vf_start,
                     const int64_t* d_vf_face, double max_len, uint8_t* d_ok, int64_t* d_quad, double* d_query, const int32_t* d_live, void* stream);
int drt_rm_flip_apply(int64_t n_items, const uint8_t* d_ok, const int64_t* d_quad, int64_t* d_faces, int64_t n_verts, int round, uint64_t* d_lock,
                      uint8_t* d_dirty, int sub_rounds, int32_t* d_n_done, const int32_t* d_live, void* stream);
int drt_rm_smooth_target(const int64_t* d_faces, const double* d_verts, const int64_t* d_vf_start, const int64_t* d_vf_face, int64_t n_verts,
                         double* d_target, void* stream);
int drt_rm_face_agreement(const int64_t* d_faces, const double* d_verts, const double* d_vn, int64_t n_faces, double* d_a0, void* stream);
int drt_rm_move_check(const int64_t* d_faces, double* d_verts, const double* d_old, const double* d_vn, const double* d_a0, int64_t n_faces,
                      int64_t n_verts, uint8_t* d_revert, int32_t* d_n_bad, void* stream);

#define DRT_REMESH_SPLIT 1u
#define DRT_REMESH_COLLAPSE 2u
#define DRT_REMESH_FLIP 4u
#define DRT_REMESH_SMOOTH 8u
#define DRT_REMESH_REPROJECT 16u
#define DRT_REMESH_CHECK_DIST 32u
#define DRT_REMESH_ALL 63u
typedef struct drt_mesh_buf drt_mesh_buf_t;
int drt_remesh_isotropic(const double* verts, int64_t n_verts, const int32_t* faces, int64_t n_faces,
                         double target_len, int iterations, double max_surf_dist, unsigned flags,
                         drt_mesh_buf_t** out);
int drt_mesh_buf_size(const drt_mesh_buf_t* b, int64_t* n_verts, int64_t* n_faces, int64_t* stats4);
int drt_mesh_buf_copy(const drt_mesh_buf_t* b, double* verts, int32_t* faces);
void drt_mesh_buf_free(drt_mesh_buf_t* b);

int drt_limit_sgd_step(double* d_param, double* d_grad, double* d_buf, int64_t n, double lr, double momentum,
                       int nesterov, int first, double max_abs, void* stream);
int drt_limit_sgd_step3(double* d_param, double* d_grad, double* d_buf, int64_t n, double lr, double momentum, int nesterov, int first,
                        double max_abs, const double* d_terms, const double* d_w3, const double* d_loss_parts, double* d_loss_total, void* stream);
int drt_weight_terms3(const double* d_terms, const double* d_w3, int64_t n, double* d_out, void* stream);
int drt_limit_sgd_step_total(double* d_param, double* d_grad, double* d_buf, int64_t n, double lr, double momentum, int nesterov, int first,
                             double max_abs, const double* d_w3, const double* d_loss_parts, double* d_loss_total, void* stream);
int drt_fx_limbs_limit_sgd_step3(const int64_t* d_limbs, int64_t n, double* d_param, double* d_grad, double* d_buf, double lr, double momentum,
                                 int nesterov, int first, double max_abs, const double* d_w3, double* d_loss_parts, double* d_loss_total, void* stream);
int drt_internal_stream(drt_scene_t* s, int which, void** out);

int64_t drt_edge_tables_workspace(int64_t n_faces);
int drt_edge_tables(const int64_t* d_faces, int64_t n_faces, const double* d_verts, int64_t n_verts,
                    void* d_workspace, int64_t* d_edges, int64_t* d_e2f, int32_t* d_row2edge,
                    double* d_mean_len, int32_t* d_status, void* stream);
int drt_subdivide_midpoint(const int64_t* d_faces, int64_t n_faces, const double* d_verts, int64_t n_verts,
                           const int64_t* d_edges, int64_t n_edges, const int32_t* d_row2edge, int round_f32,
                           int64_t* d_faces_out, double* d_verts_out, void* stream);

int drt_hull_field(const uint8_t* d_masks, int n_views, int height, int width, const double* d_proj, double lo_x, double lo_y, double lo_z,
                   double cell, int nx, int ny, int nz, int keep_outside, float* d_field, void* stream);
int drt_hull_mark(const float* d_field, int nx, int ny, int nz, double level, uint8_t* d_edge_mask, uint8_t* d_n_vert, uint8_t* d_n_tri,
                  void* stream);
int drt_hull_emit(const float* d_field, int nx, int ny, int nz, double lo_x, double lo_y, double lo_z, double cell, double level,
                  const uint8_t* d_edge_mask, const int32_t* d_v_inc, const int32_t* d_t_inc, int64_t n_verts, int64_t n_faces,
                  double* d_verts, int32_t* d_faces, void* stream);

int drt_decode_patterns(const uint8_t* d_frames, const uint8_t* d_background, int64_t background_view_stride, int n_views, int height, int width,
                        int tex_h, int tex_w, int min_contrast, int mask_shift, const double* d_screens, int zero_outside_mask, int16_t* d_codes,
                        uint8_t* d_contrast, uint8_t* d_mask, uint8_t* d_covered, double* d_positions, void* stream);

int drt_render_image(drt_scene_t* s, const double* d_verts, const double* camera21, int height, int width, int y0, int y1, int supersample,
                     double ior_int, double ior_ext, int max_bounces, int law_flags, int fresnel, const double* screen9,
                     const float* d_texture, int tex_h, int tex_w, int channels, const double* fill_void, const double* fill_invalid,
                     float* d_image, float* d_hit, float* d_through, void* stream);

int drt_render_image_loss(drt_scene_t* s, const double* d_verts, const double* camera21, int height, int width, int y0, int y1, int supersample,
                          double ior_int, double ior_ext, int max_bounces, int law_flags, int fresnel, const double* screen9,
                          const float* d_texture, int tex_h, int tex_w, int channels, const double* fill_void, const double* fill_invalid,
                          const float* d_target, const float* d_weight, double* d_loss, double* d_grad_verts, double* d_grad_ior, float* d_image,
                          int64_t* d_count, void* stream);

int drt_render_image_loss_screen(drt_scene_t* s, const double* d_verts, const double* camera21, int height, int width, int y0, int y1, int supersample,
                                 double ior_int, double ior_ext, int max_bounces, int law_flags, int fresnel, const double* screen9,
                                 const float* d_texture, int tex_h, int tex_w, int channels, const double* fill_void, const double* fill_invalid,
                                 const float* d_target, const float* d_weight, double* d_loss, double* d_grad_verts, double* d_grad_ior, float* d_image,
                                 int64_t* d_count, double* d_grad_screen, double* d_grad_texture, void* stream);

int drt_render_image_loss_camera(drt_scene_t* s, const double* d_verts, const double* camera21, int height, int width, int y0, int y1, int supersample,
                                 double ior_int, double ior_ext, int max_bounces, int law_flags, int fresnel, const double* screen9,
                                 const float* d_texture, int tex_h, int tex_w, int channels, const double* fill_void, const double* fill_invalid,
                                 const float* d_target, const float* d_weight, double* d_loss, double* d_grad_verts, double* d_grad_ior, float* d_image,
                                 int64_t* d_count, double* d_grad_screen, double* d_grad_texture, double* d_grad_camera, void* stream);

int drt_render_image_absorb(drt_scene_t* s, const double* d_verts, const double* camera21, int height, int width, int y0, int y1, int supersample,
                            double ior_int, double ior_ext, int max_bounces, int law_flags, int fresnel, const double* screen9,
                            const float* d_texture, int tex_h, int tex_w, int channels, const double* fill_void, const double* fill_invalid,
                            float* d_image, float* d_hit, float* d_through, const double* sigma, float* d_length, void* stream);
int drt_render_image_loss_absorb(drt_scene_t* s, const double* d_verts, const double* camera21, int height, int width, int y0, int y1, int supersample,
                                 double ior_int, double ior_ext, int max_bounces, int law_flags, int fresnel, const double* screen9,
                                 const float* d_texture, int tex_h, int tex_w, int channels, const double* fill_void, const double* fill_invalid,
                                 const float* d_target, const float* d_weight, double* d_loss, double* d_grad_verts, double* d_grad_ior, float* d_image,
                                 int64_t* d_count, const double* sigma, double* d_grad_sigma, void* stream);

int drt_render_image_env(drt_scene_t* s, const double* d_verts, const double* camera21, int height, int width, int y0, int y1, int supersample,
                         double ior_int, double ior_ext, int max_bounces, int law_flags, int fresnel, const double* screen9,
                         const float* d_texture, int tex_h, int tex_w, int channels, const double* fill_void, const double* fill_invalid,
                         float* d_image, float* d_hit, float* d_through, const float* d_env, int env_h, int env_w, const double* env_rot9,
                         int reflection, float* d_reflect, void* stream);

int drt_render_image_loss_env(drt_scene_t* s, const double* d_verts, const double* camera21, int height, int width, int y0, int y1, int supersample,
                              double ior_int, double ior_ext, int max_bounces, int law_flags, int fresnel, const double* screen9,
                              const float* d_texture, int tex_h, int tex_w, int channels, const double* fill_void, const double* fill_invalid,
                              const float* d_target, const float* d_weight, double* d_loss, double* d_grad_verts, double* d_grad_ior, float* d_image,
                              int64_t* d_count, const float* d_env, int env_h, int env_w, const double* env_rot9, int reflection, void* stream);

int drt_render_image_loss_env_param(drt_scene_t* s, const double* d_verts, const double* camera21, int height, int width, int y0, int y1, int supersample,
                                    double ior_int, double ior_ext, int max_bounces, int law_flags, int fresnel, const double* screen9,
                                    const float* d_texture, int tex_h, int tex_w, int channels, const double* fill_void, const double* fill_invalid,
                                    const float* d_target, const float* d_weight, double* d_loss, double* d_grad_verts, double* d_grad_ior, float* d_image,
                                    int64_t* d_count, const float* d_env, int env_h, int env_w, const double* env_rot9, int reflection, double* d_grad_env,
                                    double* d_grad_env_rot, void* stream);

typedef struct drt_image_views drt_image_views_t;
int drt_image_views_check(int n_views, const double* cameras21, const double* screens9, int height, int width);
int drt_image_views_create(drt_scene_t* s, int n_views, const double* cameras21, const double* screens9, int height, int width, drt_image_views_t** out);
void drt_image_views_destroy(drt_image_views_t* views);
int drt_render_image_loss_views(drt_scene_t* s, const double* d_verts, const drt_image_views_t* views, const int* view_ids, int k, int r0, int r1,
                                int supersample, double ior_int, double ior_ext, int max_bounces, int law_flags, int fresnel, const float* d_texture,
                                int tex_h, int tex_w, int channels, const double* fill_void, const double* fill_invalid, const float* d_targets,
                                const float* d_weights, double* d_loss, double* d_grad_verts, double* d_grad_ior, int64_t* d_count, void* stream);

int drt_render_image_loss_views_env(drt_scene_t* s, const double* d_verts, const drt_image_views_t* views, const int* view_ids, int k, int r0, int r1,
                                    int supersample, double ior_int, double ior_ext, int max_bounces, int law_flags, int fresnel, const float* d_texture,
                                    int tex_h, int tex_w, int channels, const double* fill_void, const double* fill_invalid, const float* d_targets,
                                    const float* d_weights, double* d_loss, double* d_grad_verts, double* d_grad_ior, int64_t* d_count, const float* d_env,
                                    int env_h, int env_w, const double* env_rot9, int reflection, void* stream);

#define DRT_PROFILE_STAGES 14
int drt_profile_enable(drt_scene_t* s, int on);
int drt_profile_select(drt_scene_t* s, uint32_t stage_mask);
int drt_profile_read(drt_scene_t* s, double* ms_out, int64_t* launches_out, int64_t* items_out);
int drt_profile_trace_stats(drt_scene_t* s, int64_t* out12);
int drt_route_counts(drt_scene_t* s, int64_t* out8);
int drt_raster_deal_counts(drt_scene_t* s, int64_t* out2);

int drt_check_violations(int64_t* out4);

#ifdef __cplusplus
}
#endif
#endif
```

Measured before the change: 47020 M camera-rays/s.

## Shorten front-end launch chain: fold big-tri raster, offload deal, merge late shade

Reduces the number of serial kernel launches before the first trace in each sub-batch. The pass-0 big-triangle raster kernel and its count memset are folded into the pass-1 raster kernel, using double-buffered big lists whose counters are reset in the view-fit kernels. The deal-table build is moved to an auxiliary stream and joined on the next call. When tree_late is active, shade1 is merged into k_gen_late running over all slots. Adds launch-count instrumentation, cross-call event dependencies and correctness risk around the big-list buffers.

```diff
diff --git a/drt_amd/_lib.py b/drt_amd/_lib.py
--- a/drt_amd/_lib.py
+++ b/drt_amd/_lib.py
@@ -133,6 +133,7 @@
     "drt_profile_trace_stats": (_c.c_int, [_P, _P]),
     "drt_route_counts": (_c.c_int, [_P, _P]),
     "drt_raster_deal_counts": (_c.c_int, [_P, _P]),
+    "drt_front_counts": (_c.c_int, [_P, _P]),
     "drt_check_violations": (_c.c_int, [_P]),
 }
 
diff --git a/drt_amd/csrc/drt_api.hip b/drt_amd/csrc/drt_api.hip
--- a/drt_amd/csrc/drt_api.hip
+++ b/drt_amd/csrc/drt_api.hip
@@ -143,6 +143,7 @@
     if (const char* ev = getenv("DRT_RASTER_DEAL")) s->raster_deal = atoi(ev) != 0;
     if (const char* ev = getenv("DRT_RASTER_DEAL_MIN_RUNS")) { const long long v = atoll(ev); if (v >= 0) s->raster_deal_min_runs = v; }
     if (const char* ev = getenv("DRT_RASTER_DEAL_FIXED")) { const int v = atoi(ev); if (v >= 1 && v <= 65536) s->raster_deal_fixed = (uint32_t)v; }
+    if (const char* ev = getenv("DRT_FRONT_CHAIN")) { const int v = atoi(ev); if (v >= 0 && v <= 7) s->front_chain = v; }
     if (const char* ev = getenv("DRT_HIT_SEED")) s->hit_seed = atoi(ev) != 0;
     if (const char* ev = getenv("DRT_ARM_FINISH_BESIDE")) s->arm_finish_beside = atoi(ev) != 0;
     if (const char* ev = getenv("DRT_SEED_TILED")) s->seed_tiled = atoi(ev) != 0;
@@ -158,6 +159,8 @@
         if (e == hipSuccess) e = hipEventCreateWithFlags(&w.tail, hipEventDisableTiming);
         if (e == hipSuccess) e = hipEventCreateWithFlags(&w.fill_fork, hipEventDisableTiming);
         if (e == hipSuccess) e = hipEventCreateWithFlags(&w.fill_join, hipEventDisableTiming);
+        if (e == hipSuccess) e = hipEventCreateWithFlags(&w.deal_fork, hipEventDisableTiming);
+        if (e == hipSuccess) e = hipEventCreateWithFlags(&w.deal_done, hipEventDisableTiming);
         if (e == hipSuccess) e = hipMalloc(&w.qcount, sizeof(unsigned) * kQCount);
         if (e == hipSuccess) e = hipMalloc(&w.slow_stack, sizeof(int32_t) * (size_t)kRedoGrid * kTraceBlock * kStackSlowDev);
     }
@@ -211,6 +214,8 @@
         if (w.done) (void)hipEventDestroy(w.done);
         if (w.fill_fork) (void)hipEventDestroy(w.fill_fork);
         if (w.fill_join) (void)hipEventDestroy(w.fill_join);
+        if (w.deal_fork) (void)hipEventDestroy(w.deal_fork);
+        if (w.deal_done) (void)hipEventDestroy(w.deal_done);
         if (w.tail) (void)hipEventDestroy(w.tail);
         if (w.stream) (void)hipStreamDestroy(w.stream);
     }
@@ -284,6 +289,13 @@
     return DRT_OK;
 }
 
+int drt_front_counts(drt_scene_t* s, int64_t* out) {
+    CHECK_SCENE(s);
+    if (!out) return fail(DRT_E_INVALID, "null pointer argument");
+    for (int k = 0; k < kFrontCounts; ++k) out[k] = s->front_counts[k];
+    return DRT_OK;
+}
+
 int drt_raster_deal_counts(drt_scene_t* s, int64_t* out2) {
     CHECK_SCENE(s);
     if (!out2) return fail(DRT_E_INVALID, "null pointer argument");
diff --git a/drt_amd/csrc/drt_pipeline.hip b/drt_amd/csrc/drt_pipeline.hip
--- a/drt_amd/csrc/drt_pipeline.hip
+++ b/drt_amd/csrc/drt_pipeline.hip
@@ -429,25 +429,29 @@
 __global__ void __launch_bounds__(kTraceBlock) k_gen_late(PathCtx c, const double* __restrict__ origin, const double* __restrict__ dir,
                                                           double* __restrict__ out_ori, double* __restrict__ out_dir, uint8_t* __restrict__ mask,
                                                           int32_t* __restrict__ face1, int32_t* __restrict__ face2, Pipe p,
-                                                          const int32_t* __restrict__ gen_list, bool prefilled, Ray64 r64) {
+                                                          const int32_t* __restrict__ gen_list, bool prefilled, Ray64 r64,
+                                                          bool whole ) {
     __shared__ int32_t lds[kStackFast][kTraceBlock];
-    const unsigned n = p.count[3];
+    const unsigned n = whole ? p.count[0] : p.count[3];
     if (n == 0) return;
     Stack st = make_stack(lds, c.tc);
     for (unsigned k = blockIdx.x * kTraceBlock + threadIdx.x; k < n; k += gridDim.x * kTraceBlock) {
-        const int32_t slot = gen_list[k];
-        if (p.r0.face[slot] != kFacePending) continue;
+        const int32_t slot = whole ? (int32_t)k : gen_list[k];
+        int32_t f1 = p.r0.face[slot];
+        if (!whole && f1 != kFacePending) continue;
         const int64_t i = p.r0.idx[slot];
-        const float* e = p.r0.ray + 6 * (int64_t)slot;
-        const Hit h = traverse<false>(c.tc.nodes, c.tc.tris, c.tc.n_tris, f3{e[0], e[1], e[2]}, f3{e[3], e[4], e[5]}, st);
-        p.r0.face[slot] = h.face;
-        face1[i] = h.face;
+        if (f1 == kFacePending) {
+            const float* e = p.r0.ray + 6 * (int64_t)slot;
+            f1 = traverse<false>(c.tc.nodes, c.tc.tris, c.tc.n_tris, f3{e[0], e[1], e[2]}, f3{e[3], e[4], e[5]}, st).face;
+            p.r0.face[slot] = f1;
+        }
+        face1[i] = f1;
         bool ok = false;
-        if (h.face >= 0) {
+        if (f1 >= 0) {
             d3 v0, v1, v2;
             int32_t vid[3];
             Bounce b;
-            load_tri64(c, h.face, v0, v1, v2, vid);
+            load_tri64(c, f1, v0, v1, v2, vid);
             bounce_forward(load_d3(origin, i), load_d3(dir, i), v0, v1, v2, c.ior_ext, c.ior_int, b);
             ok = !b.tir;
             if (ok) {
@@ -1179,6 +1183,8 @@
                         bool* n_finished ,
                         int32_t* seed2 = nullptr ) {
     if (n_finished) *n_finished = false;
+    s->front_open = true;
+    s->front_counts[kFrontSubs] += 1; s->front_counts[kFrontLast] = 0;
     const bool sparse_faces = (grid_mode & DRT_GRID_SPARSE_FACES) != 0;
     const bool pre_ori = (grid_mode & kIntPreOri) != 0, pre_dir = (grid_mode & kIntPreDir) != 0, pre_mask = (grid_mode & kIntPreMask) != 0;
     const bool all_verified = (grid_mode & DRT_GRID_ALL_VERIFIED) != 0 && (grid_mode & 3) == DRT_GRID_TRUST && grid_cache;
@@ -1207,8 +1213,9 @@
                 if (!pre_ori) (void)hipMemsetAsync(out_ori, 0, sizeof(double) * 3 * n, st);
                 if (!pre_dir) (void)hipMemsetAsync(out_dir, 0, sizeof(double) * 3 * n, st);
                 if (!pre_mask) (void)hipMemsetAsync(mask, 0, 3 * n, st);
-            }
-            if (!sparse_faces) { (void)hipMemsetAsync(face1, 0xFF, sizeof(int32_t) * n, st); (void)hipMemsetAsync(face2, 0xFF, sizeof(int32_t) * n, st); }
+                s->front(kFrontMemset, (int)!pre_ori + (int)!pre_dir + (int)!pre_mask);
+            }
+            if (!sparse_faces) { (void)hipMemsetAsync(face1, 0xFF, sizeof(int32_t) * n, st); (void)hipMemsetAsync(face2, 0xFF, sizeof(int32_t) * n, st); s->front(kFrontMemset, 2); }
         }
         if (late_fill && mega) {
             if (fs != st && aux) fs = aux;
@@ -1220,7 +1227,7 @@
             if (fs != st) HIP_TRY(hipEventRecord(w.fill_join, fs));
         }
         StageTimer t(s, st, kStageRaster);
-        rc = launch_raster(s, w, st, o, d, n_views, tile_w, tile_h, grid_mode == DRT_GRID_TRUST ? grid_cache : nullptr);
+        rc = launch_raster(s, w, st, o, d, n_views, tile_w, tile_h, grid_mode == DRT_GRID_TRUST ? grid_cache : nullptr, &aux);
         if (rc) return rc;
         rz = RasterIn{w.vmodel, grid_mode, w.zbuf, w.zmask, w.gen_list, tile_w, tile_h, all_verified ? 1 : 0, all_verified ? 1 : 0};
     }
@@ -1248,6 +1255,7 @@
       if (rz.views && grid_mode == DRT_GRID_TRUST) {
           uint32_t* list = reinterpret_cast<uint32_t*>(p.redo);
           k_patch_list<<<(n_patches + kPathBlock - 1) / kPathBlock, kPathBlock, 0, st>>>(n_patches, tile_w, rz, list, p.count + 7);
+          s->front(kFrontPatchList); s->front(kFrontCull);
           static const int cull_per_cu = cull_blocks_per_cu();
           const unsigned few = (unsigned)(kCullFewPerCu * s->n_cu), long_list = few * (unsigned)(kCullRun * kCullLongRuns);
           k_cull_listed<FUSED><<<cull_per_cu * s->n_cu, kPathBlock, 0, st>>>(list, p.count + 7, pc.tc.nodes, pc.tc.n_tris, o, d, valid, n, out_ori, out_dir, mask, face1, face2, p, tile_w, rz,
@@ -1255,8 +1263,10 @@
       } else {
           k_cull<FUSED><<<n_patches, kPathBlock, 0, st>>>(pc.tc.nodes, pc.tc.n_tris, o, d, valid, n, out_ori, out_dir, mask, face1, face2, p, tile_w, rz,
                                                           pre_ori && pre_dir && pre_mask && sparse_faces);
+          s->front(kFrontCull);
       } }
     auto issue_late_fills = [&]() -> int {
+        if (fs == st) s->front(kFrontMemset, (int)!pre_ori + (int)!pre_dir + (int)!pre_mask);
         if (fs != st) { HIP_TRY(hipEventRecord(w.fill_fork, st)); HIP_TRY(hipStreamWaitEvent(fs, w.fill_fork, 0)); }
         { StageTimer tf(s, fs, kStageFill);
           if (!pre_ori) (void)hipMemsetAsync(out_ori, 0, sizeof(double) * 3 * n, fs);
@@ -1267,30 +1277,38 @@
     };
     const bool fills_after_shade1 = s->fill_after_shade1 && fs != st;
     if (late_fill && !mega && !fills_after_shade1) { int rc = issue_late_fills(); if (rc) return rc; }
-    if (rz.views && grid_mode == DRT_GRID_ESTABLISH)
+    if (rz.views && grid_mode == DRT_GRID_ESTABLISH) {
         k_store_models<<<(int)(n / ((int64_t)tile_w * tile_h) + 63) / 64, 64, 0, st>>>(w.vmodel, grid_cache, (int)(n / ((int64_t)tile_w * tile_h)));
+        s->front(kFrontOther);
+    }
     { StageTimer t(s, st, kStageTrace1);
       if (rz.views && all_verified) {
       } else if (rz.views) {
+          s->front(kFrontTrace1); s->front_open = false;
           const TraceOut out{p.r0.face, nullptr, nullptr, w.gen_list};
           launch_trace_list(kTraceClosestListed, s->grid_path, st, pc.tc, p.r0.ray, p.count + 3, out, p.redo, p.count + 4, p.count + 16, s->refill_min, s->inner_min, s->prof_stats ? s->prof_counts + kProfStages + 4 * 0 : nullptr);
       } else {
+          s->front(kFrontTrace1); s->front_open = false;
           launch_trace_list(kTraceClosest, s->grid_path, st, pc.tc, p.r0.ray, p.count + 0, TraceOut{p.r0.face, nullptr, nullptr, nullptr}, p.redo, p.count + 4, p.count + 16, s->refill_min, s->inner_min, s->prof_stats ? s->prof_counts + kProfStages + 4 * 0 : nullptr);
       } }
     if (mega) {
         if (late_fill && fs != st) HIP_TRY(hipStreamWaitEvent(st, w.fill_join, 0));
         if (pre_any) HIP_TRY(hipStreamWaitEvent(st, s->prefill_done, 0));
     }
-    {
+    const bool late_merged = direct && tree_late && (s->front_chain & kFrontLateMerged) != 0;
+    if (!late_merged) {
       StageTimer t(s, st, kStageShade1);
-      k_shade1<FUSED><<<gs, kPathBlock, 0, st>>>(pc, o, d, out_ori, out_dir, mask, face1, face2, p, late_fill, r64p); }
+      k_shade1<FUSED><<<gs, kPathBlock, 0, st>>>(pc, o, d, out_ori, out_dir, mask, face1, face2, p, late_fill, r64p);
+      s->front(kFrontShade1); }
     if (late_fill && !mega && fills_after_shade1) { int rc = issue_late_fills(); if (rc) return rc; }
     if (tree_late) {
         int rc = wait_build(s, st); if (rc) return rc;
-        StageTimer t(s, st, kStageTrace1);
-        k_gen_late<FUSED><<<kRedoGrid, kTraceBlock, 0, st>>>(pc, o, d, out_ori, out_dir, mask, face1, face2, p, w.gen_list, late_fill, r64p);
+        StageTimer t(s, st, late_merged ? kStageShade1 : kStageTrace1);
+        k_gen_late<FUSED><<<kRedoGrid, kTraceBlock, 0, st>>>(pc, o, d, out_ori, out_dir, mask, face1, face2, p, w.gen_list, late_fill, r64p, late_merged);
+        s->front(kFrontGenLate);
     }
     if (mega) {
+        s->front(kFrontTrace); s->front_open = false;
         StageTimer t(s, st, kStagePath);
         k_path<FUSED><<<s->grid_mega, kPathBlock, 0, st>>>(pc, r64, out_ori, out_dir, mask, face2, p, p.count + 8, chunk_base, valid_idx,
                                                            s->mega_refill_min, s->inner_min, s->shade_min, s->prof_stats ? s->prof_counts + kProfStages + 4 * 1 : nullptr, s->prof_on);
@@ -1298,6 +1316,7 @@
         *n_finished = true;
         return DRT_OK;
     }
+    if (s->front_open) { s->front(kFrontTrace); s->front_open = false; }
     { StageTimer t(s, st, kStageTrace2);
       unsigned long long* stats = s->prof_stats ? s->prof_counts + kProfStages + 4 * 1 : nullptr;
       if (seed2 && s->hit_seed)
@@ -1316,6 +1335,7 @@
 }
 
 static int fork_streams(drt_scene* s, hipStream_t st, int streams) {
+    s->call_serial += 1;
     HIP_TRY(hipEventRecord(s->fork_ev, st));
     for (int k = 0; k < streams; ++k) HIP_TRY(hipStreamWaitEvent(s->sub[k].stream, s->fork_ev, 0));
     return DRT_OK;
diff --git a/drt_amd/csrc/drt_raster.hip b/drt_amd/csrc/drt_raster.hip
--- a/drt_amd/csrc/drt_raster.hip
+++ b/drt_amd/csrc/drt_raster.hip
@@ -1,10 +1,11 @@
 #include "drt_device.h"
 
 __global__ void __launch_bounds__(64) k_fit_views(const double* __restrict__ origin, const double* __restrict__ dir, int w, int h,
-                                                  ViewModel* __restrict__ views) {
+                                                  ViewModel* __restrict__ views, unsigned* __restrict__ big_count) {
     __shared__ ViewModel vm;
     const int64_t base = (int64_t)blockIdx.x * w * h;
     if (threadIdx.x == 0) {
+        if (blockIdx.x == 0) { big_count[0] = 0u; big_count[1] = 0u; }
         const int64_t i00 = base, iW0 = base + (w - 1), i0H = base + (int64_t)(h - 1) * w, iWH = i0H + (w - 1);
         if (fit_view_model(load_d3(origin, i00), load_d3(dir, i00), load_d3(dir, iW0), load_d3(dir, i0H), load_d3(dir, iWH),
                            (double)(w - 1), (double)(h - 1), vm))
@@ -32,11 +33,13 @@
     return h;
 }
 __global__ void __launch_bounds__(64) k_check_views(const double* __restrict__ origin, const double* __restrict__ dir, int w, int h,
-                                                    ViewModel* __restrict__ cache, ViewModel* __restrict__ views, unsigned salt, unsigned* __restrict__ salt_ctr) {
+                                                    ViewModel* __restrict__ cache, ViewModel* __restrict__ views, unsigned salt, unsigned* __restrict__ salt_ctr,
+                                                    unsigned* __restrict__ big_count) {
     __shared__ ViewModel vm;
     __shared__ unsigned s_ctr;
     const int64_t base = (int64_t)blockIdx.x * w * h;
     if (threadIdx.x == 0) {
+        if (blockIdx.x == 0) { big_count[0] = 0u; big_count[1] = 0u; }
         vm = cache[blockIdx.x];
         s_ctr = salt_ctr ? __hip_atomic_load(salt_ctr, __ATOMIC_RELAXED, __HIP_MEMORY_SCOPE_AGENT) : 0u;
         if (salt_ctr && blockIdx.x == 0) atomicAdd(salt_ctr, 1u);
@@ -91,6 +94,25 @@
 
 struct BigItem { int32_t view, tri, x0, y0, nx, ny; };
 
+__device__ __forceinline__ void raster_big_entries(const TriRec* __restrict__ tris, const ViewModel* views, const double* __restrict__ dir, int w, int h,
+                                                   unsigned long long* __restrict__ zbuf, uint32_t* __restrict__ zmask,
+                                                   const BigItem* __restrict__ big, unsigned n, unsigned wave, unsigned n_waves, int lane) {
+    for (unsigned e = wave; e < n; e += n_waves) {
+        const BigItem it = big[e];
+        const ViewModel& vm = views[it.view];
+        const TriRec t = tris[it.tri];
+        const f3 o32 = to_f32(d3{vm.o[0], vm.o[1], vm.o[2]});
+        const int64_t base = (int64_t)it.view * w * h;
+        const int cnt = it.nx * it.ny;
+        for (int p = lane; p < cnt; p += 64) {
+            const int row = (int)(((float)p + 0.5f) / (float)it.nx);
+            int y = it.y0 + row, x = it.x0 + (p - row * it.nx);
+            if (x >= it.x0 + it.nx) { x -= it.nx; ++y; } else if (x < it.x0) { x += it.nx; --y; }
+            raster_test(t, o32, dir, base + (int64_t)y * w + x, raster_slot((unsigned)x, (unsigned)(it.view * h + y), (unsigned)w), zbuf, zmask);
+        }
+    }
+}
+
 struct RasterLane {
     TriRec tri;
     int32_t x0, y0, nx, end;
@@ -103,13 +125,18 @@
 __global__ void __launch_bounds__(256, 8) k_raster(const TriRec* __restrict__ tris, int n_tris, ViewModel* views, int n_views,
                                                    const double* __restrict__ dir, int w, int h,
                                                    unsigned long long* __restrict__ zbuf, uint32_t* __restrict__ zmask,
-                                                   BigItem* __restrict__ big, unsigned* big_count,
-                                                   const DealPos* __restrict__ table ) {
+                                                   BigItem* __restrict__ big , unsigned* big_count ,
+                                                   const DealPos* __restrict__ table ,
+                                                   int fold_big ) {
     constexpr unsigned big_cap = drt_scene::kBigCap;
     __shared__ RasterLane s_lane[256];
     const int lane = threadIdx.x & 63;
     RasterLane* const wl = s_lane + (threadIdx.x & ~63);
     const unsigned n_waves = gridDim.x * 4u, wave = __builtin_amdgcn_readfirstlane(blockIdx.x * 4u + (threadIdx.x >> 6));
+    if (pass == 1 && fold_big)
+        raster_big_entries(tris, views, dir, w, h, zbuf, zmask, big, min(__builtin_amdgcn_readfirstlane(big_count[0]), big_cap), wave, n_waves, lane);
+    BigItem* const my_big = big + pass * (size_t)big_cap;
+    unsigned* const my_count = big_count + pass;
     const unsigned runs_per_view = ((unsigned)n_tris + 63u) / 64u, n_runs = runs_per_view * (unsigned)n_views;
     int cur_view = -1;
     float minv32[9] = {};
@@ -148,14 +175,14 @@
                     const int64_t cnt = (int64_t)nx * ny;
                     if (cnt > kRasterMaxPerLane) {
                         const int rows_per = max(1, kRasterBandPixels / nx), n_bands = (ny + rows_per - 1) / rows_per;
-                        const unsigned slot = sl.owner ? atomicAdd(big_count, (unsigned)n_bands) : 0u;
+                        const unsigned slot = sl.owner ? atomicAdd(my_count, (unsigned)n_bands) : 0u;
                         if (!sl.owner) {
                         } else if (slot <= big_cap && (unsigned)n_bands <= big_cap - slot) {
                             for (int b = 0; b < n_bands; ++b)
-                                big[slot + b] = BigItem{view, k, box.x0, box.y0 + b * rows_per, nx, min(rows_per, ny - b * rows_per)};
+                                my_big[slot + b] = BigItem{view, k, box.x0, box.y0 + b * rows_per, nx, min(rows_per, ny - b * rows_per)};
                         } else {
                             __hip_atomic_store(&views[view].ok, 0, __ATOMIC_RELAXED, __HIP_MEMORY_SCOPE_AGENT);
-                            for (unsigned q = slot; q < big_cap; ++q) big[q] = BigItem{view, k, 0, 0, 0, 0};
+                            for (unsigned q = slot; q < big_cap; ++q) my_big[q] = BigItem{view, k, 0, 0, 0, 0};
                         }
                     } else {
                         count = (int)cnt;
@@ -237,22 +264,8 @@
                                                     unsigned long long* __restrict__ zbuf, uint32_t* __restrict__ zmask,
                                                     const BigItem* __restrict__ big, const unsigned* __restrict__ big_count, unsigned big_cap) {
     const unsigned n = min(*big_count, big_cap);
-    const unsigned n_waves = gridDim.x * 4u;
-    const int lane = threadIdx.x & 63;
-    for (unsigned e = __builtin_amdgcn_readfirstlane(blockIdx.x * 4u + (threadIdx.x >> 6)); e < n; e += n_waves) {
-        const BigItem it = big[e];
-        const ViewModel& vm = views[it.view];
-        const TriRec t = tris[it.tri];
-        const f3 o32 = to_f32(d3{vm.o[0], vm.o[1], vm.o[2]});
-        const int64_t base = (int64_t)it.view * w * h;
-        const int cnt = it.nx * it.ny;
-        for (int p = lane; p < cnt; p += 64) {
-            const int row = (int)(((float)p + 0.5f) / (float)it.nx);
-            int y = it.y0 + row, x = it.x0 + (p - row * it.nx);
-            if (x >= it.x0 + it.nx) { x -= it.nx; ++y; } else if (x < it.x0) { x += it.nx; --y; }
-            raster_test(t, o32, dir, base + (int64_t)y * w + x, raster_slot((unsigned)x, (unsigned)(it.view * h + y), (unsigned)w), zbuf, zmask);
-        }
-    }
+    raster_big_entries(tris, views, dir, w, h, zbuf, zmask, big, n, __builtin_amdgcn_readfirstlane(blockIdx.x * 4u + (threadIdx.x >> 6)), gridDim.x * 4u,
+                       (int)(threadIdx.x & 63));
 }
 
 __global__ void k_fill_u64(unsigned long long* __restrict__ p, int64_t n, unsigned long long v) {
@@ -278,7 +291,7 @@
         HIP_TRY(hipMalloc(&w.vmodel, sizeof(ViewModel) * n_views));
         w.vm_cap = n_views;
     }
-    if (!w.big) HIP_TRY(hipMalloc(&w.big, sizeof(BigItem) * drt_scene::kBigCap));
+    if (!w.big) HIP_TRY(hipMalloc(&w.big, sizeof(BigItem) * 2 * drt_scene::kBigCap));
     drt_scene::Sub::Deal& dl = w.deal;
     if (!w.big_count) {
         const int n_waves = 8 * s->n_cu * 4;
@@ -292,36 +305,54 @@
 }
 
 int launch_raster(drt_scene* s, drt_scene::Sub& w, hipStream_t st, const double* d_origin, const double* d_dir, int n_views, int iw, int ih,
-                  ViewModel* trusted) {
+                  ViewModel* trusted, const hipStream_t* aux) {
     const int n = (int)s->n_faces;
-    HIP_TRY(hipMemsetAsync(w.big_count, 0, sizeof(unsigned), st));
+    drt_scene::Sub::Deal& dl = w.deal;
+    hipStreamCaptureStatus cap = hipStreamCaptureStatusNone;
+    (void)hipStreamIsCapturing(st, &cap);
+    const bool capturing = cap != hipStreamCaptureStatusNone;
+    if (dl.is_aside && (dl.aside_call == s->call_serial || ((!aux || dl.aside != *aux) && !capturing && !dl.aside_captured)))
+        HIP_TRY(hipStreamWaitEvent(st, w.deal_done, 0));
     if (trusted) k_check_views<<<n_views, 64, 0, st>>>(d_origin, d_dir, iw, ih, trusted, w.vmodel,
                                                         s->grid_canary ? (++s->canary_salt ? s->canary_salt : ++s->canary_salt) : 0u,
-                                                        s->vcount + 3);
-    else k_fit_views<<<n_views, 64, 0, st>>>(d_origin, d_dir, iw, ih, w.vmodel);
+                                                        s->vcount + 3,
+                                                        w.big_count);
+    else k_fit_views<<<n_views, 64, 0, st>>>(d_origin, d_dir, iw, ih, w.vmodel, w.big_count);
+    s->front(kFrontViews);
     if (n > 0) {
-        drt_scene::Sub::Deal& dl = w.deal;
         const int grid = 8 * s->n_cu;
         const int64_t n_runs = raster_runs(n, n_views);
         const bool record = s->raster_deal && dl.table && n_runs > 0 && n_runs >= s->raster_deal_min_runs && n_runs <= dl.cap_runs && grid * 4 == dl.cap_waves;
         const bool dealt = record && dl.complete && dl.dir == d_dir && dl.n_views == n_views && dl.iw == iw && dl.ih == ih && dl.n_tris == n && dl.grid == grid;
         s->raster_deal_counts[dealt ? 0 : 1] += 2;
+        const bool fold = (s->front_chain & kFrontFoldBig) != 0;
+        BigItem* const big = reinterpret_cast<BigItem*>(w.big);
         for (int pass = 0; pass < 2; ++pass) {
             auto* const kern = pass == 0 ? (dealt ? k_raster<true, true, 0> : record ? k_raster<false, true, 0> : k_raster<false, false, 0>)
                                          : (dealt ? k_raster<true, true, 1> : record ? k_raster<false, true, 1> : k_raster<false, false, 1>);
-            kern<<<grid, 256, 0, st>>>(s->tris_flat, n, w.vmodel, n_views, d_dir, iw, ih, w.zbuf, w.zmask, reinterpret_cast<BigItem*>(w.big), w.big_count,
-                                       dealt ? dl.table + pass * (dl.cap_waves + 1) : nullptr);
-            if (pass == 0) {
-                k_raster_big<<<8 * s->n_cu, 256, 0, st>>>(s->tris_flat, w.vmodel, d_dir, iw, ih, w.zbuf, w.zmask,
-                                                           reinterpret_cast<const BigItem*>(w.big), w.big_count, drt_scene::kBigCap);
-                HIP_TRY(hipMemsetAsync(w.big_count, 0, sizeof(unsigned), st));
+            kern<<<grid, 256, 0, st>>>(s->tris_flat, n, w.vmodel, n_views, d_dir, iw, ih, w.zbuf, w.zmask, big, w.big_count,
+                                       dealt ? dl.table + pass * (dl.cap_waves + 1) : nullptr, fold ? 1 : 0);
+            s->front(kFrontRaster);
+            if (pass == 0 && !fold) {
+                k_raster_big<<<8 * s->n_cu, 256, 0, st>>>(s->tris_flat, w.vmodel, d_dir, iw, ih, w.zbuf, w.zmask, big, w.big_count, drt_scene::kBigCap);
+                s->front(kFrontRasterBig);
             }
         }
-        k_raster_big<<<8 * s->n_cu, 256, 0, st>>>(s->tris_flat, w.vmodel, d_dir, iw, ih, w.zbuf, w.zmask,
-                                                   reinterpret_cast<const BigItem*>(w.big), w.big_count, drt_scene::kBigCap);
+        k_raster_big<<<8 * s->n_cu, 256, 0, st>>>(s->tris_flat, w.vmodel, d_dir, iw, ih, w.zbuf, w.zmask, big + drt_scene::kBigCap, w.big_count + 1, drt_scene::kBigCap);
+        s->front(kFrontRasterBig);
         dl.complete = false;
         if (record) {
-            k_raster_deal<<<dim3((unsigned)((n_runs + kDealBlock - 1) / kDealBlock), 2), kDealBlock, 0, st>>>(w.big_count, dl.table, (unsigned)n_runs, (unsigned)(grid * 4), s->raster_deal_fixed);
+            hipStream_t ds = (s->front_chain & kFrontDealOff) && aux && *aux != st && !s->prof_serial ? *aux : st;
+            if (ds != st) { HIP_TRY(hipEventRecord(w.deal_fork, st)); HIP_TRY(hipStreamWaitEvent(ds, w.deal_fork, 0)); }
+            k_raster_deal<<<dim3((unsigned)((n_runs + kDealBlock - 1) / kDealBlock), 2), kDealBlock, 0, ds>>>(w.big_count, dl.table, (unsigned)n_runs, (unsigned)(grid * 4), s->raster_deal_fixed);
+            if (ds != st) {
+                HIP_TRY(hipEventRecord(w.deal_done, ds));
+                dl.is_aside = true; dl.aside = ds; dl.aside_call = s->call_serial; dl.aside_captured = capturing;
+                s->front_counts[kFrontDealAside] += 1;
+            } else {
+                dl.is_aside = false;
+                s->front(kFrontDeal);
+            }
             dl.dir = d_dir; dl.n_views = n_views; dl.iw = iw; dl.ih = ih; dl.n_tris = n; dl.grid = grid;
             dl.complete = true;
         }
diff --git a/drt_amd/csrc/drt_scene.h b/drt_amd/csrc/drt_scene.h
--- a/drt_amd/csrc/drt_scene.h
+++ b/drt_amd/csrc/drt_scene.h
@@ -46,6 +46,10 @@
 constexpr int kSortBlock = 256, kSortItems = 8, kSortTile = kSortBlock * kSortItems, kRadix = 256;
 
 enum { kRouteTotal = 0, kRouteRaster, kRouteTrust, kRouteDirect, kRoutePark, kRouteLateFill, kRouteTreeLate, kRouteMega };
+enum { kFrontSubs = 0, kFrontTotal, kFrontLast, kFrontMemset, kFrontViews, kFrontRaster, kFrontRasterBig, kFrontDeal, kFrontDealAside, kFrontPatchList,
+       kFrontCull, kFrontTrace1, kFrontShade1, kFrontGenLate, kFrontOther, kFrontTrace, kFrontCounts };
+static_assert(kFrontCounts == DRT_FRONT_COUNTS, "include/drt_hip.h");
+enum { kFrontFoldBig = 1, kFrontDealOff = 2, kFrontLateMerged = 4 };
 enum { kStageBuild = 0, kStageCull, kStageTrace1, kStageShade1, kStageTrace2, kStageShade2, kStageTrace3, kStageFinish, kStageCollect, kStageBackward, kStageLossBwdFused, kStageRaster, kStageFill, kStagePath, kProfStages };
 static_assert(kProfStages == DRT_PROFILE_STAGES, "include/drt_hip.h");
 
@@ -81,6 +85,11 @@
     bool cull_park = true;
     int64_t cull_direct_min_rays = (int64_t)1 << 25;
     int64_t route_counts[8] = {0};
+    int64_t front_counts[kFrontCounts] = {0};
+    bool front_open = false;
+    void front(int kind, int n = 1) { if (front_open) { front_counts[kind] += n; front_counts[kFrontTotal] += n; front_counts[kFrontLast] += n; } }
+    int front_chain = kFrontFoldBig | kFrontDealOff | kFrontLateMerged;
+    uint64_t call_serial = 0;
     int tree_mode = 0, rebuild_every = 1, since_full = 0;
     bool topology_fixed = false;
     uint32_t* bounds_acc = nullptr;
@@ -117,6 +126,7 @@
         int vm_cap = 0;
         void* big = nullptr;
         unsigned* big_count = nullptr;
+        hipEvent_t deal_fork = nullptr, deal_done = nullptr;
         int32_t* gen_list = nullptr;
         struct Deal {
             DealPos* table = nullptr;
@@ -125,6 +135,10 @@
             const double* dir = nullptr;
             int n_views = 0, iw = 0, ih = 0, n_tris = 0, grid = 0;
             bool complete = false;
+            bool is_aside = false;
+            hipStream_t aside = nullptr;
+            uint64_t aside_call = 0;
+            bool aside_captured = false;
         } deal;
     };
     static constexpr unsigned kBigCap = 1u << 20;
@@ -193,7 +207,7 @@
 
 int ensure_raster(drt_scene* s, drt_scene::Sub& w, int64_t n_rays, int n_views, hipStream_t st);
 int launch_raster(drt_scene* s, drt_scene::Sub& w, hipStream_t st, const double* d_origin, const double* d_dir, int n_views, int iw, int ih,
-                  ViewModel* trusted);
+                  ViewModel* trusted, const hipStream_t* aux );
 
 void paths_free(drt_scene* s);
 void image_loss_free(drt_scene* s);
diff --git a/drt_amd/optix_mesh.py b/drt_amd/optix_mesh.py
--- a/drt_amd/optix_mesh.py
+++ b/drt_amd/optix_mesh.py
@@ -226,6 +226,14 @@
         _lib.check(_lib.lib().drt_raster_deal_counts(self._h, out))
         return tuple(out)
 
+    FRONT = ("subs", "total", "last", "memset", "views", "raster", "raster_big", "deal", "deal_aside", "patch_list", "cull", "trace1", "shade1",
+             "gen_late", "other", "trace")
+
+    def front_counts(self):
+        out = (ctypes.c_int64 * len(self.FRONT))()
+        _lib.check(_lib.lib().drt_front_counts(self._h, out))
+        return dict(zip(self.FRONT, out))
+
     def trace_stats(self):
         out = (ctypes.c_int64 * 12)()
         _lib.check(_lib.lib().drt_profile_trace_stats(self._h, out))
diff --git a/include/drt_hip.h b/include/drt_hip.h
--- a/include/drt_hip.h
+++ b/include/drt_hip.h
@@ -350,6 +350,8 @@
 int drt_profile_trace_stats(drt_scene_t* s, int64_t* out12);
 int drt_route_counts(drt_scene_t* s, int64_t* out8);
 int drt_raster_deal_counts(drt_scene_t* s, int64_t* out2);
+#define DRT_FRONT_COUNTS 16
+int drt_front_counts(drt_scene_t* s, int64_t* out);
 
 int drt_check_violations(int64_t* out4);
 
```

After: 47550 M camera-rays/s, median of 4. About the same (+1.1%).
